# stateSpaceRobotics/pointcloud_obstacle_processing

Measured on NVIDIA B200. Metric: points/sec per B200 job (HDL-64 120k-point frames: crop + 0.1 m voxel + RANSAC ground removal + Euclidean clustering + centroid/radius), higher is better.
Workload: dtype f32

## Files before the change

### pointcloud_obstacle_processing_b200/csrc/internal.cuh

```cuda
#pragma once
#include "common.cuh"

struct pcop_handle;

namespace pcop {

int fail_cuda(pcop_handle* h, cudaError_t e, const char* expr, const char* file, int line);

struct KernelTimers {
  static constexpr int MAX_SLOTS = 8192;
  static constexpr int MAX_NAMES = 64;
  bool enabled = false;
  cudaEvent_t* ev = nullptr;
  int used = 0;
  const char* slot_name[MAX_SLOTS];
  int n_names = 0;
  const char* names[MAX_NAMES];
  double total_us[MAX_NAMES];
  long long launches[MAX_NAMES];
};

struct Ctx {
  cudaStream_t stream;
  int B;
  int cap;
  int64_t* launches;
  KernelTimers* kt;
  int grid_cap;
  cudaEvent_t block_ev = nullptr;
};

inline cudaError_t stream_wait(cudaStream_t s, cudaEvent_t block_ev) {
  if (!block_ev) return cudaStreamSynchronize(s);
  const cudaError_t e = cudaEventRecord(block_ev, s);
  return e != cudaSuccess ? e : cudaEventSynchronize(block_ev);
}

inline void count_launch(const Ctx& c, int n = 1) { *c.launches += n; }

struct KScope {
  const Ctx& c;
  int slot;
  KScope(const Ctx& cc, const char* name) : c(cc), slot(-1) {
    KernelTimers* k = c.kt;
    if (k && k->enabled && k->ev && k->used < KernelTimers::MAX_SLOTS) {
      slot = k->used++;
      k->slot_name[slot] = name;
      cudaEventRecord(k->ev[2 * slot], c.stream);
    }
  }
  ~KScope() {
    if (slot >= 0) cudaEventRecord(c.kt->ev[2 * slot + 1], c.stream);
  }
};
#define KL(ctx, name, ...)          \
  do {                              \
    ::pcop::KScope _ks(ctx, name);  \
    __VA_ARGS__;                    \
  } while (0)

struct SortBufs {
  uint32_t* key[2];
  uint32_t* val[2];
  uint32_t* hist;
  uint32_t* desc;
  uint32_t* maxkey;
  int* npass;
  unsigned long long* stats;
};
size_t sort_desc_bytes(int B, int cap);
void radix_sort_batched(const Ctx& c, const SortBufs& s, const int* count, bool iota_vals);
void sort_reset_maxkey(const Ctx& c, const SortBufs& s);

struct CropArgs {
  const float4* in;
  size_t in_stride;
  const int* n_in;
  float4* out;
  int* kept_idx;
  int* n_out;
  MinMax* minmax;
  unsigned* desc;
  float lim[6];
};
void run_crop(const Ctx& c, const CropArgs& a);

void run_minmax(const Ctx& c, const float4* pts, size_t stride, const int* n, MinMax* minmax, bool finite_only = false);

struct VoxelArgs {
  const float4* in;
  size_t in_stride;
  const int* n_in;
  const MinMax* minmax;
  float leaf;
  VoxelFrame* vf;
  SortBufs sort;
  unsigned* desc;
  int* run_start;
  float4* out;
  uint32_t* out_keys;
  int* n_out;
  uint32_t* warnings;
};
void run_voxel(const Ctx& c, const VoxelArgs& a);

void run_grid_sort(const Ctx& c, const float4* in, size_t in_stride, const int* n_in, float cell, MinMax* minmax,
                   EceFrame* ef, const SortBufs& sort, float4* sorted_pts, int* parent, int* csize, int clique = 0);

struct VoxFusedPlan {
  int ok;
  float lim[6];
  float inv;
  int b0[3];
  uint32_t nx, ny, nz;
  int bits, npass, digit_bits;
  int part_ok, part_shift, nb, nb_pad;
};
VoxFusedPlan make_vox_fused_plan(const pcop_params& p);
void vox_part_plan(VoxFusedPlan& pl, size_t max_points);
size_t vox_fused_hist_elems(int B);
size_t vox_fused_desc_bytes(int B, int cap);
struct VoxelFusedArgs {
  const float4* in;
  size_t in_stride;
  const int* n_in;
  VoxFusedPlan plan;
  float leaf;
  MinMax* minmax;
  VoxelFrame* vf;
  SortBufs sort;
  unsigned long long* pair[2];
  unsigned* desc;
  uint32_t* flags;
  uint32_t* warnings;
  int* n_crop;
  float4* out;
  uint32_t* out_keys;
  int* n_out;
  int want_keys;
};
void run_voxel_fused(const Ctx& c, const VoxelFusedArgs& a);

int vox_part_chunks(int max_n, int B);
int vox_part_group_bound(const VoxFusedPlan& pl, int max_n);
size_t vox_part_hist_elems(int B);
size_t vox_part_start_elems(int B);
size_t vox_part_chunk_start_elems(int B);
size_t vox_part_bucket_elems(int B);
struct VoxelPartArgs {
  const float4* in;
  size_t in_stride;
  const int* n_in;
  VoxFusedPlan plan;
  float leaf;
  MinMax* minmax;
  VoxelFrame* vf;
  uint32_t* ghist;
  uint32_t* chunk_start;
  unsigned short* ne_bucket;
  uint32_t* ne_start;
  uint2* grec;
  int* n_groups;
  float4* part;
  unsigned* desc;
  int group_stride;
  int group_launch;
  uint32_t* flags;
  uint32_t* warnings;
  int* n_crop;
  float4* out;
  uint32_t* out_keys;
  int* n_out;
  int want_keys;
};
void run_voxel_part(const Ctx& c, const VoxelPartArgs& a);

struct SorArgs {
  const float4* in;
  size_t in_stride;
  const int* n_in;
  int meanK;
  double mul;
  float cell;
  MinMax* minmax;
  EceFrame* gf;
  SortBufs sort;
  float4* sorted_pts;
  float* dist;
  double* partial;
  double* thr;
  unsigned* desc;
  float4* out;
  int* kept_idx;
  int* n_out;
  uint32_t* warnings;
};
void run_sor(const Ctx& c, const SorArgs& a);

struct PlaneArgs {
  const float4* in;
  size_t in_stride;
  const int* n_in;
  int* n_in_copy;
  float4* buf[2];
  int* src[2];
  int* inlier_idx;
  PlaneFrame* pf;
  double* partial;
  unsigned* desc;
  int* n_tmp;
  int* n_active;
  int* h_n_active;
  const int* rng;
  int resident;
  int large_tier;
  PlaneConst pc;
  uint32_t* warnings;
  float4* out;
  int* out_src;
  int* n_out;
};
cudaError_t run_plane(const Ctx& c, const PlaneArgs& a);
int plane_small_tier_max();
int plane_resident_max();

struct ClusterArgs {
  const float4* in;
  size_t in_stride;
  const int* n_in;
  float tol;
  int min_size, max_size;
  int small_max;
  MinMax* minmax;
  EceFrame* ef;
  SortBufs sort;
  float4* sorted_pts;
  int* parent;
  int* csize;
  int* roots;
  int* rank_of;
  int* cell_start;
  uint32_t* cell_key;
  int* n_cells;
  int* n_route;
  unsigned* desc;
  int* offsets;
  int* indices;
  int* n_clusters;
  int* n_cluster_pts;
  float4* obstacles;
  double* partial;
  int partial_stride;
};
constexpr int ECE_SMALL_MAX = 8960;
int ece_small_limit();
bool run_cluster(const Ctx& c, const ClusterArgs& a, bool with_generic);
void run_cluster_small(const Ctx& c, const ClusterArgs& a, int small_max, bool zero_skipped);
void run_centroid_radius(const Ctx& c, const ClusterArgs& a);

struct OccGrid {
  float lim[6];
  float block_size, dev_percent;
  int W, H;
  long long cells;
};
enum { OCC_COUNT_SMEM32 = 0, OCC_COUNT_SMEM16 = 1, OCC_COUNT_GLOBAL = 2 };
constexpr int OCC_SMEM_BYTES = 220 * 1024;
int occ_count_mode(long long cells);
void run_occ_count(const Ctx& c, const float4* in, int n, const OccGrid& g, unsigned long long* counts);
void run_occ_finish(const Ctx& c, const unsigned long long* counts, const OccGrid& g, long long* row_avg, signed char* grid);
cudaError_t run_occ_count_wave(const Ctx& c, const float4* in, size_t in_stride, const int* n_in, const OccGrid& g,
                               int* counts);
void run_occ_finish_wave(const Ctx& c, const int* counts, const OccGrid& g, signed char* grids, uint32_t* warnings);

struct Mat34 {
  float m[12];
};
struct OccShadowArgs {
  const float4* cloud;
  size_t cloud_stride;
  const int* n_points;
  const int* offsets;
  size_t offsets_stride;
  const int* indices;
  size_t indices_stride;
  const int* n_clusters;
  const Mat34* mats;
  float y_min, x_max, block_size;
  int W;
  long long size;
  int opacity;
  signed char* grid;
  int* records;
  uint32_t* warnings;
};
void run_occ_shadows(const Ctx& c, const OccShadowArgs& a, int blocks_per_frame, int max_points);

}
```

### pointcloud_obstacle_processing_b200/csrc/pcop_api.cu

```cuda
#include <cstdio>
#include <cstdlib>
#include <chrono>
#include <cstring>
#include <cmath>
#include <string>
#include <vector>

#include "internal.cuh"
#include "primitives.cuh"

using namespace pcop;

namespace {

enum {
  CNT_IN = 0,
  CNT_CROP,
  CNT_VOX,
  CNT_SOR,
  CNT_REM,
  CNT_CLUS,
  CNT_CLPTS,
  CNT_TMP,
  CNT_NINL,
  CNT_CLUS1,
  CNT_CELLS,
  CNT_ROUTE,
  CNT_GROUPS,
  CNT_ROWS
};

enum {
  PK_CROP_KEPT = 0,
  PK_VOX_KEYS,
  PK_VOX_PTS,
  PK_SOR_KEPT,
  PK_INLIERS,
  PK_REM_PTS,
  PK_REM_SRC,
  PK_OFFSETS,
  PK_INDICES,
  PK_OBSTACLES,
  PK_N
};
const int kPkElem[PK_N] = {4, 4, 16, 4, 4, 16, 4, 4, 4, 16};
const int kPkCount[PK_N] = {CNT_CROP, CNT_VOX, CNT_VOX, CNT_SOR, CNT_NINL, CNT_REM, CNT_REM, CNT_CLUS1, CNT_CLPTS, CNT_CLUS};
const uint32_t kPkMask[PK_N] = {PCOP_OUT_CROP,      PCOP_OUT_VOXEL,     PCOP_OUT_VOXEL,    PCOP_OUT_SOR,
                                PCOP_OUT_PLANE,     PCOP_OUT_REMAINING, PCOP_OUT_REMAINING, PCOP_OUT_CLUSTERS,
                                PCOP_OUT_CLUSTERS,  PCOP_OUT_OBSTACLES};

struct PlaneRecord {
  int n_passes;
  int n_inliers_last;
  float4 coeff;
  int pass_points[PCOP_MAX_PLANE_PASSES_RECORDED];
  int pass_inliers[PCOP_MAX_PLANE_PASSES_RECORDED];
  float4 pass_coeff[PCOP_MAX_PLANE_PASSES_RECORDED];
};

struct PackMeta {
  unsigned long long base[PK_N];
  unsigned long long total_bytes;
  int total[PK_N];
  int overflow;
};

struct Pc2Frame {
  const unsigned char* data;
  int n, point_step, off_x, off_y, off_z;
  int is_dense, apply_transform, aligned;
  Mat34 t;
};

thread_local std::string g_global_error;

constexpr int PCOP_MIN_LANE_WAVE = 8;

}

struct pcop_handle {
  pcop_params params;
  int device = 0;
  int cap = 0;
  int maxB = 0;
  cudaStream_t stream = nullptr;
  std::string err;
  std::vector<void*> dev_allocs;
  std::vector<void*> host_allocs;

  float4 *d_in = nullptr, *d_crop = nullptr, *d_vox = nullptr, *d_sor = nullptr, *d_pbuf[2] = {nullptr, nullptr},
         *d_rem = nullptr, *d_sorted = nullptr, *d_obst = nullptr;
  int *d_crop_kept = nullptr, *d_run_start = nullptr, *d_sor_kept = nullptr, *d_psrc[2] = {nullptr, nullptr},
      *d_rem_src = nullptr, *d_inliers = nullptr, *d_parent = nullptr, *d_csize = nullptr, *d_roots = nullptr,
      *d_rank = nullptr, *d_indices = nullptr, *d_offsets = nullptr, *d_cell_start = nullptr;
  uint32_t* d_cell_key = nullptr;
  uint32_t* d_vox_keys = nullptr;
  float* d_sor_dist = nullptr;
  SortBufs sort{};
  unsigned* d_desc = nullptr;
  int* d_counts = nullptr;
  uint32_t* d_warnings = nullptr;
  MinMax* d_minmax = nullptr;
  VoxelFrame* d_vf = nullptr;
  EceFrame* d_ef = nullptr;
  PlaneFrame* d_pf = nullptr;
  PlaneRecord* d_prec = nullptr;
  double* d_partial = nullptr;
  double* d_thr = nullptr;
  int* d_n_active = nullptr;
  int* d_rng = nullptr;
  int* d_pack_off = nullptr;
  PackMeta* d_meta = nullptr;
  unsigned char* d_pack = nullptr;
  unsigned long long* d_pack_cursor = nullptr;
  cudaStream_t cstream = nullptr;
  cudaEvent_t ev_copied = nullptr;
  cudaEvent_t ev_meta = nullptr;
  int wave_seq = 0;
  int call_lane_waves = 1;
  bool pending = false;
  int pend_w0 = 0, pend_B = 0;
  double d2h_bytes = 0.0;
  float4* d_acc = nullptr;
  unsigned char* d_occ = nullptr;
  size_t occ_cap = 0;
  unsigned char* d_shadow = nullptr;
  size_t shadow_cap = 0;
  int* d_occ_counts = nullptr;
  signed char* d_occ_grids = nullptr;
  size_t occ_scratch_cells = 0;
  Mat34* d_occ_mats = nullptr;
  Mat34* h_occ_mats = nullptr;
  cudaEvent_t ev_grids_copied = nullptr;
  struct OccCall {
    OccGrid g;
    const float* world_to_sensor16;
    const float* sensor_to_world16;
    int8_t* grids;
    bool grids_on_device;
  };
  const OccCall* occ = nullptr;
  unsigned char* d_raw = nullptr;
  size_t raw_cap = 0;
  Pc2Frame* d_pc2 = nullptr;
  Pc2Frame* h_pc2 = nullptr;
  int acc_count = 0;
  size_t pack_cap = 0;
  uint32_t alloc_outputs = 0;

  int* h_n_active = nullptr;
  int* h_counts = nullptr;
  uint32_t* h_warnings = nullptr;
  PlaneRecord* h_prec = nullptr;
  PackMeta* h_meta = nullptr;
  int* h_n_in = nullptr;
  unsigned long long* h_stats = nullptr;
  unsigned long long sort_pass_keys = 0;
  unsigned char* h_pack_buf[2] = {nullptr, nullptr};
  size_t h_pack_buf_cap[2] = {0, 0};
  int h_pack_sel = 0;
  unsigned char* h_pack = nullptr;
  size_t h_pack_cap = 0;
  size_t h_pack_used = 0;

  cudaEvent_t ev_call[2] = {nullptr, nullptr};
  cudaEvent_t ev_stage[PCOP_N_STAGES][2] = {};
  bool stage_used[PCOP_N_STAGES] = {};
  float stage_us[PCOP_N_STAGES] = {};
  float last_elapsed_us = 0.f;
  int64_t launches = 0;
  double alg_bytes = 0.0;
  KernelTimers kt;

  int wave_frames = 0;
  bool trace = false;
  struct TraceRec {
    int w0, B;
    size_t bytes;
    cudaEvent_t meta, c0, c1;
  };
  std::vector<TraceRec> trace_recs;
  size_t trace_used = 0;
  int ece_small_max = 0;
  int plane_resident = 1;
  bool expect_big_remaining = false;
  bool expect_large_plane = false;
  int plane_hostloop_waves = 0;
  int vox_lsd_waves = 0;
  bool wave_plane_resident = false;
  bool wave_plane_speculated = false;
  const float4* plane_in = nullptr;
  size_t plane_stride = 0;
  const int* plane_n = nullptr;
  bool wave_cluster_speculated = false;
  int pend_max_n = 1;
  VoxFusedPlan vplan{};
  uint32_t* d_vf_flags = nullptr;
  unsigned long long* d_vf_pair[2] = {nullptr, nullptr};
  uint32_t* h_vf_flags = nullptr;
  int vox_mode = 0;
  int vox_redo = -1;
  bool vox_full_groups = false;
  bool wave_used_fused = false;
  uint32_t* d_vp_hist = nullptr;
  uint32_t* d_vp_bstart = nullptr;
  uint32_t* d_vp_nstart = nullptr;
  unsigned short* d_vp_ne = nullptr;
  uint2* d_vp_grec = nullptr;
  unsigned* d_vp_desc = nullptr;
  int vp_gstride = 0;
  int vp_group_hint = 0;
  std::vector<pcop_handle*> extra_lanes;
  std::vector<size_t> fixups;
  cudaEvent_t ev_lane_done = nullptr;

  int* cnt(int row) { return d_counts + (size_t)row * maxB; }
};

namespace pcop {
int fail_cuda(pcop_handle* h, cudaError_t e, const char* expr, const char* file, int line) {
  char buf[512];
  snprintf(buf, sizeof(buf), "CUDA error %d (%s) at %s:%d: %s", (int)e, cudaGetErrorString(e), file, line, expr);
  if (h) h->err = buf;
  g_global_error = buf;
  return PCOP_ERR_CUDA;
}
}

namespace {

int fail(pcop_handle* h, int code, const std::string& msg) {
  if (h) h->err = msg;
  g_global_error = msg;
  return code;
}

void fill_rng_table(uint32_t seed, int* out, int count) {
  uint32_t mt[624];
  mt[0] = seed;
  for (int i = 1; i < 624; ++i) mt[i] = 1812433253u * (mt[i - 1] ^ (mt[i - 1] >> 30)) + (uint32_t)i;
  int pos = 624;
  for (int k = 0; k < count; ++k) {
    if (pos >= 624) {
      for (int i = 0; i < 624; ++i) {
        const uint32_t y = (mt[i] & 0x80000000u) | (mt[(i + 1) % 624] & 0x7fffffffu);
        mt[i] = mt[(i + 397) % 624] ^ (y >> 1) ^ ((y & 1u) ? 0x9908b0dfu : 0u);
      }
      pos = 0;
    }
    uint32_t y = mt[pos++];
    y ^= y >> 11;
    y ^= (y << 7) & 0x9d2c5680u;
    y ^= (y << 15) & 0xefc60000u;
    y ^= y >> 18;
    out[k] = (int)(y >> 1);
  }
}

VoxFusedPlan make_plan(const pcop_params& p, size_t max_points, int* mode) {
  VoxFusedPlan pl = make_vox_fused_plan(p);
  vox_part_plan(pl, max_points);
  const char* s = getenv("PCOP_VOXEL_FUSED");
  if (s && s[0] == '0') pl.ok = 0;
  if (s && (s[0] == 'l' || s[0] == 'L')) pl.part_ok = 0;
  if (!pl.ok) pl.part_ok = 0;
  *mode = pl.part_ok ? 2 : (pl.ok ? 1 : 0);
  return pl;
}

int validate_params(pcop_handle* h, const pcop_params& p) {
  if (p.enable_voxel && !(p.downsample_size > 0.0f)) return fail(h, PCOP_ERR_BAD_PARAM, "downsample_size must be > 0");
  if (p.enable_sor && (p.statistical_outlier_meanK < 1 || p.statistical_outlier_meanK > 63))
    return fail(h, PCOP_ERR_BAD_PARAM, "statistical_outlier_meanK must be in [1, 63]");
  if (p.enable_plane && (p.plane_max_iterations < 0 || p.plane_max_iterations + 1 > PCOP_MAX_HYPOTHESES))
    return fail(h, PCOP_ERR_BAD_PARAM, "plane_max_iterations must be in [0, 63]");
  if (p.enable_plane && !(p.plane_probability > 0.0 && p.plane_probability < 1.0))
    return fail(h, PCOP_ERR_BAD_PARAM, "plane_probability must be in (0, 1)");
  if (p.enable_cluster && !(p.euc_cluster_tolerance > 0.0f))
    return fail(h, PCOP_ERR_BAD_PARAM, "euc_cluster_tolerance must be > 0");
  return PCOP_OK;
}

uint32_t effective_outputs(const pcop_params& p) {
  uint32_t m = p.outputs & (uint32_t)(PCOP_OUT_ALL | PCOP_OUT_DEVICE);
  if (p.publish_point_clouds) m |= PCOP_OUT_ALL;
  if (!p.enable_crop) m &= ~(uint32_t)PCOP_OUT_CROP;
  if (!p.enable_voxel) m &= ~(uint32_t)PCOP_OUT_VOXEL;
  if (!p.enable_sor) m &= ~(uint32_t)PCOP_OUT_SOR;
  if (!p.enable_plane) m &= ~(uint32_t)PCOP_OUT_PLANE;
  if (!p.enable_cluster) m &= ~(uint32_t)(PCOP_OUT_CLUSTERS | PCOP_OUT_OBSTACLES);
  return m;
}

size_t pack_capacity_bytes(uint32_t mask, int B, int cap) {
  mask &= (uint32_t)PCOP_OUT_ALL;
  size_t bytes = 0;
  for (int k = 0; k < PK_N; ++k)
    if (mask & kPkMask[k]) bytes += ((size_t)B * (cap + 1)) * kPkElem[k] + 256;
  return (bytes + 256 + 255) & ~(size_t)255;
}

template <class T>
int dalloc(pcop_handle* h, T** p, size_t n) {
  void* q = nullptr;
  cudaError_t e = cudaMalloc(&q, std::max<size_t>(n, 1) * sizeof(T));
  if (e != cudaSuccess) return fail_cuda(h, e, "cudaMalloc", __FILE__, __LINE__);
  h->dev_allocs.push_back(q);
  *p = (T*)q;
  return PCOP_OK;
}
template <class T>
int halloc(pcop_handle* h, T** p, size_t n) {
  void* q = nullptr;
  cudaError_t e = cudaHostAlloc(&q, std::max<size_t>(n, 1) * sizeof(T), cudaHostAllocMapped);
  if (e != cudaSuccess) return fail_cuda(h, e, "cudaHostAlloc", __FILE__, __LINE__);
  h->host_allocs.push_back(q);
  *p = (T*)q;
  return PCOP_OK;
}
#define TRY(x)                      \
  do {                              \
    int _s = (x);                   \
    if (_s != PCOP_OK) return _s;   \
  } while (0)

int ensure_pack_capacity(pcop_handle* h, uint32_t mask) {
  const size_t need = pack_capacity_bytes(mask, h->maxB, h->cap);
  if (need <= h->pack_cap) return PCOP_OK;
  if (h->cstream) cudaStreamSynchronize(h->cstream);
  if (h->d_pack) cudaFree(h->d_pack);
  h->d_pack = nullptr;
  h->pack_cap = 0;
  cudaError_t e = cudaMalloc((void**)&h->d_pack, need);
  if (e != cudaSuccess) return fail_cuda(h, e, "cudaMalloc(pack)", __FILE__, __LINE__);
  h->pack_cap = need;
  return PCOP_OK;
}

int ensure_host_pack(pcop_handle* h, size_t need) {
  if (need <= h->h_pack_cap) return PCOP_OK;
  size_t ncap = std::max<size_t>(need, h->h_pack_cap * 2);
  ncap = std::max<size_t>(ncap, 1 << 20);
  unsigned char* q = nullptr;
  cudaError_t e = cudaHostAlloc((void**)&q, ncap, cudaHostAllocMapped);
  if (e != cudaSuccess) return fail_cuda(h, e, "cudaHostAlloc(pack)", __FILE__, __LINE__);
  if (h->cstream) cudaStreamSynchronize(h->cstream);
  if (h->h_pack) {
    memcpy(q, h->h_pack, h->h_pack_cap);
    cudaFreeHost(h->h_pack);
  }
  h->h_pack = q;
  h->h_pack_cap = ncap;
  h->h_pack_buf[h->h_pack_sel] = q;
  h->h_pack_buf_cap[h->h_pack_sel] = ncap;
  return PCOP_OK;
}

int ensure_raw(pcop_handle* h, size_t bytes) {
  if (bytes <= h->raw_cap) return PCOP_OK;
  PCOP_CUDA_TRY(cudaStreamSynchronize(h->stream));
  if (h->d_raw) cudaFree(h->d_raw);
  h->d_raw = nullptr;
  h->raw_cap = 0;
  PCOP_CUDA_TRY(cudaMalloc((void**)&h->d_raw, bytes + bytes / 4 + 256));
  h->raw_cap = bytes + bytes / 4 + 256;
  return PCOP_OK;
}

__global__ void k_copy_counts(const int* __restrict__ src, int* __restrict__ dst, int B) {
  const int f = blockIdx.x * blockDim.x + threadIdx.x;
  if (f < B) dst[f] = src[f];
}

__global__ void k_zero_u32(uint32_t* p, int n) {
  const int i = blockIdx.x * blockDim.x + threadIdx.x;
  if (i < n) p[i] = 0u;
}

__global__ void __launch_bounds__(256)
    k_transform(const float4* __restrict__ in, int n, Mat34 t, int is_dense, float4* __restrict__ out) {
  const int i = blockIdx.x * blockDim.x + threadIdx.x;
  if (i >= n) return;
  const float4 p = __ldg(in + i);
  float4 o = p;
  const bool finite = fabsf(p.x) <= 3.402823466e+38f && fabsf(p.y) <= 3.402823466e+38f && fabsf(p.z) <= 3.402823466e+38f;
  if (is_dense || finite) {
    o.x = fadd(fadd(fadd(fmul(t.m[0], p.x), fmul(t.m[1], p.y)), fmul(t.m[2], p.z)), t.m[3]);
    o.y = fadd(fadd(fadd(fmul(t.m[4], p.x), fmul(t.m[5], p.y)), fmul(t.m[6], p.z)), t.m[7]);
    o.z = fadd(fadd(fadd(fmul(t.m[8], p.x), fmul(t.m[9], p.y)), fmul(t.m[10], p.z)), t.m[11]);
  }
  out[i] = o;
}

__device__ __forceinline__ float pc2_load_f32(const unsigned char* p) {
  if ((reinterpret_cast<uintptr_t>(p) & 3u) == 0u) return __ldg(reinterpret_cast<const float*>(p));
  const uint32_t b = (uint32_t)p[0] | ((uint32_t)p[1] << 8) | ((uint32_t)p[2] << 16) | ((uint32_t)p[3] << 24);
  return __uint_as_float(b);
}
__device__ __forceinline__ float pc2_lane(const float4& v, int k) {
  return k == 0 ? v.x : (k == 1 ? v.y : (k == 2 ? v.z : v.w));
}
__global__ void __launch_bounds__(256)
    k_pc2_ingest(const Pc2Frame* __restrict__ frames, float4* __restrict__ out, size_t out_stride) {
  const int f = blockIdx.y;
  const int n = frames[f].n;
  const int i = blockIdx.x * blockDim.x + threadIdx.x;
  if (i >= n) return;
  const Pc2Frame& d = frames[f];
  const unsigned char* rec = d.data + (size_t)i * (size_t)d.point_step;
  float x, y, z;
  if (d.aligned) {
    const float4 v = __ldg(reinterpret_cast<const float4*>(rec + (d.off_x & ~15)));
    x = pc2_lane(v, (d.off_x & 15) >> 2);
    y = pc2_lane(v, (d.off_y & 15) >> 2);
    z = pc2_lane(v, (d.off_z & 15) >> 2);
  } else {
    x = pc2_load_f32(rec + d.off_x);
    y = pc2_load_f32(rec + d.off_y);
    z = pc2_load_f32(rec + d.off_z);
  }
  float4 o = make_float4(x, y, z, 1.0f);
  const bool finite = fabsf(x) <= 3.402823466e+38f && fabsf(y) <= 3.402823466e+38f && fabsf(z) <= 3.402823466e+38f;
  if (d.apply_transform && (d.is_dense || finite)) {
    const Mat34& t = d.t;
    o.x = fadd(fadd(fadd(fmul(t.m[0], x), fmul(t.m[1], y)), fmul(t.m[2], z)), t.m[3]);
    o.y = fadd(fadd(fadd(fmul(t.m[4], x), fmul(t.m[5], y)), fmul(t.m[6], z)), t.m[7]);
    o.z = fadd(fadd(fadd(fmul(t.m[8], x), fmul(t.m[9], y)), fmul(t.m[10], z)), t.m[11]);
  }
  out[(size_t)f * out_stride + i] = o;
}

Pc2Frame make_pc2_frame(const unsigned char* src, int n, int point_step, int ox, int oy, int oz, const float* t16,
                        int is_dense) {
  Pc2Frame d{};
  d.data = src;
  d.n = n;
  d.point_step = point_step;
  d.off_x = ox;
  d.off_y = oy;
  d.off_z = oz;
  d.is_dense = is_dense ? 1 : 0;
  d.apply_transform = t16 ? 1 : 0;
  const float ident[12] = {1, 0, 0, 0, 0, 1, 0, 0, 0, 0, 1, 0};
  memcpy(d.t.m, t16 ? t16 : ident, sizeof(d.t.m));
  const bool word4 = (ox & 3) == 0 && (oy & 3) == 0 && (oz & 3) == 0;
  const bool one_word = (ox >> 4) == (oy >> 4) && (ox >> 4) == (oz >> 4);
  d.aligned = (point_step % 16 == 0 && (reinterpret_cast<uintptr_t>(src) & 15u) == 0u && word4 && one_word) ? 1 : 0;
  return d;
}

bool pc2_layout_ok(int point_step, int ox, int oy, int oz) {
  return point_step >= 4 && ox >= 0 && oy >= 0 && oz >= 0 && ox <= point_step - 4 && oy <= point_step - 4 &&
         oz <= point_step - 4;
}

__device__ __forceinline__ void pc2_store_f32(unsigned char* p, float v) {
  const uint32_t b = __float_as_uint(v);
  if ((reinterpret_cast<uintptr_t>(p) & 3u) == 0u) {
    *reinterpret_cast<uint32_t*>(p) = b;
  } else {
    p[0] = (unsigned char)b;
    p[1] = (unsigned char)(b >> 8);
    p[2] = (unsigned char)(b >> 16);
    p[3] = (unsigned char)(b >> 24);
  }
}
__global__ void __launch_bounds__(256)
    k_pc2_egress(const float4* __restrict__ in, int n, int point_step, int off_x, int off_y, int off_z,
                 unsigned char* __restrict__ out) {
  const int i = blockIdx.x * blockDim.x + threadIdx.x;
  if (i >= n) return;
  const float4 p = __ldg(in + i);
  unsigned char* rec = out + (size_t)i * (size_t)point_step;
  if (point_step == 16 && off_x == 0 && off_y == 4 && off_z == 8 && (reinterpret_cast<uintptr_t>(out) & 15u) == 0u) {
    *reinterpret_cast<float4*>(rec) = p;
    return;
  }
  for (int b = 0; b < point_step; ++b) rec[b] = 0;
  pc2_store_f32(rec + off_x, p.x);
  pc2_store_f32(rec + off_y, p.y);
  pc2_store_f32(rec + off_z, p.z);
  if (point_step == 16 && off_x == 0 && off_y == 4 && off_z == 8) pc2_store_f32(rec + 12, p.w);
}

__global__ void __launch_bounds__(CT_THREADS)
    k_copy_cloud(const float4* __restrict__ in, size_t in_stride, const int* __restrict__ n_in, float4* __restrict__ out,
                 int* __restrict__ out_src, int cap) {
  const int f = blockIdx.y, tile = blockIdx.x;
  const int n = n_in[f];
  if (tile * CT_TILE >= n) return;
#pragma unroll
  for (int k = 0; k < CT_ITEMS; ++k) {
    const int i = ct_index(tile, k);
    if (i < n) {
      out[(size_t)f * cap + i] = __ldg(in + (size_t)f * in_stride + i);
      out_src[(size_t)f * cap + i] = i;
    }
  }
}

__device__ void plane_record_one(const PlaneFrame* __restrict__ pf, PlaneRecord* __restrict__ rec, int* __restrict__ n_inl,
                                 int* __restrict__ n_clus, int* __restrict__ n_clus1, int plane_enabled, int f) {
  PlaneRecord r;
  r.n_passes = 0;
  r.n_inliers_last = 0;
  r.coeff = make_float4(0.f, 0.f, 0.f, 0.f);
  for (int k = 0; k < PCOP_MAX_PLANE_PASSES_RECORDED; ++k) {
    r.pass_points[k] = 0;
// ... 56 lines not shown
    if (lane == 0) total[k] = run;
  }
  __syncthreads();
  if (threadIdx.x == 0) {
    const unsigned long long start = cursor ? *cursor : 0ull;
    unsigned long long off = start;
    for (int k = 0; k < PK_N; ++k) {
      meta->base[k] = off;
      meta->total[k] = total[k];
      off += ((unsigned long long)total[k] * kPkElemD[k] + 255ull) & ~255ull;
    }
    meta->total_bytes = off - start;
    meta->overflow = (off > capacity) ? 1 : 0;
    if (cursor && off <= capacity) *cursor = off;
  }
}

struct MetaOut {
  const uint32_t* src[5];
  uint32_t* dst[5];
  int words[5];
  int frames;
};
__device__ __forceinline__ void meta_out_segment(const uint32_t* __restrict__ s, uint32_t* __restrict__ d, int words, int first,
                                                 int stride) {
  for (int i = first; i < words; i += stride) d[i] = s[i];
}
__device__ __forceinline__ void meta_out(const MetaOut& m, int k, int first, int stride) {
#pragma unroll
  for (int j = 0; j < 5; ++j)
    if (j == k && m.src[j]) meta_out_segment(m.src[j], m.dst[j], m.words[j], first, stride);
}
__global__ void __launch_bounds__(256) k_meta_out(MetaOut m) {
  meta_out(m, blockIdx.y, blockIdx.x * blockDim.x + threadIdx.x, gridDim.x * blockDim.x);
}
struct PackSrc {
  const uint32_t* src[PK_N];
  unsigned long long frame_stride_words[PK_N];
  int count_row[PK_N];
  int words_per_elem[PK_N];
};

__global__ void __launch_bounds__(256)
    k_pack(PackSrc ps, const int* __restrict__ counts, int maxB, const int* __restrict__ pack_off,
           const PackMeta* __restrict__ meta, unsigned char* __restrict__ pack, MetaOut mo) {
  const int which = blockIdx.z, f = blockIdx.y;
  if (f < mo.frames && which < 5)
    meta_out(mo, which, (f * gridDim.x + blockIdx.x) * blockDim.x + threadIdx.x, mo.frames * gridDim.x * blockDim.x);
  const uint32_t* base = ps.src[which];
  if (!base || meta->overflow) return;
  const int wpe = ps.words_per_elem[which];
  const int n = counts[(size_t)ps.count_row[which] * maxB + f];
  const uint32_t* s = base + (size_t)f * ps.frame_stride_words[which];
  uint32_t* dst = reinterpret_cast<uint32_t*>(pack + meta->base[which]) + (size_t)pack_off[(size_t)which * maxB + f] * wpe;
  if (wpe == 4) {
    const uint4* s4 = reinterpret_cast<const uint4*>(s);
    uint4* d4 = reinterpret_cast<uint4*>(dst);
    for (int i = blockIdx.x * blockDim.x + threadIdx.x; i < n; i += gridDim.x * blockDim.x) d4[i] = s4[i];
  } else {
    for (int i = blockIdx.x * blockDim.x + threadIdx.x; i < n; i += gridDim.x * blockDim.x) dst[i] = s[i];
  }
}

struct StageTimer {
  pcop_handle* h;
  int stage;
  StageTimer(pcop_handle* hh, int s) : h(hh), stage(s) {
    cudaEventRecord(h->ev_stage[s][0], h->stream);
    h->stage_used[s] = true;
  }
  ~StageTimer() { cudaEventRecord(h->ev_stage[stage][1], h->stream); }
};

void resolve_kernel_timers(pcop_handle* h) {
  KernelTimers& k = h->kt;
  for (int sl = 0; sl < k.used; ++sl) {
    float ms = 0.f;
    if (cudaEventElapsedTime(&ms, k.ev[2 * sl], k.ev[2 * sl + 1]) != cudaSuccess) {
      cudaGetLastError();
      continue;
    }
    int id = -1;
    for (int i = 0; i < k.n_names; ++i)
      if (k.names[i] == k.slot_name[sl] || strcmp(k.names[i], k.slot_name[sl]) == 0) {
        id = i;
        break;
      }
    if (id < 0 && k.n_names < KernelTimers::MAX_NAMES) {
      id = k.n_names++;
      k.names[id] = k.slot_name[sl];
      k.total_us[id] = 0.0;
      k.launches[id] = 0;
    }
    if (id >= 0) {
      k.total_us[id] += (double)ms * 1000.0;
      k.launches[id] += 1;
    }
  }
  k.used = 0;
}

Ctx make_ctx(pcop_handle* h, int B, int grid_cap = -1) {
  return Ctx{h->stream, B, h->cap, &h->launches, &h->kt, (grid_cap > 0 && grid_cap < h->cap) ? grid_cap : h->cap, nullptr};
}

PlaneConst make_plane_const(const pcop_params& p) {
  PlaneConst pc;
  pc.thr = p.plane_segment_dist_thres;
  pc.eps_angle = (double)p.plane_segment_angle;
  pc.cos_eps = std::cos(pc.eps_angle);
  for (int a = 0; a < 3; ++a) pc.axis[a] = (double)p.plane_axis[a];
  pc.keep_fraction = p.plane_keep_fraction;
  pc.max_iterations = p.plane_max_iterations;
  pc.probability = p.plane_probability;
  pc.log_probability = 0.0;
  pc.optimize = p.optimize_coefficients ? 1 : 0;
  return pc;
}

PlaneArgs make_plane_args(pcop_handle* h, const float4* in, size_t stride, const int* n_in) {
  PlaneArgs a{};
  a.in = in;
  a.in_stride = stride;
  a.n_in = n_in;
  a.buf[0] = h->d_pbuf[0];
  a.buf[1] = h->d_pbuf[1];
  a.src[0] = h->d_psrc[0];
  a.src[1] = h->d_psrc[1];
  a.inlier_idx = h->d_inliers;
  a.pf = h->d_pf;
  a.partial = h->d_partial;
  a.desc = h->d_desc;
  a.n_tmp = h->cnt(CNT_TMP);
  a.n_active = h->d_n_active;
  a.h_n_active = h->h_n_active;
  a.rng = h->d_rng;
  a.resident = h->plane_resident;
  a.pc = make_plane_const(h->params);
  a.warnings = h->d_warnings;
  a.out = h->d_rem;
  a.out_src = h->d_rem_src;
  a.n_out = h->cnt(CNT_REM);
  return a;
}

ClusterArgs make_cluster_args(pcop_handle* h, const float4* in, size_t stride, const int* n_in) {
  ClusterArgs a{};
  a.in = in;
  a.in_stride = stride;
  a.n_in = n_in;
  a.tol = h->params.euc_cluster_tolerance;
  a.min_size = h->params.euc_min_cluster_size;
  a.max_size = h->params.euc_max_cluster_size;
  a.small_max = h->ece_small_max;
  a.minmax = h->d_minmax;
  a.ef = h->d_ef;
  a.sort = h->sort;
  a.sorted_pts = h->d_sorted;
  a.parent = h->d_parent;
  a.csize = h->d_csize;
  a.roots = h->d_roots;
  a.rank_of = h->d_rank;
  a.cell_start = h->d_cell_start;
  a.cell_key = h->d_cell_key;
  a.n_cells = h->cnt(CNT_CELLS);
  a.n_route = h->cnt(CNT_ROUTE);
  a.desc = h->d_desc;
  a.offsets = h->d_offsets;
  a.indices = h->d_indices;
  a.n_clusters = h->cnt(CNT_CLUS);
  a.n_cluster_pts = h->cnt(CNT_CLPTS);
  a.obstacles = h->d_obst;
  a.partial = h->d_partial;
  a.partial_stride = cdiv(h->cap, TS_CHUNK) * 10;
  return a;
}

CropArgs make_crop_args(pcop_handle* h, const float4* in, size_t stride, const int* n_in) {
  CropArgs a{};
  a.in = in;
  a.in_stride = stride;
  a.n_in = n_in;
  a.out = h->d_crop;
  a.kept_idx = h->d_crop_kept;
  a.n_out = h->cnt(CNT_CROP);
  a.minmax = h->d_minmax;
  a.desc = h->d_desc;
  const pcop_params& p = h->params;
  a.lim[0] = p.x_min;
  a.lim[1] = p.x_max;
  a.lim[2] = p.y_min;
  a.lim[3] = p.y_max;
  a.lim[4] = p.z_min;
  a.lim[5] = p.z_max;
  return a;
}

VoxelArgs make_voxel_args(pcop_handle* h, const float4* in, size_t stride, const int* n_in) {
  VoxelArgs a{};
  a.in = in;
  a.in_stride = stride;
  a.n_in = n_in;
  a.minmax = h->d_minmax;
  a.leaf = h->params.downsample_size;
  a.vf = h->d_vf;
  a.sort = h->sort;
  a.desc = h->d_desc;
  a.run_start = h->d_run_start;
  a.out = h->d_vox;
  a.out_keys = h->d_vox_keys;
  a.n_out = h->cnt(CNT_VOX);
  a.warnings = h->d_warnings;
  return a;
}

SorArgs make_sor_args(pcop_handle* h, const float4* in, size_t stride, const int* n_in) {
  SorArgs a{};
  a.in = in;
  a.in_stride = stride;
  a.n_in = n_in;
  a.meanK = h->params.statistical_outlier_meanK;
  a.mul = (double)h->params.statistical_outlier_stdDevThres;
  a.cell = (h->params.enable_voxel && h->params.downsample_size > 0.0f) ? 3.0f * h->params.downsample_size : 0.05f;
  a.minmax = h->d_minmax;
  a.gf = h->d_ef;
  a.sort = h->sort;
  a.sorted_pts = h->d_sorted;
  a.dist = h->d_sor_dist;
  a.partial = h->d_partial;
  a.thr = h->d_thr;
  a.desc = h->d_desc;
  a.out = h->d_sor;
  a.kept_idx = h->d_sor_kept;
  a.n_out = h->cnt(CNT_SOR);
  a.warnings = h->d_warnings;
  return a;
}

bool is_device_pointer(const void* p) {
  cudaPointerAttributes at;
  if (cudaPointerGetAttributes(&at, p) != cudaSuccess) {
    cudaGetLastError();
    return false;
  }
  return at.type == cudaMemoryTypeDevice || at.type == cudaMemoryTypeManaged;
}

int run_wave_plane(pcop_handle* h, int B, int max_n, bool large_tier) {
  const pcop_params& p = h->params;
  Ctx c = make_ctx(h, B, max_n);
  StageTimer t(h, PCOP_STAGE_PLANE);
  h->wave_plane_speculated = false;
  if (p.enable_plane) {
    PlaneArgs a = make_plane_args(h, h->plane_in, h->plane_stride, h->plane_n);
    a.n_in_copy = p.enable_sor ? nullptr : h->cnt(CNT_SOR);
    a.large_tier = large_tier ? 1 : 0;
    if (h->plane_hostloop_waves > 0) a.resident = 0;
    h->wave_plane_resident = a.resident != 0;
    if (!(effective_outputs(p) & PCOP_OUT_PLANE)) a.inlier_idx = nullptr;
    cudaError_t e = run_plane(c, a);
    if (e != cudaSuccess) return fail_cuda(h, e, "run_plane", __FILE__, __LINE__);
    h->wave_plane_speculated = a.resident && !large_tier && max_n > plane_small_tier_max();
  } else {
    KL(c, "k_copy_counts", k_copy_counts<<<cdiv(B, 256), 256, 0, h->stream>>>(h->plane_n, h->cnt(CNT_REM), B));
    KL(c, "k_copy_cloud", k_copy_cloud<<<dim3(cdiv(c.grid_cap, CT_TILE), B), CT_THREADS, 0, h->stream>>>(
                              h->plane_in, h->plane_stride, h->plane_n, h->d_rem, h->d_rem_src, h->cap));
    count_launch(c, 2);
  }
  return PCOP_OK;
}

int run_wave_stages(pcop_handle* h, int B, const float4* in, size_t stride, int max_n) {
  const pcop_params& p = h->params;
  Ctx c = make_ctx(h, B, max_n);
  const int tiles = cdiv(h->cap, CT_TILE);
  const int vmode = (h->vox_redo >= 0) ? h->vox_redo : ((h->vox_mode == 2 && h->vox_lsd_waves > 0) ? 1 : h->vox_mode);
  const bool fused_path = vmode != 0;
  if (!fused_path || (effective_outputs(p) & PCOP_OUT_CROP)) {
    KL(c, "k_zero_u32", k_zero_u32<<<cdiv(B, 256), 256, 0, h->stream>>>(h->d_warnings, B));
    count_launch(c);
  }

  const float4* cur = in;
  size_t cur_stride = stride;
  const int* cur_n = h->cnt(CNT_IN);
  bool have_minmax = false;

  const bool fused = fused_path;
  h->wave_used_fused = fused;
  if (fused && vmode == 2) {
    {
      StageTimer t(h, PCOP_STAGE_CROP);
      if (effective_outputs(p) & PCOP_OUT_CROP) run_crop(c, make_crop_args(h, cur, cur_stride, cur_n));
    }
    StageTimer t(h, PCOP_STAGE_VOXEL);
    VoxelPartArgs a{};
    a.in = cur;
    a.in_stride = cur_stride;
    a.n_in = cur_n;
    a.plan = h->vplan;
    a.leaf = p.downsample_size;
    a.minmax = h->d_minmax;
    a.vf = h->d_vf;
    a.ghist = h->d_vp_hist;
    a.chunk_start = h->d_vp_bstart;
    a.ne_bucket = h->d_vp_ne;
    a.ne_start = h->d_vp_nstart;
    a.grec = h->d_vp_grec;
    a.n_groups = h->cnt(CNT_GROUPS);
    a.part = h->d_sorted;
    a.desc = h->d_vp_desc;
    a.group_stride = h->vp_gstride;
    a.group_launch = h->vox_full_groups ? h->vp_gstride - 1 : std::min(h->vp_group_hint, vox_part_group_bound(h->vplan, max_n));
    a.flags = h->d_vf_flags;
    a.warnings = (effective_outputs(p) & PCOP_OUT_CROP) ? nullptr : h->d_warnings;
    a.n_crop = h->cnt(CNT_CROP);
    a.out = h->d_vox;
    a.out_keys = h->d_vox_keys;
    a.n_out = h->cnt(CNT_VOX);
    a.want_keys = (effective_outputs(p) & PCOP_OUT_VOXEL) ? 1 : 0;
    run_voxel_part(c, a);
    cur = h->d_vox;
    cur_stride = h->cap;
    cur_n = h->cnt(CNT_VOX);
  } else if (fused) {
    {
      StageTimer t(h, PCOP_STAGE_CROP);
      if (effective_outputs(p) & PCOP_OUT_CROP) run_crop(c, make_crop_args(h, cur, cur_stride, cur_n));
    }
    StageTimer t(h, PCOP_STAGE_VOXEL);
    VoxelFusedArgs a{};
    a.in = cur;
    a.in_stride = cur_stride;
    a.n_in = cur_n;
    a.plan = h->vplan;
    a.leaf = p.downsample_size;
    a.minmax = h->d_minmax;
    a.vf = h->d_vf;
    a.sort = h->sort;
    a.pair[0] = h->d_vf_pair[0];
    a.pair[1] = h->d_vf_pair[1];
    a.desc = h->d_desc;
    a.flags = h->d_vf_flags;
    a.warnings = (effective_outputs(p) & PCOP_OUT_CROP) ? nullptr : h->d_warnings;
    a.n_crop = h->cnt(CNT_CROP);
    a.out = h->d_vox;
    a.out_keys = h->d_vox_keys;
    a.n_out = h->cnt(CNT_VOX);
    a.want_keys = (effective_outputs(p) & PCOP_OUT_VOXEL) ? 1 : 0;
    run_voxel_fused(c, a);
    cur = h->d_vox;
    cur_stride = h->cap;
    cur_n = h->cnt(CNT_VOX);
  } else {
    {
      StageTimer t(h, PCOP_STAGE_CROP);
      if (p.enable_crop) {
        run_crop(c, make_crop_args(h, cur, cur_stride, cur_n));
        cur = h->d_crop;
        cur_stride = h->cap;
        cur_n = h->cnt(CNT_CROP);
        have_minmax = true;
      } else {
        KL(c, "k_copy_counts", k_copy_counts<<<cdiv(B, 256), 256, 0, h->stream>>>(cur_n, h->cnt(CNT_CROP), B));
        count_launch(c);
      }
    }
    {
      StageTimer t(h, PCOP_STAGE_VOXEL);
      if (p.enable_voxel) {
        if (!have_minmax) run_minmax(c, cur, cur_stride, cur_n, h->d_minmax);
        run_voxel(c, make_voxel_args(h, cur, cur_stride, cur_n));
        cur = h->d_vox;
        cur_stride = h->cap;
        cur_n = h->cnt(CNT_VOX);
      } else {
        KL(c, "k_copy_counts", k_copy_counts<<<cdiv(B, 256), 256, 0, h->stream>>>(cur_n, h->cnt(CNT_VOX), B));
        count_launch(c);
      }
    }
  }
  {
    StageTimer t(h, PCOP_STAGE_SOR);
    if (p.enable_sor) {
      run_sor(c, make_sor_args(h, cur, cur_stride, cur_n));
      cur = h->d_sor;
      cur_stride = h->cap;
      cur_n = h->cnt(CNT_SOR);
    } else if (!p.enable_plane) {
      KL(c, "k_copy_counts", k_copy_counts<<<cdiv(B, 256), 256, 0, h->stream>>>(cur_n, h->cnt(CNT_SOR), B));
      count_launch(c);
    }
  }
  h->plane_in = cur;
  h->plane_stride = cur_stride;
  h->plane_n = cur_n;
  TRY(run_wave_plane(h, B, max_n, h->expect_large_plane));
  cudaError_t e = cudaGetLastError();
  if (e != cudaSuccess) return fail_cuda(h, e, "stage launches", __FILE__, __LINE__);
  return PCOP_OK;
}

int run_wave_cluster(pcop_handle* h, int B, int max_n, bool with_generic) {
  const pcop_params& p = h->params;
  Ctx c = make_ctx(h, B, max_n);
  ClusterArgs ca = make_cluster_args(h, h->d_rem, h->cap, h->cnt(CNT_REM));
  bool generic_centroid = false;
  {
    StageTimer t(h, PCOP_STAGE_CLUSTER);
    if (p.enable_cluster) {
      generic_centroid = run_cluster(c, ca, with_generic);
    } else {
      cudaMemsetAsync(h->cnt(CNT_CLUS), 0, sizeof(int) * B, h->stream);
      cudaMemsetAsync(h->cnt(CNT_CLPTS), 0, sizeof(int) * B, h->stream);
    }
  }
  {
    StageTimer t(h, PCOP_STAGE_CENTROID);
    if (p.enable_cluster && generic_centroid) run_centroid_radius(c, ca);
  }
  h->wave_cluster_speculated = p.enable_cluster && !generic_centroid && max_n > h->ece_small_max;
  cudaError_t e = cudaGetLastError();
  if (e != cudaSuccess) return fail_cuda(h, e, "stage launches", __FILE__, __LINE__);
  return PCOP_OK;
}

struct Pc2Call {
  const pcop_pointcloud2_frame* frames;
  const float* transform16;
  std::vector<char> on_device;
};

struct WaveInput {
  const float* xyzw;
  size_t frame_stride_points;
  const int32_t* n;
  bool on_device;
  const Pc2Call* pc2;
};

size_t pc2_payload_bytes(const pcop_pointcloud2_frame& m) { return (size_t)m.n_points * (size_t)m.point_step; }

int enqueue_wave_decode(pcop_handle* h, const Pc2Call& pc, int w0, int B, int max_n) {
  if (h->vox_redo < 0) {
    size_t off = 0;
    for (int f = 0; f < B; ++f) {
      const pcop_pointcloud2_frame& m = pc.frames[w0 + f];
      const size_t bytes = pc2_payload_bytes(m);
      const unsigned char* src = m.data;
      if (bytes > 0 && !pc.on_device[w0 + f]) {
        PCOP_CUDA_TRY(cudaMemcpyAsync(h->d_raw + off, m.data, bytes, cudaMemcpyHostToDevice, h->stream));
        src = h->d_raw + off;
        off += (bytes + 255) & ~(size_t)255;
      }
      h->h_pc2[f] = make_pc2_frame(src, m.n_points, m.point_step, m.off_x, m.off_y, m.off_z,
                                   pc.transform16 ? pc.transform16 + (size_t)(w0 + f) * 16 : nullptr, m.is_dense);
    }
    PCOP_CUDA_TRY(cudaMemcpyAsync(h->d_pc2, h->h_pc2, sizeof(Pc2Frame) * B, cudaMemcpyHostToDevice, h->stream));
  }
  Ctx c = make_ctx(h, B, max_n);
  KL(c, "k_pc2_ingest", k_pc2_ingest<<<dim3(cdiv(max_n, 256), B), 256, 0, h->stream>>>(h->d_pc2, h->d_in, (size_t)h->cap));
  count_launch(c);
  return PCOP_OK;
}

int enqueue_wave_pack(pcop_handle* h, int B, int max_n, uint32_t mask) {
  Ctx c = make_ctx(h, B, max_n);
  StageTimer t(h, PCOP_STAGE_D2H);
  const bool dev_results = (mask & PCOP_OUT_DEVICE) != 0;
  if (!dev_results && h->wave_seq >= 1) PCOP_CUDA_TRY(cudaStreamWaitEvent(h->stream, h->ev_copied, 0));
  KL(c, "k_pack_scan", k_pack_scan<<<1, 320, 0, h->stream>>>(h->d_counts, h->maxB, B, mask, h->d_pack_off, h->d_meta, h->d_pf, h->d_prec,
                                             h->params.enable_plane ? 1 : 0, dev_results ? h->d_pack_cursor : nullptr,
                                             (unsigned long long)h->pack_cap));
  count_launch(c);
  const void* srcs[PK_N] = {h->d_crop_kept, h->d_vox_keys, h->d_vox,     h->d_sor_kept, h->d_inliers,
                            h->d_rem,       h->d_rem_src,  h->d_offsets, h->d_indices,  h->d_obst};
  const size_t strides[PK_N] = {(size_t)h->cap, (size_t)h->cap, (size_t)h->cap,     (size_t)h->cap, (size_t)h->cap,
                                (size_t)h->cap, (size_t)h->cap, (size_t)h->cap + 1, (size_t)h->cap, (size_t)h->cap};
  {
    PackSrc ps{};
    bool any = false;
    for (int k = 0; k < PK_N; ++k) {
      ps.src[k] = (mask & kPkMask[k]) ? (const uint32_t*)srcs[k] : nullptr;
      ps.frame_stride_words[k] = (unsigned long long)strides[k] * (kPkElem[k] / 4);
      ps.count_row[k] = kPkCount[k];
      ps.words_per_elem[k] = kPkElem[k] / 4;
      any = any || ps.src[k];
    }
    MetaOut m{};
    int nseg = 0;
    auto seg = [&](const void* src, void* dst, size_t bytes) {
      m.src[nseg] = (const uint32_t*)src;
      m.dst[nseg] = (uint32_t*)dst;
      m.words[nseg] = (int)(bytes / 4);
      ++nseg;
    };
    seg(h->d_counts, h->h_counts, sizeof(int) * CNT_ROWS * h->maxB);
    seg(h->d_warnings, h->h_warnings, sizeof(uint32_t) * B);
    seg(h->d_prec, h->h_prec, sizeof(PlaneRecord) * B);
    seg(h->d_meta, h->h_meta, sizeof(PackMeta));
    if (h->wave_used_fused) seg(h->d_vf_flags, h->h_vf_flags, sizeof(uint32_t) * B);
    static_assert(PK_N >= 5, "one pack block per metadata segment");
    if (any) {
      const int gx = std::max(1, std::min(cdiv(c.grid_cap, 256 * 4), std::max(16, 592 / B)));
      m.frames = std::min(B, 4);
      KL(c, "k_pack", k_pack<<<dim3(gx, B, PK_N), 256, 0, h->stream>>>(ps, h->d_counts, h->maxB, h->d_pack_off, h->d_meta, h->d_pack, m));
      count_launch(c);
    } else {
      KL(c, "k_meta_out", k_meta_out<<<dim3(4, nseg), 256, 0, h->stream>>>(m));
      count_launch(c);
    }
  }
  if (h->trace) {
    if (h->trace_used == h->trace_recs.size()) {
      pcop_handle::TraceRec r{};
      cudaEventCreate(&r.meta);
      cudaEventCreate(&r.c0);
      cudaEventCreate(&r.c1);
      h->trace_recs.push_back(r);
    }
    cudaEventRecord(h->trace_recs[h->trace_used].meta, h->stream);
  }
  PCOP_CUDA_TRY(cudaEventRecord(h->ev_meta, h->stream));
  return PCOP_OK;
}

int enqueue_wave_counts(pcop_handle* h, int w0, int B, const float4* in, size_t stride, int max_n) {
  const pcop_handle::OccCall& oc = *h->occ;
  for (int f = 0; f < B; ++f) {
    memcpy(h->h_occ_mats[2 * f].m, oc.world_to_sensor16 + (size_t)(w0 + f) * 16, sizeof(Mat34));
    memcpy(h->h_occ_mats[2 * f + 1].m, oc.sensor_to_world16 + (size_t)(w0 + f) * 16, sizeof(Mat34));
  }
  PCOP_CUDA_TRY(cudaMemcpyAsync(h->d_occ_mats, h->h_occ_mats, sizeof(Mat34) * 2 * B, cudaMemcpyHostToDevice, h->stream));
  PCOP_CUDA_TRY(cudaMemsetAsync(h->d_occ_counts, 0, sizeof(int) * (size_t)B * (size_t)oc.g.cells, h->stream));
  Ctx c = make_ctx(h, B, max_n);
  const cudaError_t e = run_occ_count_wave(c, in, stride, h->cnt(CNT_IN), oc.g, h->d_occ_counts);
  if (e != cudaSuccess) return fail_cuda(h, e, "run_occ_count_wave (shared-memory opt-in or launch)", __FILE__, __LINE__);
  return PCOP_OK;
}

int enqueue_wave_grids(pcop_handle* h, int B, int max_n) {
  const pcop_handle::OccCall& oc = *h->occ;
  Ctx c = make_ctx(h, B, max_n);
  PCOP_CUDA_TRY(cudaStreamWaitEvent(h->stream, h->ev_grids_copied, 0));
  run_occ_finish_wave(c, h->d_occ_counts, oc.g, h->d_occ_grids, h->d_warnings);
  OccShadowArgs a{};
  a.cloud = h->d_rem;
  a.cloud_stride = h->cap;
  a.n_points = h->cnt(CNT_REM);
  a.offsets = h->d_offsets;
  a.offsets_stride = (size_t)h->cap + 1;
  a.indices = h->d_indices;
  a.indices_stride = h->cap;
  a.n_clusters = h->cnt(CNT_CLUS);
  a.mats = h->d_occ_mats;
  a.y_min = oc.g.lim[2];
  a.x_max = oc.g.lim[1];
  a.block_size = oc.g.block_size;
  a.W = oc.g.W;
  a.size = oc.g.cells;
  a.opacity = h->params.grid_opacity;
  a.grid = h->d_occ_grids;
  a.warnings = h->d_warnings;
  run_occ_shadows(c, a, std::max(4, std::min(64, cdiv(2048, B))), max_n);
  cudaError_t e = cudaGetLastError();
  if (e != cudaSuccess) return fail_cuda(h, e, "grid launches", __FILE__, __LINE__);
  return PCOP_OK;
}

int enqueue_wave_back(pcop_handle* h, int B, int max_n, uint32_t mask, bool cluster_with_generic) {
  TRY(run_wave_cluster(h, B, max_n, cluster_with_generic));
  if (h->occ) TRY(enqueue_wave_grids(h, B, max_n));
  return enqueue_wave_pack(h, B, max_n, mask);
}

int enqueue_wave(pcop_handle* h, const WaveInput& wi, int w0, int B, uint32_t mask) {
  for (int s = 0; s < PCOP_N_STAGES; ++s) h->stage_used[s] = false;
  const float4* in;
  size_t stride;
  const int32_t* n = wi.n;
  int max_n = 1;
  for (int f = 0; f < B; ++f) max_n = std::max(max_n, (int)n[w0 + f]);
  {
    StageTimer t(h, PCOP_STAGE_H2D);
    memcpy(h->h_n_in, n + w0, sizeof(int) * B);
    PCOP_CUDA_TRY(cudaMemcpyAsync(h->cnt(CNT_IN), h->h_n_in, sizeof(int) * B, cudaMemcpyHostToDevice, h->stream));
    if (wi.pc2) {
      TRY(enqueue_wave_decode(h, *wi.pc2, w0, B, max_n));
      in = h->d_in;
      stride = h->cap;
    } else if (wi.on_device) {
      in = reinterpret_cast<const float4*>(wi.xyzw) + (size_t)w0 * wi.frame_stride_points;
      stride = wi.frame_stride_points;
    } else {
      const float* src = wi.xyzw + (size_t)w0 * wi.frame_stride_points * 4;
      bool uniform = true;
      for (int f = 1; f < B; ++f) uniform = uniform && (n[w0 + f] == n[w0]);
      if (B > 0 && uniform && n[w0] > 0) {
        PCOP_CUDA_TRY(cudaMemcpy2DAsync(h->d_in, (size_t)h->cap * 16, src, wi.frame_stride_points * 16, (size_t)n[w0] * 16,
                                        B, cudaMemcpyHostToDevice, h->stream));
      } else {
        for (int f = 0; f < B; ++f)
          if (n[w0 + f] > 0)
            PCOP_CUDA_TRY(cudaMemcpyAsync(h->d_in + (size_t)f * h->cap, src + (size_t)f * wi.frame_stride_points * 4,
                                          (size_t)n[w0 + f] * 16, cudaMemcpyHostToDevice, h->stream));
      }
      in = h->d_in;
      stride = h->cap;
// ... 224 lines not shown
  if ((!xyzw && !pc2) || !n || !out || batch < 0) return fail(h, PCOP_ERR_BAD_PARAM, "null argument");
  PCOP_CUDA_TRY(cudaSetDevice(h->device));
  for (int f = 0; f < batch; ++f) {
    if (n[f] < 0) return fail(h, PCOP_ERR_BAD_PARAM, "negative point count");
    if (n[f] > h->cap) return fail(h, PCOP_ERR_CAPACITY, "frame has more points than max_points");
    if ((size_t)n[f] > frame_stride_points && batch > 1) return fail(h, PCOP_ERR_BAD_PARAM, "frame_stride_points < n");
  }
  const uint32_t mask = effective_outputs(h->params);
  const WaveInput wi{xyzw, frame_stride_points, n, pc2 ? false : is_device_pointer(xyzw), pc2};
  std::vector<pcop_handle*> lanes(1, h);
  if (!h->kt.enabled)
    for (pcop_handle* l : h->extra_lanes) lanes.push_back(l);
  std::vector<std::pair<int, int>> waves;
  {
    const int L = (int)lanes.size();
    int nw = std::max(1, cdiv(batch, std::max(1, std::min(h->wave_frames, h->maxB))));
    if (nw < L) nw = std::max(1, std::min(L, batch / PCOP_MIN_LANE_WAVE));
    const int full = (nw > 1) ? std::min(h->maxB, cdiv(2 * batch, 2 * nw - 1)) : std::min(h->maxB, batch);
    for (int w0 = 0; w0 < batch;) {
      const int B = std::min(full, batch - w0);
      waves.push_back({w0, B});
      w0 += B;
    }
  }
  size_t raw_need = 0;
  if (pc2)
    for (const auto& w : waves) {
      size_t bytes = 0;
      for (int f = w.first; f < w.first + w.second; ++f)
        if (!pc2->on_device[f]) bytes += (pc2_payload_bytes(pc2->frames[f]) + 255) & ~(size_t)255;
      raw_need = std::max(raw_need, bytes);
    }
  h->occ = nullptr;
  for (pcop_handle* l : h->extra_lanes) l->occ = nullptr;
  for (pcop_handle* l : lanes) {
    l->occ = occ;
    if (occ && !waves.empty()) TRY(ensure_occ_scratch(l, (size_t)waves[0].second, (size_t)occ->g.cells));
    if (raw_need) TRY(ensure_raw(l, raw_need));
    l->params = h->params;
    l->vplan = h->vplan;
    l->vox_mode = h->vox_mode;
    l->launches = 0;
    l->alg_bytes = 0.0;
    l->d2h_bytes = 0.0;
    l->kt.used = 0;
    l->sort_pass_keys = 0;
    l->h_pack_used = 0;
    l->h_pack_sel ^= 1;
    l->h_pack = l->h_pack_buf[l->h_pack_sel];
    l->h_pack_cap = l->h_pack_buf_cap[l->h_pack_sel];
    l->fixups.clear();
    l->wave_seq = 0;
    l->call_lane_waves = cdiv((int)waves.size(), (int)lanes.size());
    l->trace_used = 0;
    l->pending = false;
    for (int s = 0; s < PCOP_N_STAGES; ++s) l->stage_us[s] = 0.f;
    TRY(ensure_pack_capacity(l, mask));
  }
  PCOP_CUDA_TRY(cudaEventRecord(h->ev_call[0], h->stream));
  if (h->trace) g_trace_t0 = std::chrono::steady_clock::now();
  for (size_t l = 0; l < lanes.size(); ++l) {
    if (l > 0) PCOP_CUDA_TRY(cudaStreamWaitEvent(lanes[l]->stream, h->ev_call[0], 0));
    PCOP_CUDA_TRY(cudaMemsetAsync(lanes[l]->sort.stats, 0, sizeof(unsigned long long), lanes[l]->stream));
    if (mask & PCOP_OUT_DEVICE)
      PCOP_CUDA_TRY(cudaMemsetAsync(lanes[l]->d_pack_cursor, 0, sizeof(unsigned long long), lanes[l]->stream));
  }
  int status = PCOP_OK;
  for (size_t w = 0; w < waves.size() && status == PCOP_OK; ++w) {
    pcop_handle* l = lanes[w % lanes.size()];
    const double th0 = h->trace ? trace_host_us() : 0.0;
    status = finish_wave(l, wi, mask, out);
    const double th1 = h->trace ? trace_host_us() : 0.0;
    if (status == PCOP_OK) status = enqueue_wave(l, wi, waves[w].first, waves[w].second, mask);
    if (h->trace)
      fprintf(stderr, "[pcop trace]   host: wave %4d+%-4d lane %zu: finish of the lane's previous wave %7.0f .. %7.0f us, enqueue .. %7.0f us\n",
              waves[w].first, waves[w].second, w % lanes.size(), th0, th1, trace_host_us());
    if (status != PCOP_OK && l != h) h->err = l->err;
  }
  for (size_t k = 0; k < lanes.size(); ++k) {
    pcop_handle* l = lanes[(waves.size() + k) % lanes.size()];
    const int st = finish_wave(l, wi, mask, out);
    if (st != PCOP_OK && status == PCOP_OK) {
      status = st;
      if (l != h) h->err = l->err;
    }
  }
  for (pcop_handle* l : lanes) {
    cudaMemcpyAsync(l->h_stats, l->sort.stats, sizeof(unsigned long long), cudaMemcpyDeviceToHost, l->stream);
    cudaEventRecord(l->ev_lane_done, l->cstream);
    cudaStreamWaitEvent(l->stream, l->ev_lane_done, 0);
    cudaEventRecord(l->ev_lane_done, l->stream);
    if (l != h) cudaStreamWaitEvent(h->stream, l->ev_lane_done, 0);
  }
  PCOP_CUDA_TRY(cudaEventRecord(h->ev_call[1], h->stream));
  PCOP_CUDA_TRY(cudaEventSynchronize(h->ev_call[1]));
  if (status != PCOP_OK) return status;
  float ms = 0.f;
  PCOP_CUDA_TRY(cudaEventElapsedTime(&ms, h->ev_call[0], h->ev_call[1]));
  h->last_elapsed_us = ms * 1000.f;
  if (h->trace) {
    fprintf(stderr, "[pcop trace] call of %d frames: %.0f us on the device\n", batch, ms * 1000.f);
    for (size_t li = 0; li < lanes.size(); ++li) {
      for (size_t k = 0; k < lanes[li]->trace_used; ++k) {
        const pcop_handle::TraceRec& tr = lanes[li]->trace_recs[k];
        float a = 0.f, b = 0.f, c = 0.f;
        cudaEventElapsedTime(&a, h->ev_call[0], tr.meta);
        cudaEventElapsedTime(&b, h->ev_call[0], tr.c0);
        cudaEventElapsedTime(&c, h->ev_call[0], tr.c1);
        fprintf(stderr, "[pcop trace]   lane %zu wave %4d+%-4d counts at %7.0f us, payload copy %7.0f .. %7.0f us (%.1f MB, %.1f GB/s)\n", li,
                tr.w0, tr.B, a * 1000.f, b * 1000.f, c * 1000.f, tr.bytes / 1e6, tr.bytes / 1e3 / std::max(1e-3f, (c - b) * 1000.f));
      }
      lanes[li]->trace_used = 0;
    }
    cudaGetLastError();
  }
  for (pcop_handle* l : lanes) {
    l->sort_pass_keys = *l->h_stats;
    for (size_t fx : l->fixups) {
      const void** slot = (const void**)((unsigned char*)out + fx);
      const size_t off = (size_t)(uintptr_t)(*slot) - 1;
      *slot = l->h_pack + off;
    }
    if (l == h) continue;
    h->launches += l->launches;
    h->alg_bytes += l->alg_bytes;
    h->d2h_bytes += l->d2h_bytes;
    h->sort_pass_keys += l->sort_pass_keys;
    for (int s = 0; s < PCOP_N_STAGES; ++s) h->stage_us[s] += l->stage_us[s];
    merge_kernel_timers(h, l);
  }
  return PCOP_OK;
}

int upload_single(pcop_handle* h, const float* xyzw, int32_t n, int count_row) {
  if (n < 0) return fail(h, PCOP_ERR_BAD_PARAM, "negative point count");
  if (n > h->cap) return fail(h, PCOP_ERR_CAPACITY, "cloud has more points than max_points");
  PCOP_CUDA_TRY(cudaSetDevice(h->device));
  h->h_n_in[0] = n;
  PCOP_CUDA_TRY(cudaMemcpyAsync(h->cnt(count_row), h->h_n_in, sizeof(int), cudaMemcpyHostToDevice, h->stream));
  if (n > 0) PCOP_CUDA_TRY(cudaMemcpyAsync(h->d_in, xyzw, (size_t)n * 16, cudaMemcpyDefault, h->stream));
  k_zero_u32<<<1, 32, 0, h->stream>>>(h->d_warnings, 1);
  return PCOP_OK;
}

int download(pcop_handle* h, void* dst, const void* src, size_t bytes) {
  if (!dst || bytes == 0) return PCOP_OK;
  PCOP_CUDA_TRY(cudaMemcpyAsync(dst, src, bytes, cudaMemcpyDeviceToHost, h->stream));
  return PCOP_OK;
}

int fetch_count(pcop_handle* h, int row, int32_t* out) {
  PCOP_CUDA_TRY(cudaMemcpyAsync(h->h_counts, h->cnt(row), sizeof(int), cudaMemcpyDeviceToHost, h->stream));
  PCOP_CUDA_TRY(cudaStreamSynchronize(h->stream));
  *out = h->h_counts[0];
  return PCOP_OK;
}

int fetch_warnings(pcop_handle* h, uint32_t* w) {
  PCOP_CUDA_TRY(cudaMemcpyAsync(h->h_warnings, h->d_warnings, sizeof(uint32_t), cudaMemcpyDeviceToHost, h->stream));
  PCOP_CUDA_TRY(cudaStreamSynchronize(h->stream));
  if (w) *w = h->h_warnings[0];
  return PCOP_OK;
}

}

extern "C" {

int pcop_abi_version(void) { return PCOP_ABI_VERSION; }
const char* pcop_global_error(void) { return g_global_error.c_str(); }
const char* pcop_last_error(const pcop_handle* h) { return h ? h->err.c_str() : g_global_error.c_str(); }

void pcop_params_init_code_defaults(pcop_params* p) {
  memset(p, 0, sizeof(*p));
  p->x_min = -1.0f; p->x_max = 1.0f; p->y_min = -0.5f; p->y_max = 0.6f; p->z_min = 0.0f; p->z_max = -0.5f;
  p->downsample_size = 0.015f;
  p->statistical_outlier_meanK = 15;
  p->statistical_outlier_stdDevThres = 1.0f;
  p->plane_segment_dist_thres = 0.040f;
  p->plane_segment_angle = 20;
  p->euc_cluster_tolerance = 0.4f;
  p->euc_min_cluster_size = 5;
  p->euc_max_cluster_size = 20000;
  p->plane_axis[0] = 0.0f; p->plane_axis[1] = 0.0f; p->plane_axis[2] = 1.0f;
  p->plane_keep_fraction = 0.3;
  p->plane_max_iterations = 50;
  p->plane_probability = 0.99;
  p->ransac_seed = 12345u;
  p->optimize_coefficients = 1;
  p->enable_crop = p->enable_voxel = p->enable_sor = p->enable_plane = p->enable_cluster = 1;
  p->publish_point_clouds = 1;
  p->outputs = PCOP_OUT_DEFAULT;
  p->accumulate_count = 2;
  p->block_size = 0.15f;
  p->dev_percent = 0.5f;
  p->grid_opacity = 0;
  p->downsample_input_data = 1;
  p->passthrough_filter_enable = 1;
  p->convex_hull_alpha = 180.0f;
}

void pcop_params_init_params_yaml(pcop_params* p) {
  pcop_params_init_code_defaults(p);
  p->x_min = 0.0f; p->x_max = 4.5f; p->y_min = 0.0f; p->y_max = 3.78f; p->z_min = -0.5f; p->z_max = 0.25f;
  p->accumulate_count = 200;
  p->block_size = 0.0375f;
  p->dev_percent = 0.9f;
  p->grid_opacity = 0;
  p->downsample_size = 0.015f;
  p->statistical_outlier_meanK = 15;
  p->statistical_outlier_stdDevThres = 4.0f;
  p->plane_segment_dist_thres = 0.040f;
  p->plane_segment_angle = 20;
  p->euc_cluster_tolerance = 0.4f;
  p->euc_min_cluster_size = 5;
  p->euc_max_cluster_size = 20000;
  p->convex_hull_alpha = 180.0f;
  p->publish_point_clouds = 1;
}

static int create_lane(const pcop_params* params, int device, size_t max_points, int max_batch, pcop_handle** out) {
  *out = nullptr;
  int ndev = 0;
  cudaError_t e = cudaGetDeviceCount(&ndev);
  if (e != cudaSuccess || ndev == 0) {
    cudaGetLastError();
    return fail(nullptr, PCOP_ERR_CUDA, "pcop_create: no CUDA device (this library has no CPU fallback)");
  }
  if (device < 0 || device >= ndev) return fail(nullptr, PCOP_ERR_BAD_PARAM, "pcop_create: bad device index");
  cudaDeviceProp prop;
  if ((e = cudaGetDeviceProperties(&prop, device)) != cudaSuccess) return fail_cuda(nullptr, e, "props", __FILE__, __LINE__);
  if (prop.major != 10)
    return fail(nullptr, PCOP_ERR_CUDA, "pcop_create: device is not sm_100-class (kernels are built for sm_100a only)");
  pcop_handle* h = new pcop_handle();
  h->params = *params;
  h->vplan = make_plan(*params, max_points, &h->vox_mode);
  h->device = device;
  h->cap = (int)max_points;
  h->maxB = max_batch;
  int st = validate_params(h, *params);
  if (st != PCOP_OK) {
    g_global_error = h->err;
    delete h;
    return st;
  }
  auto bail = [&](int code) {
    g_global_error = h->err;
    pcop_destroy(h);
    return code;
  };
  if ((e = cudaSetDevice(device)) != cudaSuccess) return bail(fail_cuda(h, e, "cudaSetDevice", __FILE__, __LINE__));
  if ((e = cudaStreamCreateWithFlags(&h->stream, cudaStreamNonBlocking)) != cudaSuccess)
    return bail(fail_cuda(h, e, "cudaStreamCreate", __FILE__, __LINE__));
  const size_t BC = (size_t)h->maxB * h->cap;
  const int B = h->maxB;
  const int chunks = cdiv(h->cap, TS_CHUNK);
  const int tiles = cdiv(h->cap, CT_TILE);
#define A(x)                         \
  do {                               \
    int _s = (x);                    \
    if (_s != PCOP_OK) return bail(_s); \
  } while (0)
  A(dalloc(h, &h->d_in, BC));
  A(dalloc(h, &h->d_acc, (size_t)h->cap));
  A(dalloc(h, &h->d_crop, BC));
  A(dalloc(h, &h->d_vox, BC));
  A(dalloc(h, &h->d_sor, BC));
  h->d_pbuf[0] = h->d_crop;
  h->d_pbuf[1] = h->d_in;
  A(dalloc(h, &h->d_rem, BC));
  A(dalloc(h, &h->d_sorted, BC));
  A(dalloc(h, &h->d_obst, BC));
  A(dalloc(h, &h->d_crop_kept, BC));
  A(dalloc(h, &h->d_run_start, BC));
  A(dalloc(h, &h->d_sor_kept, BC));
  A(dalloc(h, &h->d_psrc[0], BC));
  A(dalloc(h, &h->d_psrc[1], BC));
  A(dalloc(h, &h->d_rem_src, BC));
  A(dalloc(h, &h->d_inliers, BC));
  A(dalloc(h, &h->d_parent, BC));
  A(dalloc(h, &h->d_csize, BC));
  A(dalloc(h, &h->d_roots, BC));
  A(dalloc(h, &h->d_rank, BC));
  A(dalloc(h, &h->d_indices, BC));
  A(dalloc(h, &h->d_cell_start, BC));
  A(dalloc(h, &h->d_cell_key, BC));
  A(dalloc(h, &h->d_offsets, BC + B));
  A(dalloc(h, &h->d_vox_keys, BC));
  A(dalloc(h, &h->d_sor_dist, BC));
  A(dalloc(h, &h->sort.key[0], BC));
  A(dalloc(h, &h->sort.key[1], BC));
  A(dalloc(h, &h->sort.val[0], BC));
  A(dalloc(h, &h->sort.val[1], BC));
  A(dalloc(h, &h->sort.hist, std::max((size_t)B * RS_MAX_PASSES * RS_BINS, vox_fused_hist_elems(B))));
  {
    unsigned char* d = nullptr;
    A(dalloc(h, &d, std::max(sort_desc_bytes(B, h->cap), vox_fused_desc_bytes(B, h->cap))));
    h->sort.desc = (uint32_t*)d;
  }
  A(dalloc(h, &h->d_vf_flags, B));
  if (h->vplan.part_ok) {
    h->vp_gstride = vox_part_group_bound(h->vplan, h->cap) + 1;
    h->vp_group_hint = h->vp_gstride - 1;
    A(dalloc(h, &h->d_vp_hist, vox_part_hist_elems(B)));
    A(dalloc(h, &h->d_vp_bstart, vox_part_chunk_start_elems(B)));
    A(dalloc(h, &h->d_vp_nstart, vox_part_start_elems(B)));
    A(dalloc(h, &h->d_vp_ne, vox_part_bucket_elems(B)));
    A(dalloc(h, &h->d_vp_grec, (size_t)B * h->vp_gstride));
    A(dalloc(h, &h->d_vp_desc, (size_t)B * h->vp_gstride));
  }
  h->d_vf_pair[0] = reinterpret_cast<unsigned long long*>(h->d_sorted);
  h->d_vf_pair[1] = reinterpret_cast<unsigned long long*>(h->d_sorted) + BC;
  A(halloc(h, &h->h_vf_flags, B));
  A(dalloc(h, &h->sort.maxkey, B));
  A(dalloc(h, &h->sort.npass, B));
  A(dalloc(h, &h->sort.stats, 1));
  A(halloc(h, &h->h_stats, 1));
  A(dalloc(h, &h->d_desc, (size_t)B * tiles));
  A(dalloc(h, &h->d_counts, (size_t)CNT_ROWS * B));
  A(dalloc(h, &h->d_warnings, B));
  A(dalloc(h, &h->d_minmax, B));
  A(dalloc(h, &h->d_vf, B));
  A(dalloc(h, &h->d_ef, B));
  A(dalloc(h, &h->d_pf, B));
  A(dalloc(h, &h->d_prec, B));
  A(dalloc(h, &h->d_partial, (size_t)B * chunks * 10));
  A(dalloc(h, &h->d_thr, B));
  A(dalloc(h, &h->d_n_active, 64));
  A(dalloc(h, &h->d_rng, RNG_TABLE));
  A(dalloc(h, &h->d_pack_off, (size_t)PK_N * B));
  A(dalloc(h, &h->d_meta, 1));
  A(dalloc(h, &h->d_pack_cursor, 1));
  A(dalloc(h, &h->d_pc2, B));
  A(halloc(h, &h->h_pc2, B));
  A(halloc(h, &h->h_n_active, 16));
  A(halloc(h, &h->h_counts, (size_t)CNT_ROWS * B));
  A(halloc(h, &h->h_warnings, B));
  A(halloc(h, &h->h_prec, B));
  A(halloc(h, &h->h_meta, 1));
  A(halloc(h, &h->h_n_in, (size_t)B + 16));
#undef A
  if ((e = cudaMemset(h->d_counts, 0, sizeof(int) * CNT_ROWS * B)) != cudaSuccess)
    return bail(fail_cuda(h, e, "memset", __FILE__, __LINE__));
  if ((e = cudaMemset(h->d_pf, 0, sizeof(PlaneFrame) * B)) != cudaSuccess)
    return bail(fail_cuda(h, e, "memset", __FILE__, __LINE__));
  {
    std::vector<int> tbl(RNG_TABLE);
    fill_rng_table(params->ransac_seed, tbl.data(), RNG_TABLE);
    if ((e = cudaMemcpy(h->d_rng, tbl.data(), sizeof(int) * RNG_TABLE, cudaMemcpyHostToDevice)) != cudaSuccess)
      return bail(fail_cuda(h, e, "rng upload", __FILE__, __LINE__));
  }
  for (int i = 0; i < 2; ++i)
    if ((e = cudaEventCreate(&h->ev_call[i])) != cudaSuccess) return bail(fail_cuda(h, e, "event", __FILE__, __LINE__));
  for (int s = 0; s < PCOP_N_STAGES; ++s)
    for (int i = 0; i < 2; ++i)
      if ((e = cudaEventCreate(&h->ev_stage[s][i])) != cudaSuccess)
        return bail(fail_cuda(h, e, "event", __FILE__, __LINE__));
  if ((e = cudaEventCreateWithFlags(&h->ev_lane_done, cudaEventDisableTiming)) != cudaSuccess)
    return bail(fail_cuda(h, e, "event", __FILE__, __LINE__));
  if ((e = cudaStreamCreateWithFlags(&h->cstream, cudaStreamNonBlocking)) != cudaSuccess)
    return bail(fail_cuda(h, e, "cudaStreamCreate", __FILE__, __LINE__));
  if ((e = cudaEventCreateWithFlags(&h->ev_copied, cudaEventDisableTiming)) != cudaSuccess ||
      (e = cudaEventCreateWithFlags(&h->ev_meta, cudaEventDisableTiming)) != cudaSuccess ||
      (e = cudaEventCreateWithFlags(&h->ev_grids_copied, cudaEventDisableTiming)) != cudaSuccess)
    return bail(fail_cuda(h, e, "event", __FILE__, __LINE__));
  st = ensure_pack_capacity(h, effective_outputs(h->params));
  if (st != PCOP_OK) return bail(st);
  *out = h;
  return PCOP_OK;
}

int pcop_create(const pcop_params* params, int device, size_t max_points, int max_batch, pcop_handle** out) {
  if (!params || !out || max_points == 0 || max_points > (size_t)65535 * BT_TILE || max_batch < 1)
    return fail(nullptr, PCOP_ERR_BAD_PARAM, "pcop_create: bad argument (max_points must be in [1, 268431360])");
  *out = nullptr;
  int wave_frames = std::min(max_batch, std::max(64, max_batch / 8));
  if (const char* s = getenv("PCOP_WAVE_FRAMES")) wave_frames = (int)std::min<long>(std::max<long>(strtol(s, nullptr, 10), 1), max_batch);
  int n_lanes = std::max(1, std::min(3, max_batch / wave_frames));
  if (const char* s = getenv("PCOP_LANES")) n_lanes = (int)std::min<long>(std::max<long>(strtol(s, nullptr, 10), 1), 8);
  n_lanes = std::max(1, std::min(n_lanes, max_batch / PCOP_MIN_LANE_WAVE));
  const int lane_batch = n_lanes == 1 ? max_batch : std::min(max_batch, wave_frames + wave_frames / 4);
  pcop_handle* h = nullptr;
  int st = create_lane(params, device, max_points, lane_batch, &h);
  if (st != PCOP_OK) return st;
  for (int l = 1; l < n_lanes; ++l) {
    pcop_handle* x = nullptr;
    st = create_lane(params, device, max_points, lane_batch, &x);
    if (st != PCOP_OK) {
      pcop_destroy(h);
      return st;
    }
    h->extra_lanes.push_back(x);
  }
  h->wave_frames = std::min(wave_frames, lane_batch);
  h->trace = getenv("PCOP_TRACE") != nullptr;
  for (pcop_handle* l : h->extra_lanes) l->trace = h->trace;
  h->ece_small_max = ece_small_limit();
  if (const char* s = getenv("PCOP_PLANE_RESIDENT")) h->plane_resident = (s[0] == '0') ? 0 : 1;
  for (pcop_handle* l : h->extra_lanes) {
    l->ece_small_max = h->ece_small_max;
    l->plane_resident = h->plane_resident;
  }
  *out = h;
  return PCOP_OK;
}

void pcop_destroy(pcop_handle* h) {
  if (!h) return;
  for (pcop_handle* l : h->extra_lanes) pcop_destroy(l);
  h->extra_lanes.clear();
  cudaSetDevice(h->device);
  if (h->stream) cudaStreamSynchronize(h->stream);
  if (h->cstream) cudaStreamSynchronize(h->cstream);
  for (void* p : h->dev_allocs) cudaFree(p);
  for (void* p : h->host_allocs) cudaFreeHost(p);
  if (h->d_pack) cudaFree(h->d_pack);
  if (h->d_raw) cudaFree(h->d_raw);
  if (h->d_occ) cudaFree(h->d_occ);
  if (h->d_shadow) cudaFree(h->d_shadow);
  if (h->d_occ_counts) cudaFree(h->d_occ_counts);
  if (h->d_occ_grids) cudaFree(h->d_occ_grids);
  for (int i = 0; i < 2; ++i)
    if (h->h_pack_buf[i]) cudaFreeHost(h->h_pack_buf[i]);
  if (h->kt.ev) {
    for (int i = 0; i < 2 * KernelTimers::MAX_SLOTS; ++i) cudaEventDestroy(h->kt.ev[i]);
    delete[] h->kt.ev;
  }
  for (int i = 0; i < 2; ++i)
    if (h->ev_call[i]) cudaEventDestroy(h->ev_call[i]);
  if (h->ev_lane_done) cudaEventDestroy(h->ev_lane_done);
  if (h->ev_copied) cudaEventDestroy(h->ev_copied);
  if (h->ev_meta) cudaEventDestroy(h->ev_meta);
  if (h->ev_grids_copied) cudaEventDestroy(h->ev_grids_copied);
  if (h->cstream) cudaStreamDestroy(h->cstream);
  for (int s = 0; s < PCOP_N_STAGES; ++s)
    for (int i = 0; i < 2; ++i)
      if (h->ev_stage[s][i]) cudaEventDestroy(h->ev_stage[s][i]);
  if (h->stream) cudaStreamDestroy(h->stream);
  delete h;
}

int pcop_set_params(pcop_handle* h, const pcop_params* params) {
  if (!h || !params) return fail(h, PCOP_ERR_BAD_PARAM, "null argument");
  int st = validate_params(h, *params);
  if (st != PCOP_OK) return st;
  PCOP_CUDA_TRY(cudaSetDevice(h->device));
  if (params->ransac_seed != h->params.ransac_seed) {
    std::vector<int> tbl(RNG_TABLE);
    fill_rng_table(params->ransac_seed, tbl.data(), RNG_TABLE);
    PCOP_CUDA_TRY(cudaMemcpy(h->d_rng, tbl.data(), sizeof(int) * RNG_TABLE, cudaMemcpyHostToDevice));
  }
  h->params = *params;
  h->vplan = make_plan(*params, (size_t)h->cap, &h->vox_mode);
  h->vox_lsd_waves = 0;
  h->plane_hostloop_waves = 0;
  for (pcop_handle* l : h->extra_lanes) {
    const int ls = pcop_set_params(l, params);
    if (ls != PCOP_OK) {
      h->err = l->err;
      return ls;
    }
  }
  return ensure_pack_capacity(h, effective_outputs(h->params));
}

int pcop_process(pcop_handle* h, const float* xyzw, int32_t n, pcop_frame_result* out) {
  return process_impl(h, xyzw, (size_t)(n > 0 ? n : 1), &n, 1, out);
}

int pcop_process_batch(pcop_handle* h, const float* xyzw, size_t frame_stride_points, const int32_t* n, int32_t batch,
                       pcop_frame_result* out) {
  return process_impl(h, xyzw, frame_stride_points, n, batch, out);
}

static int occ_grid_of(pcop_handle* h, OccGrid* g);

static int occ_call_of(pcop_handle* h, const char* who, const float* world_to_sensor16, const float* sensor_to_world16,
                       int8_t* grids, pcop_handle::OccCall* oc) {
  TRY(occ_grid_of(h, &oc->g));
  if (oc->g.cells > PCOP_OCC_BATCH_MAX_CELLS)
    return fail(h, PCOP_ERR_CAPACITY,
                std::string(who) + ": grid of " + std::to_string(oc->g.W) + " x " + std::to_string(oc->g.H) +
                    " cells exceeds PCOP_OCC_BATCH_MAX_CELLS (use pcop_occupancy_grid + pcop_occupancy_shadows)");
  PCOP_CUDA_TRY(cudaSetDevice(h->device));
  oc->world_to_sensor16 = world_to_sensor16;
  oc->sensor_to_world16 = sensor_to_world16;
  oc->grids = grids;
  oc->grids_on_device = is_device_pointer(grids);
  return PCOP_OK;
}

int pcop_process_batch_occupancy(pcop_handle* h, const float* xyzw, size_t frame_stride_points, const int32_t* n,
                                 int32_t batch, const float* world_to_sensor16, const float* sensor_to_world16,
                                 int8_t* grids, pcop_frame_result* out) {
  if (!h) return fail(nullptr, PCOP_ERR_BAD_PARAM, "null handle");
  if (!world_to_sensor16 || !sensor_to_world16 || !grids || !out || batch < 0 || (!xyzw && batch != 1))
    return fail(h, PCOP_ERR_BAD_PARAM, "pcop_process_batch_occupancy: null argument (xyzw = NULL takes batch = 1)");
  pcop_handle::OccCall oc{};
  TRY(occ_call_of(h, "pcop_process_batch_occupancy", world_to_sensor16, sensor_to_world16, grids, &oc));
  int st;
  if (!xyzw) {
    const int32_t acc_n = h->acc_count;
    st = process_impl(h, reinterpret_cast<const float*>(h->d_acc), (size_t)(acc_n > 0 ? acc_n : 1), &acc_n, 1, out, &oc);
    h->acc_count = 0;
  } else {
    st = process_impl(h, xyzw, frame_stride_points, n, batch, out, &oc);
  }
  h->occ = nullptr;
  for (pcop_handle* l : h->extra_lanes) l->occ = nullptr;
  return st;
}

int pcop_process_batch_pointcloud2(pcop_handle* h, const pcop_pointcloud2_frame* frames, int32_t batch,
                                   const float* transform16, const float* world_to_sensor16,
                                   const float* sensor_to_world16, int8_t* grids, pcop_frame_result* out) {
  if (!h) return fail(nullptr, PCOP_ERR_BAD_PARAM, "null handle");
  if (!out || batch < 0 || (!frames && batch > 0) || (grids && (!world_to_sensor16 || !sensor_to_world16)))
    return fail(h, PCOP_ERR_BAD_PARAM,
                "pcop_process_batch_pointcloud2: null argument (grids need world_to_sensor16 and sensor_to_world16)");
  Pc2Call pc;
  pc.frames = frames;
  pc.transform16 = transform16;
  std::vector<int32_t> n((size_t)batch + 1, 0);
  for (int f = 0; f < batch; ++f) {
    const pcop_pointcloud2_frame& m = frames[f];
    if (m.n_points < 0 || (!m.data && m.n_points > 0))
      return fail(h, PCOP_ERR_BAD_PARAM, "pcop_process_batch_pointcloud2: frame " + std::to_string(f) + ": bad count or NULL data");
    if (!pc2_layout_ok(m.point_step, m.off_x, m.off_y, m.off_z))
      return fail(h, PCOP_ERR_BAD_PARAM,
                  "pcop_process_batch_pointcloud2: frame " + std::to_string(f) + ": PointCloud2 field offsets do not fit point_step");
    if (m.n_points > h->cap)
      return fail(h, PCOP_ERR_CAPACITY, "pcop_process_batch_pointcloud2: frame " + std::to_string(f) + " has more points than max_points");
    n[f] = m.n_points;
  }
  pcop_handle::OccCall oc{};
  if (grids) TRY(occ_call_of(h, "pcop_process_batch_pointcloud2", world_to_sensor16, sensor_to_world16, grids, &oc));
  PCOP_CUDA_TRY(cudaSetDevice(h->device));
  pc.on_device.resize((size_t)batch);
  for (int f = 0; f < batch; ++f) pc.on_device[f] = frames[f].n_points > 0 && is_device_pointer(frames[f].data);
  const int st = process_impl(h, nullptr, (size_t)h->cap, n.data(), batch, out, grids ? &oc : nullptr, &pc);
  h->occ = nullptr;
  for (pcop_handle* l : h->extra_lanes) l->occ = nullptr;
  return st;
}

int pcop_enable_kernel_timing(pcop_handle* h, int enable) {
  if (!h) return PCOP_ERR_BAD_PARAM;
  PCOP_CUDA_TRY(cudaSetDevice(h->device));
  if (enable && !h->kt.ev) {
    h->kt.ev = new cudaEvent_t[2 * KernelTimers::MAX_SLOTS];
    for (int i = 0; i < 2 * KernelTimers::MAX_SLOTS; ++i) PCOP_CUDA_TRY(cudaEventCreate(&h->kt.ev[i]));
  }
  h->kt.enabled = enable != 0;
  h->kt.used = 0;
  h->kt.n_names = 0;
  return PCOP_OK;
}

int pcop_kernel_timing_count(const pcop_handle* h) { return h ? h->kt.n_names : 0; }

int pcop_kernel_timing_get(const pcop_handle* h, int i, const char** name, double* total_us, int64_t* launches) {
  if (!h || i < 0 || i >= h->kt.n_names) return PCOP_ERR_BAD_PARAM;
  if (name) *name = h->kt.names[i];
  if (total_us) *total_us = h->kt.total_us[i];
  if (launches) *launches = h->kt.launches[i];
  return PCOP_OK;
}

float pcop_last_elapsed_us(const pcop_handle* h) { return h ? h->last_elapsed_us : 0.f; }
int pcop_stage_times_us(const pcop_handle* h, float us[PCOP_N_STAGES]) {
  if (!h || !us) return PCOP_ERR_BAD_PARAM;
  for (int s = 0; s < PCOP_N_STAGES; ++s) us[s] = h->stage_us[s];
  return PCOP_OK;
}
int64_t pcop_last_launch_count(const pcop_handle* h) { return h ? h->launches : 0; }
double pcop_last_algorithmic_bytes(const pcop_handle* h) { return h ? h->alg_bytes : 0.0; }
int pcop_download(pcop_handle* h, void* dst, const void* src_device, size_t bytes) {
  if (!h || (bytes && (!dst || !src_device))) return fail(h, PCOP_ERR_BAD_PARAM, "null argument");
  PCOP_CUDA_TRY(cudaSetDevice(h->device));
  if (bytes) PCOP_CUDA_TRY(cudaMemcpyAsync(dst, src_device, bytes, cudaMemcpyDefault, h->stream));
  PCOP_CUDA_TRY(cudaStreamSynchronize(h->stream));
  return PCOP_OK;
}

int64_t pcop_last_sort_pass_keys(const pcop_handle* h) { return h ? (int64_t)h->sort_pass_keys : 0; }
double pcop_last_d2h_bytes(const pcop_handle* h) { return h ? h->d2h_bytes : 0.0; }

static int transform_into(pcop_handle* h, const float* xyzw, int32_t n, const float* t16, int is_dense, float4* dst) {
  const float4* src = reinterpret_cast<const float4*>(xyzw);
  if (!is_device_pointer(xyzw)) {
    PCOP_CUDA_TRY(cudaMemcpyAsync(h->d_in, xyzw, (size_t)n * 16, cudaMemcpyHostToDevice, h->stream));
    src = h->d_in;
  }
  Mat34 t;
  const float ident[12] = {1, 0, 0, 0, 0, 1, 0, 0, 0, 0, 1, 0};
  memcpy(t.m, t16 ? t16 : ident, sizeof(t.m));
  Ctx c = make_ctx(h, 1, n);
  KL(c, "k_transform", k_transform<<<cdiv(n, 256), 256, 0, h->stream>>>(src, n, t, is_dense, dst));
  count_launch(c);
  return PCOP_OK;
}

int pcop_accumulate(pcop_handle* h, const float* xyzw, int32_t n, const float* transform16, int32_t is_dense, int32_t* total) {
  if (!h || (!xyzw && n > 0) || n < 0) return fail(h, PCOP_ERR_BAD_PARAM, "pcop_accumulate: bad argument");
  if ((long long)h->acc_count + n > h->cap) return fail(h, PCOP_ERR_CAPACITY, "accumulated cloud exceeds max_points");
  PCOP_CUDA_TRY(cudaSetDevice(h->device));
  if (n > 0) {
    TRY(transform_into(h, xyzw, n, transform16, is_dense, h->d_acc + h->acc_count));
// ... 385 lines not shown
```

### pointcloud_obstacle_processing_b200/csrc/primitives.cuh

```cuda
#pragma once
#include "common.cuh"

namespace pcop {

__device__ __forceinline__ int lane_id() { return threadIdx.x & 31; }
__device__ __forceinline__ int warp_id() { return threadIdx.x >> 5; }
__device__ __forceinline__ unsigned lanemask_lt() { return (1u << (threadIdx.x & 31)) - 1u; }

__device__ __forceinline__ unsigned ld_volatile_u32(const unsigned* p) {
  unsigned v;
  asm volatile("ld.volatile.global.u32 %0, [%1];" : "=r"(v) : "l"(p));
  return v;
}
__device__ __forceinline__ void st_volatile_u32(unsigned* p, unsigned v) {
  asm volatile("st.volatile.global.u32 [%0], %1;" ::"l"(p), "r"(v) : "memory");
}

__device__ __forceinline__ unsigned lookback_wait(const unsigned* p) {
  unsigned d = ld_volatile_u32(p);
#ifdef PCOP_LOOKBACK_SPIN_LIMIT
  unsigned long long polls = 0ull;
#endif
  while ((d >> 30) == 0u) {
#ifdef PCOP_LOOKBACK_SPIN_LIMIT
    if (++polls > (unsigned long long)(PCOP_LOOKBACK_SPIN_LIMIT)) __trap();
#endif
    d = ld_volatile_u32(p);
  }
  return d;
}

constexpr unsigned LB_AGG = 1u << 30;
constexpr unsigned LB_PREFIX = 2u << 30;
constexpr unsigned LB_VALUE = (1u << 30) - 1u;

__device__ __forceinline__ unsigned lookback_warp(unsigned* desc_frame, int tile, unsigned aggregate) {
  const int lane = lane_id();
  if (tile == 0) {
    if (lane == 0) st_volatile_u32(desc_frame, LB_PREFIX | aggregate);
    return 0u;
  }
  if (lane == 0) st_volatile_u32(desc_frame + tile, LB_AGG | aggregate);
  unsigned exclusive = 0u;
  int look = tile - 1;
  while (true) {
    const int idx = look - lane;
    unsigned d = LB_PREFIX;
    if (idx >= 0) {
      d = lookback_wait(desc_frame + idx);
    }
    const unsigned is_prefix = __ballot_sync(FULL, (d >> 30) == 2u);
    const int first = is_prefix ? (__ffs(is_prefix) - 1) : 31;
    unsigned v = (lane <= first) ? (d & LB_VALUE) : 0u;
    v = __reduce_add_sync(FULL, v);
    exclusive += v;
    if (is_prefix) break;
    look -= 32;
  }
  if (lane == 0) st_volatile_u32(desc_frame + tile, LB_PREFIX | (exclusive + aggregate));
  return exclusive;
}

struct CompactSmem {
  unsigned warp_total[CT_THREADS / 32];
  unsigned tile_excl;
  unsigned tile_total;
};

__device__ __forceinline__ unsigned tile_compact_positions(const bool (&keep)[CT_ITEMS], unsigned (&pos)[CT_ITEMS],
                                                           unsigned* desc_frame, int tile, CompactSmem& sm) {
  const int lane = lane_id(), warp = warp_id();
  unsigned row_base = 0;
#pragma unroll
  for (int k = 0; k < CT_ITEMS; ++k) {
    const unsigned m = __ballot_sync(FULL, keep[k]);
    pos[k] = row_base + __popc(m & lanemask_lt());
    row_base += __popc(m);
  }
  if (lane == 0) sm.warp_total[warp] = row_base;
  __syncthreads();
  if (warp == 0) {
    unsigned t = (lane < CT_THREADS / 32) ? sm.warp_total[lane] : 0u;
    unsigned incl = t;
#pragma unroll
    for (int o = 1; o < CT_THREADS / 32; o <<= 1) {
      const unsigned up = __shfl_up_sync(FULL, incl, o);
      if (lane >= o) incl += up;
    }
    const unsigned tile_total = __shfl_sync(FULL, incl, CT_THREADS / 32 - 1);
    const unsigned excl = lookback_warp(desc_frame, tile, tile_total);
    if (lane < CT_THREADS / 32) sm.warp_total[lane] = excl + incl - t;
    if (lane == 0) {
      sm.tile_excl = excl;
      sm.tile_total = tile_total;
    }
  }
  __syncthreads();
  const unsigned wbase = sm.warp_total[warp];
#pragma unroll
  for (int k = 0; k < CT_ITEMS; ++k) pos[k] += wbase;
  return sm.tile_excl + sm.tile_total;
}

template <int ITEMS>
__device__ __forceinline__ int bt_index(int tile, int k) {
  return tile * (CT_THREADS * ITEMS) + warp_id() * (32 * ITEMS) + k * 32 + lane_id();
}
template <int ITEMS>
__device__ __forceinline__ unsigned big_tile_scan(unsigned keepmask, unsigned* desc_frame, int tile, CompactSmem& sm,
                                                  unsigned& wbase) {
  const int lane = lane_id(), warp = warp_id();
  unsigned wtotal = __reduce_add_sync(FULL, (unsigned)__popc(keepmask));
  if (lane == 0) sm.warp_total[warp] = wtotal;
  __syncthreads();
  if (warp == 0) {
    unsigned t = (lane < CT_THREADS / 32) ? sm.warp_total[lane] : 0u;
    unsigned incl = t;
#pragma unroll
    for (int o = 1; o < CT_THREADS / 32; o <<= 1) {
      const unsigned up = __shfl_up_sync(FULL, incl, o);
      if (lane >= o) incl += up;
    }
    const unsigned tile_total = __shfl_sync(FULL, incl, CT_THREADS / 32 - 1);
    const unsigned excl = lookback_warp(desc_frame, tile, tile_total);
    if (lane < CT_THREADS / 32) sm.warp_total[lane] = excl + incl - t;
    if (lane == 0) {
      sm.tile_excl = excl;
      sm.tile_total = tile_total;
    }
  }
  __syncthreads();
  wbase = sm.warp_total[warp];
  return sm.tile_excl + sm.tile_total;
}

__device__ __forceinline__ int ct_index(int tile, int k) {
  return tile * CT_TILE + warp_id() * (32 * CT_ITEMS) + k * 32 + lane_id();
}

__device__ __forceinline__ double tree_butterfly(double v) {
#pragma unroll
  for (int off = 16; off >= 1; off >>= 1) v = dadd(v, __shfl_xor_sync(FULL, v, off));
  return v;
}

}
```

### pointcloud_obstacle_processing_b200/csrc/stage_plane.cu

```cuda
#include "det_math.cuh"
#include <cstdio>
#include "internal.cuh"
#include "primitives.cuh"

namespace pcop {
#ifdef PCOP_PLANE_DEBUG_CLK
__device__ long long g_plane_loop_clk[16];
#define PL_CLK(k)                                                                  \
  do {                                                                             \
    if (blockIdx.y == 0 && rank == 0 && threadIdx.x == 0) g_plane_loop_clk[k] = clock64(); \
  } while (0)
#else
#define PL_CLK(k) \
  do {            \
  } while (0)
#endif

namespace {

constexpr int MAP_CAP = RNG_TABLE + 8;
constexpr double kHalfPi = 1.57079632679489661923;

__device__ __forceinline__ const float4* cur_cloud(const PlaneFrame& P, const float4* in, size_t in_stride,
                                                   float4* const* buf, int f, int cap) {
// ... 419 lines not shown
#pragma unroll
    for (int k = 0; k < 9; ++k) sh[warp_id()][k] = a[k];
    shc[warp_id()] = cnt;
  }
  __syncthreads();
  double* out = partial + ((size_t)f * chunks + chunk) * 10;
  if (threadIdx.x < 9) {
    double s = sh[0][threadIdx.x];
    for (int w = 1; w < 8; ++w) s = dadd(s, sh[w][threadIdx.x]);
    out[threadIdx.x] = s;
  } else if (threadIdx.x == 9) {
    int c = 0;
    for (int w = 0; w < 8; ++w) c += shc[w];
    out[9] = (double)c;
  }
}

__device__ void compute_roots2(double b, double c, double* r) {
  r[0] = 0.0;
  double d = dsub(dmul(b, b), dmul(4.0, c));
  if (d < 0.0) d = 0.0;
  const double sd = __dsqrt_rn(d);
  r[2] = dmul(0.5, dadd(b, sd));
  r[1] = dmul(0.5, dsub(b, sd));
}

__device__ void compute_roots(const double* m, double* r) {
  const double m00 = m[0], m01 = m[1], m02 = m[2], m11 = m[4], m12 = m[5], m22 = m[8];
  double c0 = dmul(dmul(m00, m11), m22);
  c0 = dadd(c0, dmul(dmul(dmul(2.0, m01), m02), m12));
  c0 = dsub(c0, dmul(dmul(m00, m12), m12));
  c0 = dsub(c0, dmul(dmul(m11, m02), m02));
  c0 = dsub(c0, dmul(dmul(m22, m01), m01));
  double c1 = dsub(dmul(m00, m11), dmul(m01, m01));
  c1 = dadd(c1, dmul(m00, m22));
  c1 = dsub(c1, dmul(m02, m02));
  c1 = dadd(c1, dmul(m11, m22));
  c1 = dsub(c1, dmul(m12, m12));
  const double c2 = dadd(dadd(m00, m11), m22);
  if (fabs(c0) < 2.220446049250313e-16) {
    compute_roots2(c2, c1, r);
    return;
  }
  const double s_inv3 = ddiv(1.0, 3.0);
  const double s_sqrt3 = __dsqrt_rn(3.0);
  const double c2_over_3 = dmul(c2, s_inv3);
  double a_over_3 = dmul(dsub(c1, dmul(c2, c2_over_3)), s_inv3);
  if (a_over_3 > 0.0) a_over_3 = 0.0;
  const double half_b =
      dmul(0.5, dadd(c0, dmul(c2_over_3, dsub(dmul(dmul(2.0, c2_over_3), c2_over_3), c1))));
  double q = dadd(dmul(half_b, half_b), dmul(dmul(a_over_3, a_over_3), a_over_3));
  if (q > 0.0) q = 0.0;
  const double rho = __dsqrt_rn(-a_over_3);
  const double theta = dmul(det_atan2_ypos(__dsqrt_rn(-q), half_b), s_inv3);
  const double cos_theta = det_cos(theta);
  const double sin_theta = det_sin(theta);
  r[0] = dadd(c2_over_3, dmul(dmul(2.0, rho), cos_theta));
  r[1] = dsub(c2_over_3, dmul(rho, dadd(cos_theta, dmul(s_sqrt3, sin_theta))));
  r[2] = dsub(c2_over_3, dmul(rho, dsub(cos_theta, dmul(s_sqrt3, sin_theta))));
  double t;
  if (r[0] >= r[1]) {
    t = r[0];
    r[0] = r[1];
    r[1] = t;
  }
  if (r[1] >= r[2]) {
    t = r[1];
    r[1] = r[2];
    r[2] = t;
    if (r[0] >= r[1]) {
      t = r[0];
      r[0] = r[1];
      r[1] = t;
    }
  }
  if (r[0] <= 0.0) compute_roots2(c2, c1, r);
}

__device__ __forceinline__ void cross3(const double* a, const double* b, double* o) {
  o[0] = dsub(dmul(a[1], b[2]), dmul(a[2], b[1]));
  o[1] = dsub(dmul(a[2], b[0]), dmul(a[0], b[2]));
  o[2] = dsub(dmul(a[0], b[1]), dmul(a[1], b[0]));
}

__device__ void eigen33_smallest(const double* mat, double* evec) {
  double scale = 0.0;
  for (int i = 0; i < 9; ++i) scale = fabs(mat[i]) > scale ? fabs(mat[i]) : scale;
  if (scale <= 2.2250738585072014e-308) scale = 1.0;
  double sm[9];
  for (int i = 0; i < 9; ++i) sm[i] = ddiv(mat[i], scale);
  double r[3];
  compute_roots(sm, r);
  sm[0] = dsub(sm[0], r[0]);
  sm[4] = dsub(sm[4], r[0]);
  sm[8] = dsub(sm[8], r[0]);
  double v1[3], v2[3], v3[3];
  cross3(&sm[0], &sm[3], v1);
  cross3(&sm[0], &sm[6], v2);
  cross3(&sm[3], &sm[6], v3);
  const double l1 = dadd(dadd(dmul(v1[0], v1[0]), dmul(v1[1], v1[1])), dmul(v1[2], v1[2]));
  const double l2 = dadd(dadd(dmul(v2[0], v2[0]), dmul(v2[1], v2[1])), dmul(v2[2], v2[2]));
  const double l3 = dadd(dadd(dmul(v3[0], v3[0]), dmul(v3[1], v3[1])), dmul(v3[2], v3[2]));
  const double* v;
  double l;
  if (l1 >= l2 && l1 >= l3) {
    v = v1;
    l = l1;
  } else if (l2 >= l1 && l2 >= l3) {
    v = v2;
    l = l2;
  } else {
    v = v3;
    l = l3;
  }
  const double s = __dsqrt_rn(l);
  evec[0] = ddiv(v[0], s);
  evec[1] = ddiv(v[1], s);
  evec[2] = ddiv(v[2], s);
}

__device__ bool plane_refine_model(const PlaneConst& pc, const double* sums, double cntd, float4& out) {
  if (cntd < 4.0) return false;
  double a[9];
#pragma unroll
  for (int k = 0; k < 9; ++k) a[k] = ddiv(sums[k], cntd);
  double cov[9];
  cov[0] = dsub(a[0], dmul(a[6], a[6]));
  cov[1] = dsub(a[1], dmul(a[6], a[7]));
  cov[2] = dsub(a[2], dmul(a[6], a[8]));
  cov[4] = dsub(a[3], dmul(a[7], a[7]));
  cov[5] = dsub(a[4], dmul(a[7], a[8]));
  cov[8] = dsub(a[5], dmul(a[8], a[8]));
  cov[3] = cov[1];
  cov[6] = cov[2];
  cov[7] = cov[5];
  double vec[3];
  eigen33_smallest(cov, vec);
  float4 o;
  o.x = (float)vec[0];
  o.y = (float)vec[1];
  o.z = (float)vec[2];
  const float cx = (float)a[6], cy = (float)a[7], cz = (float)a[8];
  o.w = -fadd(fadd(fmul(o.x, cx), fmul(o.y, cy)), fmul(o.z, cz));
  if (!model_valid(pc, o)) return false;
  out = o;
  return true;
}

__global__ void __launch_bounds__(32)
    k_plane_refine(PlaneFrame* __restrict__ pf, const double* __restrict__ partial, PlaneConst pc, int chunks) {
  const int f = blockIdx.x;
  PlaneFrame& P = pf[f];
  if (!P.active) return;
  if (!pc.optimize || !P.model_ok) return;
  const int lane = threadIdx.x;
  const int nch = cdiv(P.n, TS_CHUNK);
  double tot = 0.0;
  if (lane < 10) {
    const double* src = partial + (size_t)f * chunks * 10 + lane;
    for (int c = 0; c < nch; ++c) tot = dadd(tot, src[(size_t)c * 10]);
  }
  double a[9];
#pragma unroll
  for (int k = 0; k < 9; ++k) a[k] = __shfl_sync(FULL, tot, k);
  const double cntd = __shfl_sync(FULL, tot, 9);
  if (lane != 0) return;
  float4 o;
  if (plane_refine_model(pc, a, cntd, o)) P.coeff_ref = o;
}

template <int MINB>
__global__ void __launch_bounds__(CT_THREADS, MINB)
    k_plane_extract(const PlaneFrame* __restrict__ pf, const float4* __restrict__ in, size_t in_stride, BufPair bp,
                    float thr, int* __restrict__ inlier_idx, int* __restrict__ n_tmp, unsigned* __restrict__ desc, int cap,
                    int tiles) {
  const int f = blockIdx.x, tile = blockIdx.y;
  const PlaneFrame& P = pf[f];
  if (!P.active) return;
  const int n = P.n;
  if (tile * BT_TILE >= n) {
    if (tile == 0 && threadIdx.x == 0) n_tmp[f] = 0;
    return;
  }
  __shared__ CompactSmem sm;
  const float4* pts = cur_cloud(P, in, in_stride, bp.p, f, cap);
  const int* srcidx = (P.cur < 0) ? nullptr : (bp.s[P.cur] + (size_t)f * cap);
  const int dst = (P.cur < 0) ? 0 : (1 - P.cur);
  float4* dpts = bp.p[dst] + (size_t)f * cap;
  int* dsrc = bp.s[dst] + (size_t)f * cap;
  const float4 co = P.coeff_ref;
  const bool ok = P.model_ok != 0;
  unsigned keepmask = 0u;
#pragma unroll
  for (int k = 0; k < BT_ITEMS; ++k) {
    const int i = bt_index<BT_ITEMS>(tile, k);
    if (i < n) {
      const float4 p = __ldg(pts + i);
      const bool inl = ok && plane_dist(co, p.x, p.y, p.z) < thr;
      if (!inl) keepmask |= 1u << k;
    }
  }
  unsigned wbase;
  const unsigned incl_total = big_tile_scan<BT_ITEMS>(keepmask, desc + (size_t)f * tiles, tile, sm, wbase);
#pragma unroll
  for (int k = 0; k < BT_ITEMS; ++k) {
    const int i = bt_index<BT_ITEMS>(tile, k);
    const bool keep = (keepmask >> k) & 1u;
    const unsigned m = __ballot_sync(FULL, keep);
    const unsigned pos = wbase + __popc(m & lanemask_lt());
    if (keep) {
      dpts[pos] = __ldg(pts + i);
      dsrc[pos] = srcidx ? srcidx[i] : i;
    } else if (i < n && inlier_idx) {
      inlier_idx[(size_t)f * cap + (i - (int)pos)] = i;
    }
    wbase += __popc(m);
  }
  if ((tile + 1) * BT_TILE >= n && threadIdx.x == 0) n_tmp[f] = (int)incl_total;
}

__global__ void k_plane_update(PlaneFrame* __restrict__ pf, const int* __restrict__ n_tmp, double keep_fraction,
                               int* __restrict__ n_active, uint32_t* __restrict__ warnings, int B) {
  const int f = blockIdx.x * blockDim.x + threadIdx.x;
  if (f >= B) return;
  PlaneFrame& P = pf[f];
  if (!P.active) {
    atomicMax(n_active + 1, P.n);
    atomicAdd(n_active + 2, P.n);
    return;
  }
  const int remaining = n_tmp[f];
  const int inliers = P.n - remaining;
  P.n_inliers_last = inliers;
  if (inliers == 0) {
    P.active = 0;
    atomicOr(&warnings[f], (uint32_t)PCOP_WARN_PLANE_BREAK);
    atomicMax(n_active + 1, P.n);
    atomicAdd(n_active + 2, P.n);
    return;
  }
  if (P.n_passes < PCOP_MAX_PLANE_PASSES_RECORDED) {
    P.pass_points[P.n_passes] = P.n;
    P.pass_inliers[P.n_passes] = inliers;
    P.pass_coeff[P.n_passes] = P.coeff_ref;
  }
  P.n_passes += 1;
  P.cur = (P.cur < 0) ? 0 : (1 - P.cur);
  P.n = remaining;
  P.active = ((double)remaining > dmul(keep_fraction, (double)P.nr_points)) ? 1 : 0;
  if (P.active) atomicAdd(n_active, 1);
  atomicMax(n_active + 1, P.n);
  atomicAdd(n_active + 2, P.n);
}

__global__ void __launch_bounds__(CT_THREADS)
    k_plane_finalize(const PlaneFrame* __restrict__ pf, const float4* __restrict__ in, size_t in_stride, BufPair bp,
                     float4* __restrict__ out, int* __restrict__ out_src, int* __restrict__ n_out, int cap) {
  const int f = blockIdx.y, tile = blockIdx.x;
  const PlaneFrame& P = pf[f];
  const int n = P.n;
  if (tile == 0 && threadIdx.x == 0) n_out[f] = n;
  if (tile * CT_TILE >= n) return;
  const float4* pts = cur_cloud(P, in, in_stride, bp.p, f, cap);
  const int* srcidx = (P.cur < 0) ? nullptr : (bp.s[P.cur] + (size_t)f * cap);
#pragma unroll
  for (int k = 0; k < CT_ITEMS; ++k) {
    const int i = ct_index(tile, k);
    if (i < n) {
      out[(size_t)f * cap + i] = __ldg(pts + i);
      out_src[(size_t)f * cap + i] = srcidx ? srcidx[i] : i;
    }
  }
}


constexpr int PL_CL = 8;
constexpr int PL_MAX_THREADS = 1024;
constexpr int PL_MAX_WARPS = PL_MAX_THREADS / 32;
constexpr int PL_MAX_GROUPS = PL_MAX_THREADS / 256;
constexpr int PL_N_BATCHES = 3;
__constant__ const int PL_BATCH_END[PL_N_BATCHES] = {4, 8, MAX_HYP};

struct PlShared {
  float4 hyp[MAX_HYP];
  int hyp_valid[MAX_HYP];
  int cnt[MAX_HYP];
  int cnt_all[PL_CL][MAX_HYP];
  int kept_all[PL_CL];
  int warp_excl[PL_MAX_WARPS];
  double msh[PL_MAX_GROUPS][8][9];
  int mcnt[PL_MAX_GROUPS][8];
  double log_prob;
  float4 coeff_sel, coeff_ref;
  int model_ok, need_more, nh, gen_end;
};

template <int GROUPS>
__device__ __forceinline__ void group_bar_sync(int g) {
  if (g == 0) asm volatile("bar.sync 1, 256;" ::: "memory");
  else if (g == 1) asm volatile("bar.sync 2, 256;" ::: "memory");
  else if (GROUPS > 2 && g == 2) asm volatile("bar.sync 3, 256;" ::: "memory");
  else if (GROUPS > 2) asm volatile("bar.sync 4, 256;" ::: "memory");
}
__device__ __forceinline__ unsigned cluster_ctarank() {
  unsigned r;
  asm volatile("mov.u32 %0, %%cluster_ctarank;" : "=r"(r));
  return r;
}
__device__ __forceinline__ void cluster_sync_all() {
  asm volatile("barrier.cluster.arrive.release.aligned;\n\tbarrier.cluster.wait.acquire.aligned;" ::: "memory");
}
template <class T>
__device__ __forceinline__ T* dsmem_ptr(T* p, unsigned rank) {
  unsigned long long out;
  asm volatile("mapa.u64 %0, %1, %2;" : "=l"(out) : "l"((unsigned long long)p), "r"(rank));
  return reinterpret_cast<T*>(out);
}

__global__ void __launch_bounds__(32)
    k_plane_gen0(PlaneFrame* __restrict__ pf, const float4* __restrict__ in, size_t in_stride, const int* __restrict__ n_in,
                 int* __restrict__ n_in_copy, const int* __restrict__ rng, PlaneConst pc, uint32_t* __restrict__ warnings) {
  const int f = blockIdx.x;
  const int lane = threadIdx.x;
  PlaneFrame& P = pf[f];
  const int n = n_in[f];
  const int active = ((double)n > dmul(pc.keep_fraction, (double)n)) ? 1 : 0;
  if (lane == 0) {
    if (n_in_copy) n_in_copy[f] = n;
    P.cur = -1;
    P.nr_points = n;
    P.n = n;
    P.n_passes = 0;
    P.best = -1;
    P.model_ok = 0;
    P.need_more = 0;
    P.n_inliers_last = 0;
    P.coeff_sel = make_float4(0.f, 0.f, 0.f, 0.f);
    P.coeff_ref = make_float4(0.f, 0.f, 0.f, 0.f);
    P.active = active;
  }
  if (lane == 1) P.log_prob = det_log(dsub(1.0, pc.probability));
  for (int k = lane; k < PCOP_MAX_PLANE_PASSES_RECORDED; k += 32) {
    P.pass_points[k] = 0;
    P.pass_inliers[k] = 0;
    P.pass_coeff[k] = make_float4(0.f, 0.f, 0.f, 0.f);
  }
  int nh = 0, gen_end = 0;
  if (active) {
    __shared__ GenScratch G;
    plane_gen_warp(in + (size_t)f * in_stride, n, rng, pc, G, P.hyp, P.hyp_valid, nh, gen_end);
  }
  if (lane == 0) {
    P.n_hyp = nh;
    P.gen_end = gen_end;
    if (gen_end == 2) atomicOr(&warnings[f], (uint32_t)PCOP_WARN_RNG_TABLE_EXHAUSTED);
  }
}

template <int G, int THREADS>
__device__ __forceinline__ void pl_score(PlShared& S, const float* __restrict__ sx, const float* __restrict__ sy,
                                         const float* __restrict__ sz, int sn, float thr, int h_begin, int h_end) {
  const int lane = threadIdx.x & 31;
  for (int h0 = h_begin; h0 < h_end; h0 += G) {
    int c[G];
    float4 co[G];
#pragma unroll
    for (int j = 0; j < G; ++j) {
      c[j] = 0;
      co[j] = S.hyp[h0 + j];
    }
    for (int i = threadIdx.x; i < sn; i += THREADS) {
      const float x = sx[i], y = sy[i], z = sz[i];
#pragma unroll
      for (int j = 0; j < G; ++j) c[j] += (plane_dist(co[j], x, y, z) < thr) ? 1 : 0;
    }
#pragma unroll
    for (int j = 0; j < G; ++j) {
      const int s = __reduce_add_sync(FULL, c[j]);
      if (lane == 0 && s) atomicAdd(&S.cnt[h0 + j], s);
    }
  }
}

template <int THREADS>
__device__ __forceinline__ void pl_push_counts(PlShared& S, unsigned rank, int h_begin, int h_end) {
  const int nhh = h_end - h_begin;
  for (int k = threadIdx.x; k < PL_CL * nhh; k += THREADS) {
    const unsigned r = (unsigned)(k / nhh);
    const int h = h_begin + k % nhh;
    *dsmem_ptr(&S.cnt_all[rank][h], r) = S.cnt[h];
  }
}

__device__ __forceinline__ void pl_select(PlShared& S, const PlaneConst& pc, int n, int navail) {
  int sel = -1;
  const PlShared* Sp = &S;
  const bool more = plane_select_replay(pc, S.log_prob, n, S.nh, navail, S.hyp_valid,
                                        [Sp](int h) {
                                          int c = 0;
#pragma unroll
                                          for (int r = 0; r < PL_CL; ++r) c += Sp->cnt_all[r][h];
                                          return c;
                                        },
                                        sel);
  S.need_more = more ? 1 : 0;
  if (more) return;
  S.model_ok = (sel >= 0 && S.hyp_valid[sel]) ? 1 : 0;
  S.coeff_sel = (sel >= 0) ? S.hyp[sel] : make_float4(0.f, 0.f, 0.f, 0.f);
  S.coeff_ref = S.coeff_sel;
}

template <int THREADS>
__global__ void __cluster_dims__(PL_CL, 1, 1) __launch_bounds__(THREADS, THREADS == 512 ? 2 : 1)
    k_plane_loop(PlaneFrame* __restrict__ pf, const float4* __restrict__ in, size_t in_stride, BufPair bp, PlaneConst pc,
                 const int* __restrict__ rng, int* __restrict__ inlier_idx, float4* __restrict__ out,
                 int* __restrict__ out_src, int* __restrict__ n_out, uint32_t* __restrict__ warnings, int cap,
                 int slice_cap, int nch_max, int n_lo, int n_hi) {
  constexpr int PL_THREADS = THREADS, PL_WARPS = THREADS / 32, PL_GROUPS = THREADS / 256;
  const unsigned rank = cluster_ctarank();
  const int f = blockIdx.y;
  const int tid = threadIdx.x, lane = tid & 31, warp = tid >> 5;
  extern __shared__ __align__(16) unsigned char pl_smem[];
  PlShared& S = *reinterpret_cast<PlShared*>(pl_smem);
  double* part = reinterpret_cast<double*>(pl_smem + sizeof(PlShared));
  float* sx = reinterpret_cast<float*>(pl_smem + sizeof(PlShared) + (size_t)nch_max * 80);
  float* sy = sx + slice_cap;
  float* sz = sy + slice_cap;
  GenScratch& G = *reinterpret_cast<GenScratch*>(sx);

  PlaneFrame& P = pf[f];
  int n = P.n, cur = P.cur, active = P.active, n_passes = P.n_passes;
  const int nr = P.nr_points;
  if (n <= n_lo || n > n_hi) return;
  bool first = true;

  if (!active) {
    const float4* pts = in + (size_t)f * in_stride;
    for (int i = (int)rank * PL_THREADS + tid; i < n; i += PL_CL * PL_THREADS) {
      out[(size_t)f * cap + i] = __ldg(pts + i);
      out_src[(size_t)f * cap + i] = i;
    }
    if (rank == 0 && tid == 0) n_out[f] = n;
    return;
  }

  while (true) {
    PL_CLK(0);
    const float4* pts = (cur < 0) ? (in + (size_t)f * in_stride) : (bp.p[cur] + (size_t)f * cap);
    const int* srcidx = (cur < 0) ? nullptr : (bp.s[cur] + (size_t)f * cap);
    const int SL = min(slice_cap, cdiv(cdiv(n, PL_CL), TS_CHUNK) * TS_CHUNK);
    const int lo = min((int)rank * SL, n), hi = min(lo + SL, n), sn = hi - lo;
    {
      const bool fresh = !first;
      for (int i0 = tid; i0 < sn; i0 += 8 * PL_THREADS) {
        float4 p[8];
#pragma unroll
        for (int u = 0; u < 8; ++u) {
          const int i = i0 + u * PL_THREADS;
          p[u] = (i < sn) ? (fresh ? __ldcg(pts + lo + i) : __ldg(pts + lo + i)) : make_float4(0.f, 0.f, 0.f, 0.f);
        }
#pragma unroll
        for (int u = 0; u < 8; ++u) {
          const int i = i0 + u * PL_THREADS;
          if (i < sn) {
            sx[i] = p[u].x;
            sy[i] = p[u].y;
            sz[i] = p[u].z;
          }
        }
      }
    }
    if (first) {
      if (tid == 0) {
        S.nh = P.n_hyp;
        S.gen_end = P.gen_end;
        S.log_prob = P.log_prob;
      }
      if (tid < MAX_HYP) {
        S.hyp[tid] = P.hyp[tid];
        S.hyp_valid[tid] = P.hyp_valid[tid];
      }
      first = false;
    }
    __syncthreads();
    if (tid < MAX_HYP) {
      const float qnan = __uint_as_float(0x7fc00000u);
      if (tid >= S.nh) S.hyp[tid] = make_float4(qnan, qnan, qnan, qnan);
      S.cnt[tid] = 0;
    }
    __syncthreads();
    const int nh = S.nh;
    PL_CLK(1);

    for (int ph = 0, scored = 0; ph < PL_N_BATCHES; ++ph) {
      const int end = PL_BATCH_END[ph];
      if (end - scored <= 4) pl_score<4, PL_THREADS>(S, sx, sy, sz, sn, pc.thr, scored, min(nh, end));
      else pl_score<8, PL_THREADS>(S, sx, sy, sz, sn, pc.thr, scored, min(nh, end));
      __syncthreads();
      pl_push_counts<PL_THREADS>(S, rank, scored, end);
      PL_CLK(2);
      cluster_sync_all();
      PL_CLK(3);
      if (tid == 0) pl_select(S, pc, n, end);
      __syncthreads();
      PL_CLK(4);
      if (!S.need_more) break;
      scored = end;
    }
    const bool ok = S.model_ok != 0;
    PL_CLK(5);

    if (pc.optimize && ok) {
      const float4 co = S.coeff_sel;
      const int g = tid >> 8, t = tid & 255, gw = (tid >> 5) & 7;
      const int nlc = cdiv(sn, TS_CHUNK);
      const int gc0 = lo / TS_CHUNK;
      for (int lc = g; lc < nlc; lc += PL_GROUPS) {
        double a[9];
#pragma unroll
        for (int k = 0; k < 9; ++k) a[k] = 0.0;
        int cnt = 0;
#pragma unroll
        for (int r = 0; r < TS_CHUNK / 256; ++r) {
          const int i = lc * TS_CHUNK + r * 256 + t;
          double e[9];
#pragma unroll
          for (int k = 0; k < 9; ++k) e[k] = 0.0;
          if (i < sn) {
            const float px = sx[i], py = sy[i], pz = sz[i];
            if (plane_dist(co, px, py, pz) < pc.thr) {
              const double x = px, y = py, z = pz;
              e[0] = dmul(x, x);
              e[1] = dmul(x, y);
              e[2] = dmul(x, z);
              e[3] = dmul(y, y);
              e[4] = dmul(y, z);
              e[5] = dmul(z, z);
              e[6] = x;
              e[7] = y;
              e[8] = z;
              ++cnt;
            }
          }
#pragma unroll
          for (int k = 0; k < 9; ++k) a[k] = dadd(a[k], e[k]);
        }
#pragma unroll
        for (int k = 0; k < 9; ++k) a[k] = tree_butterfly(a[k]);
        cnt = __reduce_add_sync(FULL, cnt);
        if (lane == 0) {
#pragma unroll
          for (int k = 0; k < 9; ++k) S.msh[g][gw][k] = a[k];
          S.mcnt[g][gw] = cnt;
        }
        group_bar_sync<PL_GROUPS>(g);
        double* o = part + (size_t)(gc0 + lc) * 10;
        if (t < 9) {
          double s = S.msh[g][0][t];
          for (int w = 1; w < 8; ++w) s = dadd(s, S.msh[g][w][t]);
          o[t] = s;
        } else if (t == 9) {
          int c = 0;
          for (int w = 0; w < 8; ++w) c += S.mcnt[g][w];
          o[9] = (double)c;
        }
        group_bar_sync<PL_GROUPS>(g);
      }
      __syncthreads();
      const int nv = nlc * 10;
      for (int k = tid; k < (PL_CL - 1) * nv; k += PL_THREADS) {
        const unsigned r = (rank + 1u + (unsigned)(k / nv)) % PL_CL;
        double* mine = part + (size_t)gc0 * 10 + k % nv;
        *dsmem_ptr(mine, r) = *mine;
      }
      PL_CLK(6);
      cluster_sync_all();
      PL_CLK(7);
      if (warp == 0) {
        const int nch = cdiv(n, TS_CHUNK);
        double tot = 0.0;
        if (lane < 10)
          for (int c = 0; c < nch; ++c) tot = dadd(tot, part[(size_t)c * 10 + lane]);
        double a[9];
#pragma unroll
        for (int k = 0; k < 9; ++k) a[k] = __shfl_sync(FULL, tot, k);
        const double cntd = __shfl_sync(FULL, tot, 9);
        if (lane == 0) {
          float4 o;
          if (plane_refine_model(pc, a, cntd, o)) S.coeff_ref = o;
        }
      }
      __syncthreads();
    }

    PL_CLK(8);
    const float4 co = S.coeff_ref;
    const int per_warp = cdiv(cdiv(sn, PL_WARPS), 32) * 32;
    const int rows = per_warp / 32;
    const int wb = warp * per_warp;
    unsigned keepmask = 0u;
    for (int r = 0; r < rows; ++r) {
      const int i = wb + r * 32 + lane;
      if (i < sn) {
        const bool inl = ok && plane_dist(co, sx[i], sy[i], sz[i]) < pc.thr;
        if (!inl) keepmask |= 1u << r;
      }
    }
    const unsigned wtotal = __reduce_add_sync(FULL, (unsigned)__popc(keepmask));
    if (lane == 0) S.warp_excl[warp] = (int)wtotal;
    __syncthreads();
    if (warp == 0) {
      const int v = (lane < PL_WARPS) ? S.warp_excl[lane] : 0;
      int incl = v;
#pragma unroll
      for (int o = 1; o < 32; o <<= 1) {
        const int up = __shfl_up_sync(FULL, incl, o);
        if (lane >= o) incl += up;
      }
      if (lane < PL_WARPS) S.warp_excl[lane] = incl - v;
      const int total = __shfl_sync(FULL, incl, 31);
      if (lane < PL_CL) *dsmem_ptr(&S.kept_all[rank], (unsigned)lane) = total;
// ... 194 lines not shown
```

### pointcloud_obstacle_processing_b200/csrc/stage_voxel_part.cu

```cuda
#include <cmath>
#include <cstddef>
#include <cstdlib>

#include "internal.cuh"
#include "primitives.cuh"

namespace pcop {
#ifdef PCOP_VP_DEBUG_CLK
__device__ long long g_vp_reduce_clk[16];
#define VP_CLK(k)                                                                          \
  do {                                                                                     \
    if (blockIdx.x == 5 && blockIdx.y == 20 && threadIdx.x == 0) g_vp_reduce_clk[k] = clock64(); \
  } while (0)
#else
#define VP_CLK(k) \
  do {            \
  } while (0)
#endif

namespace {

constexpr int VP_THREADS = 256;
constexpr int VP_WARPS = VP_THREADS / 32;
constexpr int VP_NB_MAX = 16384;
constexpr int VP_MAX_CHUNKS = 8;
constexpr int VP_EMAX = 2048;
constexpr int VPR_THREADS = 512;
constexpr int VPR_WARPS = VPR_THREADS / 32;
constexpr int VP_EPT = VP_EMAX / VPR_THREADS;
constexpr int VP_BITMAP_WORDS = 4096;
constexpr int VP_KMAX = 256;
constexpr int VP_SCAN_THREADS = 512;
constexpr int VP_SCAN_WARPS = VP_SCAN_THREADS / 32;
constexpr int VP_MAX_ROUNDS = VP_NB_MAX / 32;

__device__ __forceinline__ bool vp_keep(const float4 p, const VoxFusedPlan& pl) {
  return !((p.x != p.x) || p.x < pl.lim[0] || p.x > pl.lim[1] || p.z < pl.lim[4] || p.z > pl.lim[5] || p.y < pl.lim[2] ||
           p.y > pl.lim[3]);
}
__device__ __forceinline__ uint32_t vp_key(float x, float y, float z, const VoxFusedPlan& pl) {
  const int cx = __float2int_rz(floorf(fmul(x, pl.inv))) - pl.b0[0];
  const int cy = __float2int_rz(floorf(fmul(y, pl.inv))) - pl.b0[1];
  const int cz = __float2int_rz(floorf(fmul(z, pl.inv))) - pl.b0[2];
  return (uint32_t)cx + pl.nx * ((uint32_t)cy + pl.ny * (uint32_t)cz);
}
__device__ __forceinline__ void vp_chunk(int n, int chunks, int c, int& i0, int& i1) {
  const int cs = cdiv(cdiv(n, chunks), 4 * VP_THREADS) * (4 * VP_THREADS);
  i0 = min(c * cs, n);
  i1 = min(i0 + cs, n);
}

constexpr int VP_CHUNK_TAIL = 8;

template <bool NEED_MINMAX>
__global__ void __launch_bounds__(VP_THREADS)
    k_vp_hist(const float4* __restrict__ in, size_t in_stride, const int* __restrict__ n_in, VoxFusedPlan pl,
              uint32_t* __restrict__ ghist, int chunks) {
  const int c = blockIdx.x, f = blockIdx.y;
  extern __shared__ uint32_t vp_sh[];
  __shared__ float shmm[VP_WARPS][6];
  const int nwords = pl.nb_pad >> 1;
  for (int w = threadIdx.x; w < nwords; w += VP_THREADS) vp_sh[w] = 0u;
  __syncthreads();
  const int n = n_in[f];
  int i0, i1;
  vp_chunk(n, chunks, c, i0, i1);
  const float4* src = in + (size_t)f * in_stride;
  float mn[3] = {3.402823466e+38f, 3.402823466e+38f, 3.402823466e+38f};
  float mx[3] = {-3.402823466e+38f, -3.402823466e+38f, -3.402823466e+38f};
  bool odd = false;
  for (int b0 = i0 + threadIdx.x; b0 < i1; b0 += 4 * VP_THREADS) {
    float4 p[4];
#pragma unroll
    for (int u = 0; u < 4; ++u) {
      const int i = b0 + u * VP_THREADS;
      const float qnan = __uint_as_float(0x7fc00000u);
      p[u] = (i < i1) ? __ldg(src + i) : make_float4(qnan, 0.f, 0.f, 0.f);
    }
#pragma unroll
    for (int u = 0; u < 4; ++u) {
      if (vp_keep(p[u], pl)) {
        odd = odd || !(fabsf(p[u].y) <= 3.0e38f) || !(fabsf(p[u].z) <= 3.0e38f);
        if (NEED_MINMAX) {
          const float v[3] = {p[u].x, p[u].y, p[u].z};
#pragma unroll
          for (int a = 0; a < 3; ++a) {
            if (v[a] < mn[a]) mn[a] = v[a];
            if (v[a] > mx[a]) mx[a] = v[a];
          }
        }
        const uint32_t bucket = min(vp_key(p[u].x, p[u].y, p[u].z, pl) >> pl.part_shift, (uint32_t)pl.nb - 1u);
        atomicAdd(&vp_sh[bucket >> 1], 1u << ((bucket & 1u) * 16u));
      }
    }
  }
  const int any_odd = __syncthreads_or(odd ? 1 : 0);
  uint32_t* gh = ghist + ((size_t)f * chunks + c) * (nwords + VP_CHUNK_TAIL);
  if (NEED_MINMAX) {
#pragma unroll
    for (int a = 0; a < 3; ++a) {
#pragma unroll
      for (int o = 16; o >= 1; o >>= 1) {
        mn[a] = fminf(mn[a], __shfl_xor_sync(FULL, mn[a], o));
        mx[a] = fmaxf(mx[a], __shfl_xor_sync(FULL, mx[a], o));
      }
    }
    if (lane_id() == 0) {
#pragma unroll
      for (int a = 0; a < 3; ++a) {
        shmm[warp_id()][a] = mn[a];
        shmm[warp_id()][3 + a] = mx[a];
      }
    }
    __syncthreads();
    if (threadIdx.x < 6) {
      const int a = threadIdx.x;
      float v = shmm[0][a];
      for (int w = 1; w < VP_WARPS; ++w) v = (a < 3) ? fminf(v, shmm[w][a]) : fmaxf(v, shmm[w][a]);
      gh[nwords + a] = __float_as_uint(v);
    }
  }
  if (threadIdx.x == 6) gh[nwords + 6] = any_odd ? 1u : 0u;
  for (int w = threadIdx.x; w < nwords; w += VP_THREADS) gh[w] = vp_sh[w];
}

__device__ void vp_setup_one(const float (&mnv)[3], const float (&mxv)[3], float leaf, VoxelFrame* __restrict__ vf, int f) {
  VoxelFrame v;
  v.inv = fdiv(1.0f, leaf);
  unsigned div_b[3];
#pragma unroll
  for (int a = 0; a < 3; ++a) {
    v.min_b[a] = cvt_f2i(floorf(fmul(mnv[a], v.inv)));
    const int max_b = cvt_f2i(floorf(fmul(mxv[a], v.inv)));
    div_b[a] = (unsigned)max_b - (unsigned)v.min_b[a] + 1u;
  }
  v.overflow = 0;
  v.mul1 = div_b[0];
  v.mul2 = div_b[0] * div_b[1];
  vf[f] = v;
}

__device__ __forceinline__ unsigned warp_incl_scan(unsigned v) {
  const int lane = lane_id();
#pragma unroll
  for (int o = 1; o < 32; o <<= 1) {
    const unsigned up = __shfl_up_sync(FULL, v, o);
    if (lane >= o) v += up;
  }
  return v;
}

template <int PER>
__device__ __forceinline__ unsigned warp0_excl_scan(uint32_t* a, int n) {
  const int lane = lane_id();
  unsigned v[PER];
  unsigned sum = 0u;
#pragma unroll
  for (int j = 0; j < PER; ++j) {
    const int i = lane * PER + j;
    v[j] = (i < n) ? a[i] : 0u;
    sum += v[j];
  }
  const unsigned incl = warp_incl_scan(sum);
  unsigned run = incl - sum;
#pragma unroll
  for (int j = 0; j < PER; ++j) {
    const int i = lane * PER + j;
    if (i < n) a[i] = run;
    run += v[j];
  }
  return __shfl_sync(FULL, incl, 31);
}

__device__ __forceinline__ void vp_unpack4(const uint2 w, unsigned (&v)[4]) {
  v[0] = w.x & 0xffffu;
  v[1] = w.x >> 16;
  v[2] = w.y & 0xffffu;
  v[3] = w.y >> 16;
}
__device__ __forceinline__ void vp_bucket_totals4(const unsigned short* gh16, size_t chunk_stride16, int chunks, int b0,
                                                  unsigned (&t)[4]) {
#pragma unroll
  for (int k = 0; k < 4; ++k) t[k] = 0u;
#pragma unroll
  for (int c = 0; c < VP_MAX_CHUNKS; ++c) {
    if (c < chunks) {
      unsigned v[4];
      vp_unpack4(*reinterpret_cast<const uint2*>(gh16 + (size_t)c * chunk_stride16 + b0), v);
#pragma unroll
      for (int k = 0; k < 4; ++k) t[k] += v[k];
    }
  }
}

__global__ void __launch_bounds__(VP_SCAN_THREADS, 2)
    k_vp_scan(const uint32_t* __restrict__ ghist, uint32_t* __restrict__ chunk_start, unsigned short* __restrict__ ne_bucket,
              uint32_t* __restrict__ ne_start,
              uint2* __restrict__ grec, int* __restrict__ n_groups, int* __restrict__ n_crop,
              uint32_t* __restrict__ flags, uint32_t* __restrict__ warnings, float leaf, VoxelFrame* __restrict__ vf,
              VoxFusedPlan pl, int chunks, int want_keys, int gmax, int gstride) {
  const int f = blockIdx.x, tid = threadIdx.x, lane = lane_id(), warp = warp_id();
  __shared__ uint32_t s_rt[VP_MAX_ROUNDS / 4 + 1];
  __shared__ uint32_t s_rn[VP_MAX_ROUNDS / 4 + 1];
  __shared__ unsigned s_total[2];
  const int nwords = pl.nb_pad >> 1;
  const uint32_t* gh = ghist + (size_t)f * chunks * (nwords + VP_CHUNK_TAIL);
  const size_t chunk_stride16 = 2 * (size_t)(nwords + VP_CHUNK_TAIL);
  const unsigned short* gh16 = reinterpret_cast<const unsigned short*>(gh);
  if (tid == 0) {
    float mnv[3] = {3.402823466e+38f, 3.402823466e+38f, 3.402823466e+38f};
    float mxv[3] = {-3.402823466e+38f, -3.402823466e+38f, -3.402823466e+38f};
    uint32_t odd = 0u;
    for (int c = 0; c < chunks; ++c) {
      const uint32_t* tail = gh + (size_t)c * (nwords + VP_CHUNK_TAIL) + nwords;
      odd |= tail[6];
      if (want_keys) {
#pragma unroll
        for (int a = 0; a < 3; ++a) {
          mnv[a] = fminf(mnv[a], __uint_as_float(tail[a]));
          mxv[a] = fmaxf(mxv[a], __uint_as_float(tail[3 + a]));
        }
      }
    }
    flags[f] = odd;
    if (warnings) warnings[f] = 0u;
    if (want_keys) vp_setup_one(mnv, mxv, leaf, vf, f);
  }
  __syncthreads();
  uint32_t* cs_out = chunk_start + (size_t)f * chunks * pl.nb_pad;
  unsigned short* ne_out = ne_bucket + (size_t)f * VP_NB_MAX;
  uint32_t* ns_out = ne_start + (size_t)f * (VP_NB_MAX + 1);
  const int nrounds = (pl.nb_pad + 127) >> 7;
  bool too_big = false;
  for (int r = warp; r < nrounds; r += VP_SCAN_WARPS) {
    const int b0 = 128 * r + 4 * lane;
    unsigned t[4] = {0u, 0u, 0u, 0u};
    if (b0 < pl.nb_pad) vp_bucket_totals4(gh16, chunk_stride16, chunks, b0, t);
    unsigned nz = 0u;
#pragma unroll
    for (int k = 0; k < 4; ++k) {
      too_big = too_big || t[k] > (unsigned)VP_EMAX;
      nz += (t[k] != 0u) ? 1u : 0u;
    }
    const unsigned sum = __reduce_add_sync(FULL, t[0] + t[1] + t[2] + t[3]);
    const unsigned ne = __reduce_add_sync(FULL, nz);
    if (lane == 0) {
      s_rt[r] = sum;
      s_rn[r] = ne;
    }
  }
  if (too_big) atomicOr(&flags[f], 2u);
  __syncthreads();
  if (warp == 0) {
    const unsigned m = warp0_excl_scan<(VP_MAX_ROUNDS / 4 + 31) / 32>(s_rt, nrounds);
    const unsigned ne = warp0_excl_scan<(VP_MAX_ROUNDS / 4 + 31) / 32>(s_rn, nrounds);
    if (lane == 0) {
      s_total[0] = m;
      s_total[1] = ne;
      n_crop[f] = (int)m;
    }
  }
  __syncthreads();
  const unsigned M = s_total[0];
  const int NE = (int)s_total[1];
  for (int r = warp; r < nrounds; r += VP_SCAN_WARPS) {
    const int b0 = 128 * r + 4 * lane;
    unsigned t[4] = {0u, 0u, 0u, 0u};
    const bool in_range = b0 < pl.nb_pad;
    if (in_range) vp_bucket_totals4(gh16, chunk_stride16, chunks, b0, t);
    const unsigned mine = t[0] + t[1] + t[2] + t[3];
    const unsigned incl = warp_incl_scan(mine);
    unsigned nz = 0u;
#pragma unroll
    for (int k = 0; k < 4; ++k) nz += (t[k] != 0u) ? 1u : 0u;
    const unsigned nz_incl = warp_incl_scan(nz);
    unsigned start[4];
    start[0] = s_rt[r] + incl - mine;
    start[1] = start[0] + t[0];
    start[2] = start[1] + t[1];
    start[3] = start[2] + t[2];
    if (in_range) {
      unsigned run[4] = {start[0], start[1], start[2], start[3]};
#pragma unroll
      for (int c = 0; c < chunks; ++c) {
        *reinterpret_cast<uint4*>(cs_out + (size_t)c * pl.nb_pad + b0) = make_uint4(run[0], run[1], run[2], run[3]);
        unsigned v[4];
        vp_unpack4(*reinterpret_cast<const uint2*>(gh16 + (size_t)c * chunk_stride16 + b0), v);
#pragma unroll
        for (int k = 0; k < 4; ++k) run[k] += v[k];
      }
      unsigned o = s_rn[r] + nz_incl - nz;
#pragma unroll
      for (int k = 0; k < 4; ++k) {
        if (t[k] != 0u) {
          ne_out[o] = (unsigned short)(b0 + k);
          ns_out[o] = start[k];
          ++o;
        }
      }
    }
  }
  if (tid == 0) ns_out[NE] = M;
  __syncthreads();
  if (warp != 0) return;
  const int K = min(VP_KMAX, (VP_BITMAP_WORDS * 32) >> pl.part_shift);
  uint2* gf = grec + (size_t)f * gstride;
  int ng = 0;
  if (NE > 0) {
    unsigned gs = 0u;
    int go = 0;
    if (lane == 0) gf[0] = make_uint2(0u, 0u);
    ng = 1;
    for (int base = 0; base < NE; base += 32) {
      const int o = base + lane;
      const unsigned st = (o < NE) ? ns_out[o] : 0u, en = (o < NE) ? ns_out[o + 1] : 0u;
      while (true) {
        const bool breaks = (o < NE) && (o > go) && (en - gs > (unsigned)VP_EMAX || o - go >= K);
        const unsigned m = __ballot_sync(FULL, breaks);
        if (!m) break;
        const int l = __ffs(m) - 1;
        go = base + l;
        gs = __shfl_sync(FULL, st, l);
        if (lane == 0 && ng < gmax) gf[ng] = make_uint2(gs, (unsigned)go);
        ++ng;
      }
    }
  }
  if (lane == 0) {
    n_groups[f] = ng;
    if (ng <= gmax) gf[ng] = make_uint2(M, (unsigned)NE);
    else atomicOr(&flags[f], 4u);
  }
}

constexpr int VPS_THREADS = 512;
__global__ void __launch_bounds__(VPS_THREADS)
    k_vp_scatter(const float4* __restrict__ in, size_t in_stride, const int* __restrict__ n_in, VoxFusedPlan pl,
                 const uint32_t* __restrict__ chunk_start, const uint32_t* __restrict__ flags, float4* __restrict__ part,
                 int cap, int chunks) {
  const int c = blockIdx.x, f = blockIdx.y;
  if (flags[f]) return;
  extern __shared__ uint32_t vp_sh[];
  const uint32_t* cs = chunk_start + ((size_t)f * chunks + c) * pl.nb_pad;
  for (int b = threadIdx.x; b < pl.nb_pad; b += VPS_THREADS) vp_sh[b] = cs[b];
  __syncthreads();
  const int n = n_in[f];
  int i0, i1;
  vp_chunk(n, chunks, c, i0, i1);
  const float4* src = in + (size_t)f * in_stride;
  float4* dst = part + (size_t)f * cap;
  const float qnan = __uint_as_float(0x7fc00000u);
  float4 nxt[4];
#pragma unroll
  for (int u = 0; u < 4; ++u) {
    const int i = i0 + threadIdx.x + u * VPS_THREADS;
    nxt[u] = (i < i1) ? __ldg(src + i) : make_float4(qnan, 0.f, 0.f, 0.f);
  }
  for (int b0 = i0 + threadIdx.x; b0 < i1; b0 += 4 * VPS_THREADS) {
    float4 p[4];
#pragma unroll
    for (int u = 0; u < 4; ++u) {
      p[u] = nxt[u];
      const int i = b0 + (4 + u) * VPS_THREADS;
      nxt[u] = (i < i1) ? __ldg(src + i) : make_float4(qnan, 0.f, 0.f, 0.f);
    }
#pragma unroll
    for (int u = 0; u < 4; ++u) {
      if (vp_keep(p[u], pl)) {
        const uint32_t bucket = vp_key(p[u].x, p[u].y, p[u].z, pl) >> pl.part_shift;
        const uint32_t pos = atomicAdd(&vp_sh[bucket], 1u);
        dst[pos] = make_float4(p[u].x, p[u].y, p[u].z, __int_as_float(b0 + u * VPS_THREADS));
      }
    }
  }
}

constexpr int VP_ORD_TAB = 1024;

struct alignas(16) VpReduceSmem {
  uint32_t bitmap[VP_BITMAP_WORDS];
  unsigned short wprefix[VP_BITMAP_WORDS];
  uint32_t rbase[VP_BITMAP_WORDS / 128 + 4];
  uint32_t start[VP_EMAX + 4];
  uint32_t srt[VP_EMAX / 128 + 1];
  int sidx[VP_EMAX];
  float sx[VP_EMAX], sy[VP_EMAX], sz[VP_EMAX];
  uint32_t bkt_start[VP_KMAX + 1];
  unsigned short bkt_id[VP_KMAX];
  unsigned char ord_tab[VP_ORD_TAB];
  unsigned vbase, nvox;
};

static_assert(offsetof(VpReduceSmem, start) % 16 == 0 && offsetof(VpReduceSmem, wprefix) % 8 == 0, "vector accesses");

__device__ __forceinline__ unsigned vp_round_scan(const unsigned (&c)[4], unsigned& total) {
  const unsigned mine = c[0] + c[1] + c[2] + c[3];
  const unsigned incl = warp_incl_scan(mine);
  total = __shfl_sync(FULL, incl, 31);
  return incl - mine;
}

template <bool WITH_KEYS>
__global__ void __launch_bounds__(VPR_THREADS, 3)
    k_vp_reduce(const float4* __restrict__ part, const uint32_t* __restrict__ ne_start,
                const unsigned short* __restrict__ ne_bucket, const uint2* __restrict__ grec,
                const int* __restrict__ n_groups, const uint32_t* __restrict__ flags, VoxFusedPlan pl,
                const VoxelFrame* __restrict__ vf, float4* __restrict__ out, uint32_t* __restrict__ out_keys,
                int* __restrict__ n_out, unsigned* __restrict__ desc, int cap, int gstride) {
  const int f = blockIdx.x, g = blockIdx.y;
  const int tid = threadIdx.x, lane = lane_id(), warp = warp_id();
  const int ng = n_groups[f];
  const uint32_t declined = flags[f];
  const uint2 r0 = grec[(size_t)f * gstride + g], r1 = grec[(size_t)f * gstride + g + 1];
  if (declined || g >= ng) {
    if (g == 0 && tid == 0) n_out[f] = 0;
    return;
  }
  VP_CLK(0);
  extern __shared__ __align__(16) unsigned char vp_raw[];
  VpReduceSmem& sm = *reinterpret_cast<VpReduceSmem*>(vp_raw);
  const uint32_t e0 = r0.x;
  const int E = (int)(r1.x - r0.x);
  const int o0 = (int)r0.y, KB = (int)(r1.y - r0.y);
  const float4* src = part + (size_t)f * cap + e0;
  float4 p[VP_EPT];
#pragma unroll
  for (int k = 0; k < VP_EPT; ++k) {
    const int e = tid + k * VPR_THREADS;
    p[k] = (e < E) ? __ldg(src + e) : make_float4(0.f, 0.f, 0.f, 0.f);
  }
  const int S = pl.part_shift;
  const int wpb = (1 << S) >> 5;
  const int nwords = KB * wpb;
  int my_bucket = 0;
  if (tid < KB) {
    my_bucket = ne_bucket[(size_t)f * VP_NB_MAX + o0 + tid];
    sm.bkt_id[tid] = (unsigned short)my_bucket;
  }
  if (tid <= KB) sm.bkt_start[tid] = ne_start[(size_t)f * (VP_NB_MAX + 1) + o0 + tid];
  for (int w = 4 * tid; w < nwords; w += 4 * VPR_THREADS)
    *reinterpret_cast<uint4*>(&sm.bitmap[w]) = make_uint4(0u, 0u, 0u, 0u);
  for (int v = 4 * tid; v < E + 4; v += 4 * VPR_THREADS) *reinterpret_cast<uint4*>(&sm.start[v]) = make_uint4(0u, 0u, 0u, 0u);
  __syncthreads();
  const int b_first = sm.bkt_id[0];
  const bool direct = (int)sm.bkt_id[KB - 1] - b_first < VP_ORD_TAB;
  if (direct && tid < KB) sm.ord_tab[my_bucket - b_first] = (unsigned char)tid;
  __syncthreads();
  VP_CLK(1);

  uint32_t slot[VP_EPT];
#pragma unroll
  for (int k = 0; k < VP_EPT; ++k) {
    const int e = tid + k * VPR_THREADS;
    slot[k] = 0u;
    if (e < E) {
      const uint32_t key = vp_key(p[k].x, p[k].y, p[k].z, pl);
      int ord;
      if (direct) {
        ord = sm.ord_tab[(int)(key >> S) - b_first];
      } else {
        int lo = 0, hi = KB - 1;
        const uint32_t pos = e0 + (uint32_t)e;
        while (lo < hi) {
          const int mid = (lo + hi + 1) >> 1;
          if (sm.bkt_start[mid] <= pos) lo = mid;
          else hi = mid - 1;
        }
        ord = lo;
      }
      const uint32_t s = ((uint32_t)ord << S) | (key & ((1u << S) - 1u));
      slot[k] = s;
      atomicOr(&sm.bitmap[s >> 5], 1u << (s & 31u));
    }
  }
  __syncthreads();
  VP_CLK(2);
  const int nr = cdiv(nwords, 128);
  for (int r = warp; r < nr; r += VPR_WARPS) {
    const int w = 128 * r + 4 * lane;
    const uint4 bw = (w < nwords) ? *reinterpret_cast<const uint4*>(&sm.bitmap[w]) : make_uint4(0u, 0u, 0u, 0u);
    const unsigned c[4] = {(unsigned)__popc(bw.x), (unsigned)__popc(bw.y), (unsigned)__popc(bw.z), (unsigned)__popc(bw.w)};
    unsigned total;
    const unsigned ex = vp_round_scan(c, total);
    if (w < nwords) {
      const unsigned a0 = ex, a1 = a0 + c[0], a2 = a1 + c[1], a3 = a2 + c[2];
      *reinterpret_cast<uint2*>(&sm.wprefix[w]) = make_uint2(a0 | (a1 << 16), a2 | (a3 << 16));
    }
    if (lane == 0) sm.rbase[r] = total;
  }
  __syncthreads();
  if (warp == 0) {
    const unsigned v = warp0_excl_scan<1>(sm.rbase, nr);
    if (lane == 0) sm.nvox = v;
  }
  __syncthreads();
  const int V = (int)sm.nvox;
  unsigned* dd = desc + (size_t)f * gstride;
  if (tid == 0) st_volatile_u32(dd + g, ((g == 0) ? LB_PREFIX : LB_AGG) | (unsigned)V);
  VP_CLK(3);
#pragma unroll
  for (int k = 0; k < VP_EPT; ++k) {
    const int e = tid + k * VPR_THREADS;
    if (e < E) {
      const uint32_t s = slot[k];
      const uint32_t r = sm.rbase[s >> 12] + (uint32_t)sm.wprefix[s >> 5] +
                         (uint32_t)__popc(sm.bitmap[s >> 5] & ((1u << (s & 31u)) - 1u));
      const uint32_t j = atomicAdd(&sm.start[r], 1u);
      slot[k] = (r << 16) | j;
    }
  }
  __syncthreads();
  VP_CLK(4);
  {
    const int vr = cdiv(V, 128);
    unsigned keep[4] = {0u, 0u, 0u, 0u};
    int my_r = -1;
    for (int r = warp; r < vr; r += VPR_WARPS) {
      const int v = 128 * r + 4 * lane;
      const uint4 cw = *reinterpret_cast<const uint4*>(&sm.start[v]);
      const unsigned c[4] = {cw.x, cw.y, cw.z, cw.w};
      unsigned total;
      const unsigned ex = vp_round_scan(c, total);
      keep[0] = ex;
      keep[1] = ex + c[0];
      keep[2] = keep[1] + c[1];
      keep[3] = keep[2] + c[2];
      my_r = r;
      if (lane == 0) sm.srt[r] = total;
    }
    __syncthreads();
    if (warp == 0) warp0_excl_scan<1>(sm.srt, vr);
    __syncthreads();
    if (my_r >= 0) {
      const unsigned base = sm.srt[my_r];
      const int v = 128 * my_r + 4 * lane;
      *reinterpret_cast<uint4*>(&sm.start[v]) = make_uint4(base + keep[0], base + keep[1], base + keep[2], base + keep[3]);
    }
    __syncthreads();
    if (tid == 0) sm.start[V] = (unsigned)E;
  }
  __syncthreads();
  VP_CLK(5);
#pragma unroll
  for (int k = 0; k < VP_EPT; ++k) {
    const int e = tid + k * VPR_THREADS;
    if (e < E) sm.sidx[sm.start[slot[k] >> 16] + (slot[k] & 0xffffu)] = __float_as_int(p[k].w);
  }
  __syncthreads();
  VP_CLK(6);
#pragma unroll
  for (int k = 0; k < VP_EPT; ++k) {
    const int e = tid + k * VPR_THREADS;
    if (e < E) {
      const uint32_t r = slot[k] >> 16;
      const int s0 = (int)sm.start[r], cnt = (int)sm.start[r + 1] - s0;
      int rank = (int)(slot[k] & 0xffffu);
      if (cnt > 2) {
        const int mine = __float_as_int(p[k].w);
        rank = 0;
        for (int t = 0; t < cnt; ++t) rank += (sm.sidx[s0 + t] < mine) ? 1 : 0;
      }
      sm.sx[s0 + rank] = p[k].x;
      sm.sy[s0 + rank] = p[k].y;
      sm.sz[s0 + rank] = p[k].z;
    }
  }
  __syncthreads();
  VP_CLK(7);
  VoxelFrame vfr;
  float fb0 = 0.f, fb1 = 0.f, fb2 = 0.f;
  if (WITH_KEYS) {
    vfr = vf[f];
    fb0 = (float)vfr.min_b[0];
    fb1 = (float)vfr.min_b[1];
    fb2 = (float)vfr.min_b[2];
  }
  constexpr int VPT = VP_EMAX / VPR_THREADS;
  float4 cen[VPT];
  uint32_t vkey[VPT];
#pragma unroll
  for (int k = 0; k < VPT; ++k) {
    const int v = tid + k * VPR_THREADS;
    cen[k] = make_float4(0.f, 0.f, 0.f, 1.0f);
    vkey[k] = 0u;
    if (v < V) {
      const int s0 = (int)sm.start[v], s1 = (int)sm.start[v + 1];
      float ax = 0.0f, ay = 0.0f, az = 0.0f;
      for (int t = s0; t < s1; ++t) {
        ax = fadd(ax, sm.sx[t]);
        ay = fadd(ay, sm.sy[t]);
        az = fadd(az, sm.sz[t]);
      }
      const float c = (float)(s1 - s0);
      cen[k] = (s1 - s0 == 1) ? make_float4(ax, ay, az, 1.0f) : make_float4(fdiv(ax, c), fdiv(ay, c), fdiv(az, c), 1.0f);
      if (WITH_KEYS) {
        const int i0 = cvt_f2i(fsub(floorf(fmul(sm.sx[s0], vfr.inv)), fb0));
        const int i1 = cvt_f2i(fsub(floorf(fmul(sm.sy[s0], vfr.inv)), fb1));
        const int i2 = cvt_f2i(fsub(floorf(fmul(sm.sz[s0], vfr.inv)), fb2));
        vkey[k] = (uint32_t)i0 + (uint32_t)i1 * vfr.mul1 + (uint32_t)i2 * vfr.mul2;
      }
    }
  }
  if (warp == 0 && g > 0) {
    unsigned excl = 0u;
    int look = g - 1;
    while (true) {
      const int idx = look - lane;
      unsigned d = LB_PREFIX;
      if (idx >= 0) {
        d = lookback_wait(dd + idx);
      }
      const unsigned is_prefix = __ballot_sync(FULL, (d >> 30) == 2u);
      const int first = is_prefix ? (__ffs(is_prefix) - 1) : 31;
      unsigned v = (lane <= first) ? (d & LB_VALUE) : 0u;
      v = __reduce_add_sync(FULL, v);
      excl += v;
      if (is_prefix) break;
      look -= 32;
    }
    if (lane == 0) {
      st_volatile_u32(dd + g, LB_PREFIX | (excl + (unsigned)V));
      sm.vbase = excl;
    }
  } else if (tid == 0 && g == 0) {
    sm.vbase = 0u;
  }
  __syncthreads();
  VP_CLK(8);
  const unsigned vbase = sm.vbase;
  if (g == ng - 1 && tid == 0) n_out[f] = (int)(vbase + (unsigned)V);
#pragma unroll
  for (int k = 0; k < VPT; ++k) {
    const int v = tid + k * VPR_THREADS;
    if (v < V) {
      const size_t o = (size_t)f * cap + vbase + (unsigned)v;
      out[o] = cen[k];
      if (WITH_KEYS) out_keys[o] = vkey[k];
    }
  }
  VP_CLK(9);
}

}

void vox_part_plan(VoxFusedPlan& pl, size_t max_points) {
  pl.part_ok = 0;
  if (!pl.ok) return;
  if (max_points > (size_t)VP_MAX_CHUNKS * 61440) return;
  int lg = 0;
  while (((size_t)1 << lg) < max_points) ++lg;
  const int nbits = std::min(14, std::max(8, lg - 3));
  const int shift = std::max(5, pl.bits - nbits);
  if (pl.bits - shift > 14 || shift > 16) return;
  const unsigned long long total = (unsigned long long)pl.nx * pl.ny * pl.nz;
  pl.part_shift = shift;
  pl.nb = (int)((total + (1ull << shift) - 1) >> shift);
  if (pl.nb < 1) pl.nb = 1;
  if (pl.nb > VP_NB_MAX) return;
  pl.nb_pad = (pl.nb + 31) & ~31;
  pl.part_ok = 1;
}

int vox_part_chunks(int max_n, int B) {
  const int per = (B < 32) ? 12288 : 24576;
  return std::max(1, std::min(VP_MAX_CHUNKS, max_n / per));
}
int vox_part_group_bound(const VoxFusedPlan& pl, int max_n) {
  const int K = std::min(VP_KMAX, (VP_BITMAP_WORDS * 32) >> pl.part_shift);
  const int ne = std::min(pl.nb, max_n);
  const long long b = 2ll * max_n / VP_EMAX + ne / K + 3;
  return (int)std::min<long long>(b, 65535);
}
size_t vox_part_hist_elems(int B) { return (size_t)B * VP_MAX_CHUNKS * (VP_NB_MAX / 2 + VP_CHUNK_TAIL); }
size_t vox_part_start_elems(int B) { return (size_t)B * (VP_NB_MAX + 1); }
size_t vox_part_chunk_start_elems(int B) { return (size_t)B * VP_MAX_CHUNKS * VP_NB_MAX; }
size_t vox_part_bucket_elems(int B) { return (size_t)B * VP_NB_MAX; }

void run_voxel_part(const Ctx& c, const VoxelPartArgs& a) {
  const VoxFusedPlan& pl = a.plan;
  const int chunks = vox_part_chunks(c.grid_cap, c.B);
  const int gmax = std::max(1, std::min(a.group_launch, a.group_stride - 1));
  cudaMemsetAsync(a.desc, 0, (size_t)c.B * a.group_stride * sizeof(unsigned), c.stream);
  const size_t hsm = (size_t)(pl.nb_pad / 2) * sizeof(uint32_t);
  if (a.want_keys)
    KL(c, "k_vp_hist", k_vp_hist<true><<<dim3(chunks, c.B), VP_THREADS, hsm, c.stream>>>(a.in, a.in_stride, a.n_in, pl, a.ghist,
                                                                                        chunks));
  else
    KL(c, "k_vp_hist", k_vp_hist<false><<<dim3(chunks, c.B), VP_THREADS, hsm, c.stream>>>(a.in, a.in_stride, a.n_in, pl, a.ghist,
                                                                                         chunks));
  KL(c, "k_vp_scan", k_vp_scan<<<c.B, VP_SCAN_THREADS, 0, c.stream>>>(a.ghist, a.chunk_start, a.ne_bucket, a.ne_start, a.grec, a.n_groups,
                                                                      a.n_crop, a.flags, a.warnings, a.leaf, a.vf, pl, chunks,
                                                                      a.want_keys, gmax, a.group_stride));
  const size_t ssm = (size_t)pl.nb_pad * sizeof(uint32_t);
  cudaFuncSetAttribute(k_vp_scatter, cudaFuncAttributeMaxDynamicSharedMemorySize, (int)ssm);
  KL(c, "k_vp_scatter", k_vp_scatter<<<dim3(chunks, c.B), VPS_THREADS, ssm, c.stream>>>(a.in, a.in_stride, a.n_in, pl, a.chunk_start,
                                                                                       a.flags, a.part, c.cap, chunks));
  const size_t rsm = sizeof(VpReduceSmem);
  if (a.want_keys) {
    cudaFuncSetAttribute(k_vp_reduce<true>, cudaFuncAttributeMaxDynamicSharedMemorySize, (int)rsm);
    KL(c, "k_vp_reduce", k_vp_reduce<true><<<dim3(c.B, gmax), VPR_THREADS, rsm, c.stream>>>(
                             a.part, a.ne_start, a.ne_bucket, a.grec, a.n_groups, a.flags, pl, a.vf, a.out, a.out_keys,
                             a.n_out, a.desc, c.cap, a.group_stride));
  } else {
    cudaFuncSetAttribute(k_vp_reduce<false>, cudaFuncAttributeMaxDynamicSharedMemorySize, (int)rsm);
    KL(c, "k_vp_reduce", k_vp_reduce<false><<<dim3(c.B, gmax), VPR_THREADS, rsm, c.stream>>>(
                             a.part, a.ne_start, a.ne_bucket, a.grec, a.n_groups, a.flags, pl, a.vf, a.out, a.out_keys,
                             a.n_out, a.desc, c.cap, a.group_stride));
  }
  count_launch(c, 4);
}

}

#ifdef PCOP_VP_DEBUG_CLK
extern "C" int pcop_debug_vp_reduce_cycles(long long* out16) {
  return (int)cudaMemcpyFromSymbol(out16, pcop::g_vp_reduce_clk, sizeof(long long) * 16);
}
#endif
```

Baseline: 21.67 billion.

## Fuse voxel partition hist/scan/scatter into one cluster kernel using DSMEM

Replaces the three-kernel voxel partition pipeline (per-chunk histogram to global, per-frame scan, scatter) and a memset with a single thread-block-cluster kernel. Each CTA of a frame's cluster keeps its bucket counts in shared memory, and the prefix offsets are computed across CTAs through distributed shared memory. The global histogram and chunk-start buffers go away, which removes launches and global round trips. In exchange, every chunk of a frame must be co-scheduled as one cluster of up to 8 CTAs with larger shared memory per CTA. The chunk count heuristic also stops depending on batch size, so large batches now get more chunks.

```diff
diff --git a/pointcloud_obstacle_processing_b200/csrc/internal.cuh b/pointcloud_obstacle_processing_b200/csrc/internal.cuh
--- a/pointcloud_obstacle_processing_b200/csrc/internal.cuh
+++ b/pointcloud_obstacle_processing_b200/csrc/internal.cuh
@@ -143,9 +143,7 @@
 
 int vox_part_chunks(int max_n, int B);
 int vox_part_group_bound(const VoxFusedPlan& pl, int max_n);
-size_t vox_part_hist_elems(int B);
 size_t vox_part_start_elems(int B);
-size_t vox_part_chunk_start_elems(int B);
 size_t vox_part_bucket_elems(int B);
 struct VoxelPartArgs {
   const float4* in;
@@ -155,8 +153,6 @@
   float leaf;
   MinMax* minmax;
   VoxelFrame* vf;
-  uint32_t* ghist;
-  uint32_t* chunk_start;
   unsigned short* ne_bucket;
   uint32_t* ne_start;
   uint2* grec;
diff --git a/pointcloud_obstacle_processing_b200/csrc/pcop_api.cu b/pointcloud_obstacle_processing_b200/csrc/pcop_api.cu
--- a/pointcloud_obstacle_processing_b200/csrc/pcop_api.cu
+++ b/pointcloud_obstacle_processing_b200/csrc/pcop_api.cu
@@ -202,8 +202,6 @@
   int vox_redo = -1;
   bool vox_full_groups = false;
   bool wave_used_fused = false;
-  uint32_t* d_vp_hist = nullptr;
-  uint32_t* d_vp_bstart = nullptr;
   uint32_t* d_vp_nstart = nullptr;
   unsigned short* d_vp_ne = nullptr;
   uint2* d_vp_grec = nullptr;
@@ -866,8 +864,6 @@
     a.leaf = p.downsample_size;
     a.minmax = h->d_minmax;
     a.vf = h->d_vf;
-    a.ghist = h->d_vp_hist;
-    a.chunk_start = h->d_vp_bstart;
     a.ne_bucket = h->d_vp_ne;
     a.ne_start = h->d_vp_nstart;
     a.grec = h->d_vp_grec;
@@ -1698,8 +1694,6 @@
   if (h->vplan.part_ok) {
     h->vp_gstride = vox_part_group_bound(h->vplan, h->cap) + 1;
     h->vp_group_hint = h->vp_gstride - 1;
-    A(dalloc(h, &h->d_vp_hist, vox_part_hist_elems(B)));
-    A(dalloc(h, &h->d_vp_bstart, vox_part_chunk_start_elems(B)));
     A(dalloc(h, &h->d_vp_nstart, vox_part_start_elems(B)));
     A(dalloc(h, &h->d_vp_ne, vox_part_bucket_elems(B)));
     A(dalloc(h, &h->d_vp_grec, (size_t)B * h->vp_gstride));
diff --git a/pointcloud_obstacle_processing_b200/csrc/primitives.cuh b/pointcloud_obstacle_processing_b200/csrc/primitives.cuh
--- a/pointcloud_obstacle_processing_b200/csrc/primitives.cuh
+++ b/pointcloud_obstacle_processing_b200/csrc/primitives.cuh
@@ -6,6 +6,21 @@
 __device__ __forceinline__ int lane_id() { return threadIdx.x & 31; }
 __device__ __forceinline__ int warp_id() { return threadIdx.x >> 5; }
 __device__ __forceinline__ unsigned lanemask_lt() { return (1u << (threadIdx.x & 31)) - 1u; }
+
+__device__ __forceinline__ unsigned cluster_ctarank() {
+  unsigned r;
+  asm volatile("mov.u32 %0, %%cluster_ctarank;" : "=r"(r));
+  return r;
+}
+__device__ __forceinline__ void cluster_sync_all() {
+  asm volatile("barrier.cluster.arrive.release.aligned;\n\tbarrier.cluster.wait.acquire.aligned;" ::: "memory");
+}
+template <class T>
+__device__ __forceinline__ T* dsmem_ptr(T* p, unsigned rank) {
+  unsigned long long out;
+  asm volatile("mapa.u64 %0, %1, %2;" : "=l"(out) : "l"((unsigned long long)p), "r"(rank));
+  return reinterpret_cast<T*>(out);
+}
 
 __device__ __forceinline__ unsigned ld_volatile_u32(const unsigned* p) {
   unsigned v;
diff --git a/pointcloud_obstacle_processing_b200/csrc/stage_plane.cu b/pointcloud_obstacle_processing_b200/csrc/stage_plane.cu
--- a/pointcloud_obstacle_processing_b200/csrc/stage_plane.cu
+++ b/pointcloud_obstacle_processing_b200/csrc/stage_plane.cu
@@ -745,21 +745,6 @@
   else if (GROUPS > 2 && g == 2) asm volatile("bar.sync 3, 256;" ::: "memory");
   else if (GROUPS > 2) asm volatile("bar.sync 4, 256;" ::: "memory");
 }
-__device__ __forceinline__ unsigned cluster_ctarank() {
-  unsigned r;
-  asm volatile("mov.u32 %0, %%cluster_ctarank;" : "=r"(r));
-  return r;
-}
-__device__ __forceinline__ void cluster_sync_all() {
-  asm volatile("barrier.cluster.arrive.release.aligned;\n\tbarrier.cluster.wait.acquire.aligned;" ::: "memory");
-}
-template <class T>
-__device__ __forceinline__ T* dsmem_ptr(T* p, unsigned rank) {
-  unsigned long long out;
-  asm volatile("mapa.u64 %0, %1, %2;" : "=l"(out) : "l"((unsigned long long)p), "r"(rank));
-  return reinterpret_cast<T*>(out);
-}
-
 __global__ void __launch_bounds__(32)
     k_plane_gen0(PlaneFrame* __restrict__ pf, const float4* __restrict__ in, size_t in_stride, const int* __restrict__ n_in,
                  int* __restrict__ n_in_copy, const int* __restrict__ rng, PlaneConst pc, uint32_t* __restrict__ warnings) {
diff --git a/pointcloud_obstacle_processing_b200/csrc/stage_voxel_part.cu b/pointcloud_obstacle_processing_b200/csrc/stage_voxel_part.cu
--- a/pointcloud_obstacle_processing_b200/csrc/stage_voxel_part.cu
+++ b/pointcloud_obstacle_processing_b200/csrc/stage_voxel_part.cu
@@ -20,8 +20,6 @@
 
 namespace {
 
-constexpr int VP_THREADS = 256;
-constexpr int VP_WARPS = VP_THREADS / 32;
 constexpr int VP_NB_MAX = 16384;
 constexpr int VP_MAX_CHUNKS = 8;
 constexpr int VP_EMAX = 2048;
@@ -30,9 +28,6 @@
 constexpr int VP_EPT = VP_EMAX / VPR_THREADS;
 constexpr int VP_BITMAP_WORDS = 4096;
 constexpr int VP_KMAX = 256;
-constexpr int VP_SCAN_THREADS = 512;
-constexpr int VP_SCAN_WARPS = VP_SCAN_THREADS / 32;
-constexpr int VP_MAX_ROUNDS = VP_NB_MAX / 32;
 
 __device__ __forceinline__ bool vp_keep(const float4 p, const VoxFusedPlan& pl) {
   return !((p.x != p.x) || p.x < pl.lim[0] || p.x > pl.lim[1] || p.z < pl.lim[4] || p.z > pl.lim[5] || p.y < pl.lim[2] ||
@@ -44,37 +39,176 @@
   const int cz = __float2int_rz(floorf(fmul(z, pl.inv))) - pl.b0[2];
   return (uint32_t)cx + pl.nx * ((uint32_t)cy + pl.ny * (uint32_t)cz);
 }
+constexpr int VP_CHUNK_ALIGN = 1024;
 __device__ __forceinline__ void vp_chunk(int n, int chunks, int c, int& i0, int& i1) {
-  const int cs = cdiv(cdiv(n, chunks), 4 * VP_THREADS) * (4 * VP_THREADS);
+  const int cs = cdiv(cdiv(n, chunks), VP_CHUNK_ALIGN) * VP_CHUNK_ALIGN;
   i0 = min(c * cs, n);
   i1 = min(i0 + cs, n);
 }
 
-constexpr int VP_CHUNK_TAIL = 8;
+__device__ void vp_setup_one(const float (&mnv)[3], const float (&mxv)[3], float leaf, VoxelFrame* __restrict__ vf, int f) {
+  VoxelFrame v;
+  v.inv = fdiv(1.0f, leaf);
+  unsigned div_b[3];
+#pragma unroll
+  for (int a = 0; a < 3; ++a) {
+    v.min_b[a] = cvt_f2i(floorf(fmul(mnv[a], v.inv)));
+    const int max_b = cvt_f2i(floorf(fmul(mxv[a], v.inv)));
+    div_b[a] = (unsigned)max_b - (unsigned)v.min_b[a] + 1u;
+  }
+  v.overflow = 0;
+  v.mul1 = div_b[0];
+  v.mul2 = div_b[0] * div_b[1];
+  vf[f] = v;
+}
+
+template <class T>
+__device__ __forceinline__ T warp_incl_scan(T v) {
+  const int lane = lane_id();
+#pragma unroll
+  for (int o = 1; o < 32; o <<= 1) {
+    const T up = __shfl_up_sync(FULL, v, o);
+    if (lane >= o) v += up;
+  }
+  return v;
+}
+
+template <int PER>
+__device__ __forceinline__ unsigned warp0_excl_scan(uint32_t* a, int n) {
+  const int lane = lane_id();
+  unsigned v[PER];
+  unsigned sum = 0u;
+#pragma unroll
+  for (int j = 0; j < PER; ++j) {
+    const int i = lane * PER + j;
+    v[j] = (i < n) ? a[i] : 0u;
+    sum += v[j];
+  }
+  const unsigned incl = warp_incl_scan(sum);
+  unsigned run = incl - sum;
+#pragma unroll
+  for (int j = 0; j < PER; ++j) {
+    const int i = lane * PER + j;
+    if (i < n) a[i] = run;
+    run += v[j];
+  }
+  return __shfl_sync(FULL, incl, 31);
+}
+
+__device__ __forceinline__ void vp_unpack4(const uint2 w, unsigned (&v)[4]) {
+  v[0] = w.x & 0xffffu;
+  v[1] = w.x >> 16;
+  v[2] = w.y & 0xffffu;
+  v[3] = w.y >> 16;
+}
+__device__ __forceinline__ void vp_bucket_totals4(const uint32_t* cnt, int chunks, int q, unsigned (&t)[4]) {
+#pragma unroll
+  for (int k = 0; k < 4; ++k) t[k] = 0u;
+#pragma unroll
+  for (int c = 0; c < VP_MAX_CHUNKS; ++c) {
+    if (c < chunks) {
+      unsigned v[4];
+      vp_unpack4(*dsmem_ptr(reinterpret_cast<const uint2*>(cnt) + q, (unsigned)c), v);
+#pragma unroll
+      for (int k = 0; k < 4; ++k) t[k] += v[k];
+    }
+  }
+}
+
+struct VpSlice {
+  uint32_t m;
+  uint32_t ne;
+  uint32_t flags;
+  float mn[3], mx[3];
+};
+constexpr int VP_SLICE_WORDS = sizeof(VpSlice) / sizeof(uint32_t);
+
+using u64 = unsigned long long;
+
+constexpr int VPP_THREADS = 512;
+constexpr int VPP_WARPS = VPP_THREADS / 32;
+
+struct VpPartSmem {
+  VpSlice rec[VP_MAX_CHUNKS];
+  VpSlice mine;
+  float shmm[VPP_WARPS][6];
+  u64 wsum[2][VPP_WARPS];
+};
+
+__device__ __forceinline__ void vp_build_groups(const uint32_t* ns, int NE, unsigned M, int part_shift, uint2* gf,
+                                                int* n_groups, uint32_t* flags, int gmax) {
+  const int lane = lane_id();
+  const int K = min(VP_KMAX, (VP_BITMAP_WORDS * 32) >> part_shift);
+  constexpr int AHEAD = 4;
+  int ng = 0;
+  if (NE > 0) {
+    unsigned gs = 0u;
+    int go = 0;
+    if (lane == 0) gf[0] = make_uint2(0u, 0u);
+    ng = 1;
+    for (int base0 = 0; base0 < NE; base0 += 32 * AHEAD) {
+      unsigned st[AHEAD], en[AHEAD];
+#pragma unroll
+      for (int j = 0; j < AHEAD; ++j) {
+        const int o = base0 + 32 * j + lane;
+        st[j] = (o < NE) ? __ldcg(ns + o) : 0u;
+        en[j] = (o < NE) ? __ldcg(ns + o + 1) : 0u;
+      }
+#pragma unroll
+      for (int j = 0; j < AHEAD; ++j) {
+        const int base = base0 + 32 * j;
+        const int o = base + lane;
+        while (true) {
+          const bool breaks = (o < NE) && (o > go) && (en[j] - gs > (unsigned)VP_EMAX || o - go >= K);
+          const unsigned m = __ballot_sync(FULL, breaks);
+          if (!m) break;
+          const int l = __ffs(m) - 1;
+          go = base + l;
+          gs = __shfl_sync(FULL, st[j], l);
+          if (lane == 0 && ng < gmax) gf[ng] = make_uint2(gs, (unsigned)go);
+          ++ng;
+        }
+      }
+    }
+  }
+  if (lane == 0) {
+    *n_groups = ng;
+    if (ng <= gmax) gf[ng] = make_uint2(M, (unsigned)NE);
+    else atomicOr(flags, 4u);
+  }
+}
 
 template <bool NEED_MINMAX>
-__global__ void __launch_bounds__(VP_THREADS)
-    k_vp_hist(const float4* __restrict__ in, size_t in_stride, const int* __restrict__ n_in, VoxFusedPlan pl,
-              uint32_t* __restrict__ ghist, int chunks) {
-  const int c = blockIdx.x, f = blockIdx.y;
-  extern __shared__ uint32_t vp_sh[];
-  __shared__ float shmm[VP_WARPS][6];
+__global__ void __launch_bounds__(VPP_THREADS, 2)
+    k_vp_part(const float4* __restrict__ in, size_t in_stride, const int* __restrict__ n_in, VoxFusedPlan pl,
+              float4* __restrict__ part, int cap, unsigned short* __restrict__ ne_bucket, uint32_t* __restrict__ ne_start,
+              uint2* __restrict__ grec, int* __restrict__ n_groups, int* __restrict__ n_crop, uint32_t* __restrict__ flags,
+              uint32_t* __restrict__ warnings, float leaf, VoxelFrame* __restrict__ vf, unsigned* __restrict__ desc,
+              int gmax, int gstride) {
+  const int r = blockIdx.x, f = blockIdx.y, C = gridDim.x;
+  const int tid = threadIdx.x, lane = lane_id(), warp = warp_id();
+  extern __shared__ __align__(16) uint32_t vp_sh[];
   const int nwords = pl.nb_pad >> 1;
-  for (int w = threadIdx.x; w < nwords; w += VP_THREADS) vp_sh[w] = 0u;
+  uint32_t* cnt = vp_sh;
+  uint32_t* cur = vp_sh + nwords;
+  __shared__ VpPartSmem s;
+
+  for (int w = tid; w < nwords; w += VPP_THREADS) cnt[w] = 0u;
+  if (tid == 0) s.mine.m = s.mine.ne = s.mine.flags = 0u;
   __syncthreads();
   const int n = n_in[f];
   int i0, i1;
-  vp_chunk(n, chunks, c, i0, i1);
+  vp_chunk(n, C, r, i0, i1);
   const float4* src = in + (size_t)f * in_stride;
+  const float qnan = __uint_as_float(0x7fc00000u);
   float mn[3] = {3.402823466e+38f, 3.402823466e+38f, 3.402823466e+38f};
   float mx[3] = {-3.402823466e+38f, -3.402823466e+38f, -3.402823466e+38f};
   bool odd = false;
-  for (int b0 = i0 + threadIdx.x; b0 < i1; b0 += 4 * VP_THREADS) {
+  for (int b0 = i0 + tid; b0 < i1; b0 += 4 * VPP_THREADS) {
     float4 p[4];
 #pragma unroll
     for (int u = 0; u < 4; ++u) {
-      const int i = b0 + u * VP_THREADS;
-      const float qnan = __uint_as_float(0x7fc00000u);
+      const int i = b0 + u * VPP_THREADS;
       p[u] = (i < i1) ? __ldg(src + i) : make_float4(qnan, 0.f, 0.f, 0.f);
     }
 #pragma unroll
@@ -90,12 +224,11 @@
           }
         }
         const uint32_t bucket = min(vp_key(p[u].x, p[u].y, p[u].z, pl) >> pl.part_shift, (uint32_t)pl.nb - 1u);
-        atomicAdd(&vp_sh[bucket >> 1], 1u << ((bucket & 1u) * 16u));
+        atomicAdd(&cnt[bucket >> 1], 1u << ((bucket & 1u) * 16u));
       }
     }
   }
   const int any_odd = __syncthreads_or(odd ? 1 : 0);
-  uint32_t* gh = ghist + ((size_t)f * chunks + c) * (nwords + VP_CHUNK_TAIL);
   if (NEED_MINMAX) {
 #pragma unroll
     for (int a = 0; a < 3; ++a) {
@@ -105,271 +238,156 @@
         mx[a] = fmaxf(mx[a], __shfl_xor_sync(FULL, mx[a], o));
       }
     }
-    if (lane_id() == 0) {
+    if (lane == 0) {
 #pragma unroll
       for (int a = 0; a < 3; ++a) {
-        shmm[warp_id()][a] = mn[a];
-        shmm[warp_id()][3 + a] = mx[a];
+        s.shmm[warp][a] = mn[a];
+        s.shmm[warp][3 + a] = mx[a];
       }
     }
     __syncthreads();
-    if (threadIdx.x < 6) {
-      const int a = threadIdx.x;
-      float v = shmm[0][a];
-      for (int w = 1; w < VP_WARPS; ++w) v = (a < 3) ? fminf(v, shmm[w][a]) : fmaxf(v, shmm[w][a]);
-      gh[nwords + a] = __float_as_uint(v);
-    }
-  }
-  if (threadIdx.x == 6) gh[nwords + 6] = any_odd ? 1u : 0u;
-  for (int w = threadIdx.x; w < nwords; w += VP_THREADS) gh[w] = vp_sh[w];
-}
-
-__device__ void vp_setup_one(const float (&mnv)[3], const float (&mxv)[3], float leaf, VoxelFrame* __restrict__ vf, int f) {
-  VoxelFrame v;
-  v.inv = fdiv(1.0f, leaf);
-  unsigned div_b[3];
-#pragma unroll
-  for (int a = 0; a < 3; ++a) {
-    v.min_b[a] = cvt_f2i(floorf(fmul(mnv[a], v.inv)));
-    const int max_b = cvt_f2i(floorf(fmul(mxv[a], v.inv)));
-    div_b[a] = (unsigned)max_b - (unsigned)v.min_b[a] + 1u;
-  }
-  v.overflow = 0;
-  v.mul1 = div_b[0];
-  v.mul2 = div_b[0] * div_b[1];
-  vf[f] = v;
-}
-
-__device__ __forceinline__ unsigned warp_incl_scan(unsigned v) {
-  const int lane = lane_id();
-#pragma unroll
-  for (int o = 1; o < 32; o <<= 1) {
-    const unsigned up = __shfl_up_sync(FULL, v, o);
-    if (lane >= o) v += up;
-  }
-  return v;
-}
-
-template <int PER>
-__device__ __forceinline__ unsigned warp0_excl_scan(uint32_t* a, int n) {
-  const int lane = lane_id();
-  unsigned v[PER];
-  unsigned sum = 0u;
-#pragma unroll
-  for (int j = 0; j < PER; ++j) {
-    const int i = lane * PER + j;
-    v[j] = (i < n) ? a[i] : 0u;
-    sum += v[j];
-  }
-  const unsigned incl = warp_incl_scan(sum);
-  unsigned run = incl - sum;
-#pragma unroll
-  for (int j = 0; j < PER; ++j) {
-    const int i = lane * PER + j;
-    if (i < n) a[i] = run;
-    run += v[j];
-  }
-  return __shfl_sync(FULL, incl, 31);
-}
-
-__device__ __forceinline__ void vp_unpack4(const uint2 w, unsigned (&v)[4]) {
-  v[0] = w.x & 0xffffu;
-  v[1] = w.x >> 16;
-  v[2] = w.y & 0xffffu;
-  v[3] = w.y >> 16;
-}
-__device__ __forceinline__ void vp_bucket_totals4(const unsigned short* gh16, size_t chunk_stride16, int chunks, int b0,
-                                                  unsigned (&t)[4]) {
-#pragma unroll
-  for (int k = 0; k < 4; ++k) t[k] = 0u;
-#pragma unroll
-  for (int c = 0; c < VP_MAX_CHUNKS; ++c) {
-    if (c < chunks) {
-      unsigned v[4];
-      vp_unpack4(*reinterpret_cast<const uint2*>(gh16 + (size_t)c * chunk_stride16 + b0), v);
-#pragma unroll
-      for (int k = 0; k < 4; ++k) t[k] += v[k];
-    }
-  }
-}
-
-__global__ void __launch_bounds__(VP_SCAN_THREADS, 2)
-    k_vp_scan(const uint32_t* __restrict__ ghist, uint32_t* __restrict__ chunk_start, unsigned short* __restrict__ ne_bucket,
-              uint32_t* __restrict__ ne_start,
-              uint2* __restrict__ grec, int* __restrict__ n_groups, int* __restrict__ n_crop,
-              uint32_t* __restrict__ flags, uint32_t* __restrict__ warnings, float leaf, VoxelFrame* __restrict__ vf,
-              VoxFusedPlan pl, int chunks, int want_keys, int gmax, int gstride) {
-  const int f = blockIdx.x, tid = threadIdx.x, lane = lane_id(), warp = warp_id();
-  __shared__ uint32_t s_rt[VP_MAX_ROUNDS / 4 + 1];
-  __shared__ uint32_t s_rn[VP_MAX_ROUNDS / 4 + 1];
-  __shared__ unsigned s_total[2];
-  const int nwords = pl.nb_pad >> 1;
-  const uint32_t* gh = ghist + (size_t)f * chunks * (nwords + VP_CHUNK_TAIL);
-  const size_t chunk_stride16 = 2 * (size_t)(nwords + VP_CHUNK_TAIL);
-  const unsigned short* gh16 = reinterpret_cast<const unsigned short*>(gh);
-  if (tid == 0) {
-    float mnv[3] = {3.402823466e+38f, 3.402823466e+38f, 3.402823466e+38f};
-    float mxv[3] = {-3.402823466e+38f, -3.402823466e+38f, -3.402823466e+38f};
-    uint32_t odd = 0u;
-    for (int c = 0; c < chunks; ++c) {
-      const uint32_t* tail = gh + (size_t)c * (nwords + VP_CHUNK_TAIL) + nwords;
-      odd |= tail[6];
-      if (want_keys) {
-#pragma unroll
-        for (int a = 0; a < 3; ++a) {
-          mnv[a] = fminf(mnv[a], __uint_as_float(tail[a]));
-          mxv[a] = fmaxf(mxv[a], __uint_as_float(tail[3 + a]));
-        }
-      }
-    }
-    flags[f] = odd;
-    if (warnings) warnings[f] = 0u;
-    if (want_keys) vp_setup_one(mnv, mxv, leaf, vf, f);
-  }
-  __syncthreads();
-  uint32_t* cs_out = chunk_start + (size_t)f * chunks * pl.nb_pad;
+    if (tid < 6) {
+      const int a = tid;
+      float v = s.shmm[0][a];
+      for (int w = 1; w < VPP_WARPS; ++w) v = (a < 3) ? fminf(v, s.shmm[w][a]) : fmaxf(v, s.shmm[w][a]);
+      if (a < 3) s.mine.mn[a] = v;
+      else s.mine.mx[a - 3] = v;
+    }
+  }
+  if (tid == 0 && any_odd) s.mine.flags = 1u;
+  cluster_sync_all();
+
+  const int nq = pl.nb_pad >> 2;
+  const int q0 = (int)((long long)nq * r / C), q1 = (int)((long long)nq * (r + 1) / C);
+  {
+    unsigned sum = 0u, nz = 0u;
+    bool too_big = false;
+    for (int q = q0 + tid; q < q1; q += VPP_THREADS) {
+      unsigned t[4];
+      vp_bucket_totals4(cnt, C, q, t);
+#pragma unroll
+      for (int k = 0; k < 4; ++k) {
+        too_big = too_big || t[k] > (unsigned)VP_EMAX;
+        nz += (t[k] != 0u) ? 1u : 0u;
+        sum += t[k];
+      }
+    }
+    sum = __reduce_add_sync(FULL, sum);
+    nz = __reduce_add_sync(FULL, nz);
+    const bool any_big = __any_sync(FULL, too_big);
+    if (lane == 0) {
+      if (sum) atomicAdd(&s.mine.m, sum);
+      if (nz) atomicAdd(&s.mine.ne, nz);
+      if (any_big) atomicOr(&s.mine.flags, 2u);
+    }
+  }
+  __syncthreads();
+  if (tid < C * VP_SLICE_WORDS) {
+    const int p = tid / VP_SLICE_WORDS, w = tid % VP_SLICE_WORDS;
+    *dsmem_ptr(reinterpret_cast<uint32_t*>(&s.rec[r]) + w, (unsigned)p) = reinterpret_cast<const uint32_t*>(&s.mine)[w];
+  }
+  cluster_sync_all();
+
+  unsigned M = 0u, NE = 0u, fl = 0u;
+  u64 base = 0ull;
+  for (int p = 0; p < C; ++p) {
+    if (p == r) base = ((u64)NE << 32) | M;
+    M += s.rec[p].m;
+    NE += s.rec[p].ne;
+    fl |= s.rec[p].flags;
+  }
   unsigned short* ne_out = ne_bucket + (size_t)f * VP_NB_MAX;
   uint32_t* ns_out = ne_start + (size_t)f * (VP_NB_MAX + 1);
-  const int nrounds = (pl.nb_pad + 127) >> 7;
-  bool too_big = false;
-  for (int r = warp; r < nrounds; r += VP_SCAN_WARPS) {
-    const int b0 = 128 * r + 4 * lane;
+  if (r == 0) {
+    if (tid == 0) {
+      n_crop[f] = (int)M;
+      flags[f] = fl;
+      if (warnings) warnings[f] = 0u;
+      if (NEED_MINMAX) {
+        float mnv[3], mxv[3];
+#pragma unroll
+        for (int a = 0; a < 3; ++a) {
+          mnv[a] = s.rec[0].mn[a];
+          mxv[a] = s.rec[0].mx[a];
+        }
+        for (int p = 1; p < C; ++p) {
+#pragma unroll
+          for (int a = 0; a < 3; ++a) {
+            mnv[a] = fminf(mnv[a], s.rec[p].mn[a]);
+            mxv[a] = fmaxf(mxv[a], s.rec[p].mx[a]);
+          }
+        }
+        vp_setup_one(mnv, mxv, leaf, vf, f);
+      }
+    }
+    for (int g = tid; g < gstride; g += VPP_THREADS) desc[(size_t)f * gstride + g] = 0u;
+  }
+  if (r == C - 1 && tid == 0) ns_out[NE] = M;
+  int par = 0;
+  for (int qb = q0; qb < q1; qb += VPP_THREADS) {
+    const int q = qb + tid;
+    const bool in_range = q < q1;
     unsigned t[4] = {0u, 0u, 0u, 0u};
-    if (b0 < pl.nb_pad) vp_bucket_totals4(gh16, chunk_stride16, chunks, b0, t);
+    if (in_range) vp_bucket_totals4(cnt, C, q, t);
     unsigned nz = 0u;
 #pragma unroll
-    for (int k = 0; k < 4; ++k) {
-      too_big = too_big || t[k] > (unsigned)VP_EMAX;
-      nz += (t[k] != 0u) ? 1u : 0u;
-    }
-    const unsigned sum = __reduce_add_sync(FULL, t[0] + t[1] + t[2] + t[3]);
-    const unsigned ne = __reduce_add_sync(FULL, nz);
-    if (lane == 0) {
-      s_rt[r] = sum;
-      s_rn[r] = ne;
-    }
-  }
-  if (too_big) atomicOr(&flags[f], 2u);
-  __syncthreads();
-  if (warp == 0) {
-    const unsigned m = warp0_excl_scan<(VP_MAX_ROUNDS / 4 + 31) / 32>(s_rt, nrounds);
-    const unsigned ne = warp0_excl_scan<(VP_MAX_ROUNDS / 4 + 31) / 32>(s_rn, nrounds);
-    if (lane == 0) {
-      s_total[0] = m;
-      s_total[1] = ne;
-      n_crop[f] = (int)m;
-    }
-  }
-  __syncthreads();
-  const unsigned M = s_total[0];
-  const int NE = (int)s_total[1];
-  for (int r = warp; r < nrounds; r += VP_SCAN_WARPS) {
-    const int b0 = 128 * r + 4 * lane;
-    unsigned t[4] = {0u, 0u, 0u, 0u};
-    const bool in_range = b0 < pl.nb_pad;
-    if (in_range) vp_bucket_totals4(gh16, chunk_stride16, chunks, b0, t);
-    const unsigned mine = t[0] + t[1] + t[2] + t[3];
-    const unsigned incl = warp_incl_scan(mine);
-    unsigned nz = 0u;
-#pragma unroll
     for (int k = 0; k < 4; ++k) nz += (t[k] != 0u) ? 1u : 0u;
-    const unsigned nz_incl = warp_incl_scan(nz);
-    unsigned start[4];
-    start[0] = s_rt[r] + incl - mine;
-    start[1] = start[0] + t[0];
-    start[2] = start[1] + t[1];
-    start[3] = start[2] + t[2];
+    const u64 mine = (u64)(t[0] + t[1] + t[2] + t[3]) | ((u64)nz << 32);
+    const u64 incl = warp_incl_scan(mine);
+    if (lane == 31) s.wsum[par][warp] = incl;
+    __syncthreads();
+    u64 before = base;
+    for (int w = 0; w < VPP_WARPS; ++w) {
+      const u64 x = s.wsum[par][w];
+      if (w < warp) before += x;
+      base += x;
+    }
+    par ^= 1;
     if (in_range) {
+      const u64 ex = before + incl - mine;
+      unsigned o = (unsigned)(ex >> 32);
+      unsigned start[4];
+      start[0] = (unsigned)ex;
+      start[1] = start[0] + t[0];
+      start[2] = start[1] + t[1];
+      start[3] = start[2] + t[2];
       unsigned run[4] = {start[0], start[1], start[2], start[3]};
-#pragma unroll
-      for (int c = 0; c < chunks; ++c) {
-        *reinterpret_cast<uint4*>(cs_out + (size_t)c * pl.nb_pad + b0) = make_uint4(run[0], run[1], run[2], run[3]);
+      for (int c = 0; c < C; ++c) {
+        *dsmem_ptr(reinterpret_cast<uint4*>(cur) + q, (unsigned)c) = make_uint4(run[0], run[1], run[2], run[3]);
         unsigned v[4];
-        vp_unpack4(*reinterpret_cast<const uint2*>(gh16 + (size_t)c * chunk_stride16 + b0), v);
+        vp_unpack4(*dsmem_ptr(reinterpret_cast<const uint2*>(cnt) + q, (unsigned)c), v);
 #pragma unroll
         for (int k = 0; k < 4; ++k) run[k] += v[k];
       }
-      unsigned o = s_rn[r] + nz_incl - nz;
 #pragma unroll
       for (int k = 0; k < 4; ++k) {
         if (t[k] != 0u) {
-          ne_out[o] = (unsigned short)(b0 + k);
+          ne_out[o] = (unsigned short)(4 * q + k);
           ns_out[o] = start[k];
           ++o;
         }
       }
     }
   }
-  if (tid == 0) ns_out[NE] = M;
-  __syncthreads();
-  if (warp != 0) return;
-  const int K = min(VP_KMAX, (VP_BITMAP_WORDS * 32) >> pl.part_shift);
-  uint2* gf = grec + (size_t)f * gstride;
-  int ng = 0;
-  if (NE > 0) {
-    unsigned gs = 0u;
-    int go = 0;
-    if (lane == 0) gf[0] = make_uint2(0u, 0u);
-    ng = 1;
-    for (int base = 0; base < NE; base += 32) {
-      const int o = base + lane;
-      const unsigned st = (o < NE) ? ns_out[o] : 0u, en = (o < NE) ? ns_out[o + 1] : 0u;
-      while (true) {
-        const bool breaks = (o < NE) && (o > go) && (en - gs > (unsigned)VP_EMAX || o - go >= K);
-        const unsigned m = __ballot_sync(FULL, breaks);
-        if (!m) break;
-        const int l = __ffs(m) - 1;
-        go = base + l;
-        gs = __shfl_sync(FULL, st, l);
-        if (lane == 0 && ng < gmax) gf[ng] = make_uint2(gs, (unsigned)go);
-        ++ng;
-      }
-    }
-  }
-  if (lane == 0) {
-    n_groups[f] = ng;
-    if (ng <= gmax) gf[ng] = make_uint2(M, (unsigned)NE);
-    else atomicOr(&flags[f], 4u);
-  }
-}
-
-constexpr int VPS_THREADS = 512;
-__global__ void __launch_bounds__(VPS_THREADS)
-    k_vp_scatter(const float4* __restrict__ in, size_t in_stride, const int* __restrict__ n_in, VoxFusedPlan pl,
-                 const uint32_t* __restrict__ chunk_start, const uint32_t* __restrict__ flags, float4* __restrict__ part,
-                 int cap, int chunks) {
-  const int c = blockIdx.x, f = blockIdx.y;
-  if (flags[f]) return;
-  extern __shared__ uint32_t vp_sh[];
-  const uint32_t* cs = chunk_start + ((size_t)f * chunks + c) * pl.nb_pad;
-  for (int b = threadIdx.x; b < pl.nb_pad; b += VPS_THREADS) vp_sh[b] = cs[b];
-  __syncthreads();
-  const int n = n_in[f];
-  int i0, i1;
-  vp_chunk(n, chunks, c, i0, i1);
-  const float4* src = in + (size_t)f * in_stride;
+  cluster_sync_all();
+
+  if (r == C - 1 && warp == 0)
+    vp_build_groups(ns_out, (int)NE, M, pl.part_shift, grec + (size_t)f * gstride, n_groups + f, flags + f, gmax);
+  if (fl) return;
   float4* dst = part + (size_t)f * cap;
-  const float qnan = __uint_as_float(0x7fc00000u);
-  float4 nxt[4];
-#pragma unroll
-  for (int u = 0; u < 4; ++u) {
-    const int i = i0 + threadIdx.x + u * VPS_THREADS;
-    nxt[u] = (i < i1) ? __ldg(src + i) : make_float4(qnan, 0.f, 0.f, 0.f);
-  }
-  for (int b0 = i0 + threadIdx.x; b0 < i1; b0 += 4 * VPS_THREADS) {
+  for (int b0 = i0 + tid; b0 < i1; b0 += 4 * VPP_THREADS) {
     float4 p[4];
 #pragma unroll
     for (int u = 0; u < 4; ++u) {
-      p[u] = nxt[u];
-      const int i = b0 + (4 + u) * VPS_THREADS;
-      nxt[u] = (i < i1) ? __ldg(src + i) : make_float4(qnan, 0.f, 0.f, 0.f);
+      const int i = b0 + u * VPP_THREADS;
+      p[u] = (i < i1) ? __ldg(src + i) : make_float4(qnan, 0.f, 0.f, 0.f);
     }
 #pragma unroll
     for (int u = 0; u < 4; ++u) {
       if (vp_keep(p[u], pl)) {
         const uint32_t bucket = vp_key(p[u].x, p[u].y, p[u].z, pl) >> pl.part_shift;
-        const uint32_t pos = atomicAdd(&vp_sh[bucket], 1u);
-        dst[pos] = make_float4(p[u].x, p[u].y, p[u].z, __int_as_float(b0 + u * VPS_THREADS));
+        const uint32_t pos = atomicAdd(&cur[bucket], 1u);
+        dst[pos] = make_float4(p[u].x, p[u].y, p[u].z, __int_as_float(b0 + u * VPP_THREADS));
       }
     }
   }
@@ -661,9 +679,8 @@
   pl.part_ok = 1;
 }
 
-int vox_part_chunks(int max_n, int B) {
-  const int per = (B < 32) ? 12288 : 24576;
-  return std::max(1, std::min(VP_MAX_CHUNKS, max_n / per));
+int vox_part_chunks(int max_n, int ) {
+  return std::max(1, std::min(VP_MAX_CHUNKS, max_n / 12288));
 }
 int vox_part_group_bound(const VoxFusedPlan& pl, int max_n) {
   const int K = std::min(VP_KMAX, (VP_BITMAP_WORDS * 32) >> pl.part_shift);
@@ -671,30 +688,37 @@
   const long long b = 2ll * max_n / VP_EMAX + ne / K + 3;
   return (int)std::min<long long>(b, 65535);
 }
-size_t vox_part_hist_elems(int B) { return (size_t)B * VP_MAX_CHUNKS * (VP_NB_MAX / 2 + VP_CHUNK_TAIL); }
 size_t vox_part_start_elems(int B) { return (size_t)B * (VP_NB_MAX + 1); }
-size_t vox_part_chunk_start_elems(int B) { return (size_t)B * VP_MAX_CHUNKS * VP_NB_MAX; }
 size_t vox_part_bucket_elems(int B) { return (size_t)B * VP_NB_MAX; }
+
+template <bool NEED_MINMAX>
+static cudaError_t launch_vp_part(const Ctx& c, const VoxelPartArgs& a, int chunks, int gmax) {
+  const VoxFusedPlan& pl = a.plan;
+  const size_t smem = (size_t)pl.nb_pad * (sizeof(uint16_t) + sizeof(uint32_t));
+  cudaFuncSetAttribute(k_vp_part<NEED_MINMAX>, cudaFuncAttributeMaxDynamicSharedMemorySize, (int)smem);
+  cudaLaunchConfig_t cfg = {};
+  cfg.gridDim = dim3(chunks, c.B);
+  cfg.blockDim = dim3(VPP_THREADS);
+  cfg.dynamicSmemBytes = smem;
+  cfg.stream = c.stream;
+  cudaLaunchAttribute attr[1];
+  attr[0].id = cudaLaunchAttributeClusterDimension;
+  attr[0].val.clusterDim.x = chunks;
+  attr[0].val.clusterDim.y = 1;
+  attr[0].val.clusterDim.z = 1;
+  cfg.attrs = attr;
+  cfg.numAttrs = 1;
+  return cudaLaunchKernelEx(&cfg, k_vp_part<NEED_MINMAX>, a.in, a.in_stride, a.n_in, pl, a.part, c.cap, a.ne_bucket,
+                            a.ne_start, a.grec, a.n_groups, a.n_crop, a.flags, a.warnings, a.leaf, a.vf, a.desc, gmax,
+                            a.group_stride);
+}
 
 void run_voxel_part(const Ctx& c, const VoxelPartArgs& a) {
   const VoxFusedPlan& pl = a.plan;
   const int chunks = vox_part_chunks(c.grid_cap, c.B);
   const int gmax = std::max(1, std::min(a.group_launch, a.group_stride - 1));
-  cudaMemsetAsync(a.desc, 0, (size_t)c.B * a.group_stride * sizeof(unsigned), c.stream);
-  const size_t hsm = (size_t)(pl.nb_pad / 2) * sizeof(uint32_t);
-  if (a.want_keys)
-    KL(c, "k_vp_hist", k_vp_hist<true><<<dim3(chunks, c.B), VP_THREADS, hsm, c.stream>>>(a.in, a.in_stride, a.n_in, pl, a.ghist,
-                                                                                        chunks));
-  else
-    KL(c, "k_vp_hist", k_vp_hist<false><<<dim3(chunks, c.B), VP_THREADS, hsm, c.stream>>>(a.in, a.in_stride, a.n_in, pl, a.ghist,
-                                                                                         chunks));
-  KL(c, "k_vp_scan", k_vp_scan<<<c.B, VP_SCAN_THREADS, 0, c.stream>>>(a.ghist, a.chunk_start, a.ne_bucket, a.ne_start, a.grec, a.n_groups,
-                                                                      a.n_crop, a.flags, a.warnings, a.leaf, a.vf, pl, chunks,
-                                                                      a.want_keys, gmax, a.group_stride));
-  const size_t ssm = (size_t)pl.nb_pad * sizeof(uint32_t);
-  cudaFuncSetAttribute(k_vp_scatter, cudaFuncAttributeMaxDynamicSharedMemorySize, (int)ssm);
-  KL(c, "k_vp_scatter", k_vp_scatter<<<dim3(chunks, c.B), VPS_THREADS, ssm, c.stream>>>(a.in, a.in_stride, a.n_in, pl, a.chunk_start,
-                                                                                       a.flags, a.part, c.cap, chunks));
+  if (a.want_keys) KL(c, "k_vp_part", launch_vp_part<true>(c, a, chunks, gmax));
+  else KL(c, "k_vp_part", launch_vp_part<false>(c, a, chunks, gmax));
   const size_t rsm = sizeof(VpReduceSmem);
   if (a.want_keys) {
     cudaFuncSetAttribute(k_vp_reduce<true>, cudaFuncAttributeMaxDynamicSharedMemorySize, (int)rsm);
@@ -707,7 +731,7 @@
                              a.part, a.ne_start, a.ne_bucket, a.grec, a.n_groups, a.flags, pl, a.vf, a.out, a.out_keys,
                              a.n_out, a.desc, c.cap, a.group_stride));
   }
-  count_launch(c, 4);
+  count_launch(c, 2);
 }
 
 }
```

Result: no change. 21.67 billion (median of 6 runs) (+0.0%).
